# aleflabo/COSKAD

Measured on AMD Instinct MI355X. Metric: pose_clips_per_sec_fwd_bwd, higher is better.
Workload: dtype f32; 1 GPU; euclidean_encoder_dynamicCenter train step (fwd+mse-to-centre+L2 reg+bwd+Adam), synthetic clips B=4096/GPU T=12 V=17 C=2, channels 2-32-16-32-64, latent 16; clips_per_gpu=4096, global_batch=4096, head=euclidean, parallelism=dp1, hip_graph=False

## Files before the change

coskad_amd/csrc/api.hip:

```cpp
#include "common.h"
#include <utility>
#include <vector>

namespace coskad {

char* err_buf() {
  static thread_local char buf[512] = {0};
  return buf;
}

int fail(int code, const char* fmt, ...) {
  va_list ap;
  va_start(ap, fmt);
  vsnprintf(err_buf(), 512, fmt, ap);
  va_end(ap);
  return code;
}

int check_launch(const char* what) {
  hipError_t e = hipGetLastError();
  if (e != hipSuccess) return fail(COSKAD_ERR_LAUNCH, "%s: %s", what, hipGetErrorString(e));
  return COSKAD_OK;
}

}

namespace coskad {
namespace {
struct Probe {
  int kernel = 0, ci = 0, co = 0;
  int stride = 1, seen = 0;
  std::vector<std::pair<hipEvent_t, hipEvent_t>> evs;
} g_probe;
}

ProbeScope::ProbeScope(int kernel, int ci, int co, hipStream_t st) : st_(st) {
  if (g_probe.kernel == kernel && g_probe.ci == ci && g_probe.co == co && g_probe.evs.size() < 4096 &&
      (g_probe.seen++ % g_probe.stride) == 0) {
    hipEvent_t a, b;
    if (hipEventCreate(&a) == hipSuccess && hipEventCreate(&b) == hipSuccess) {
      (void)hipEventRecord(a, st);
      g_probe.evs.emplace_back(a, b);
      armed_ = true;
    }
  }
}
ProbeScope::~ProbeScope() {
  if (armed_) (void)hipEventRecord(g_probe.evs.back().second, st_);
}
}

extern "C" {
int coskad_probe_begin(int kernel, int Ci, int Co) {
  for (auto& e : coskad::g_probe.evs) { (void)hipEventDestroy(e.first); (void)hipEventDestroy(e.second); }
  coskad::g_probe.evs.clear();
  coskad::g_probe.kernel = kernel;
  coskad::g_probe.ci = Ci;
  coskad::g_probe.co = Co;
  coskad::g_probe.seen = 0;
  return COSKAD_OK;
}

int coskad_probe_stride(int n) {
  if (n < 1) return coskad::fail(COSKAD_ERR_ARG, "probe_stride: n=%d", n);
  coskad::g_probe.stride = n;
  return COSKAD_OK;
}

int coskad_probe_end(float* avg_ms, int* launches) {
  double tot = 0.0;
  int n = 0;
  for (auto& e : coskad::g_probe.evs) {
    float ms = 0.f;
    if (hipEventSynchronize(e.second) == hipSuccess && hipEventElapsedTime(&ms, e.first, e.second) == hipSuccess) {
      tot += ms;
      ++n;
    }
    (void)hipEventDestroy(e.first);
    (void)hipEventDestroy(e.second);
  }
  coskad::g_probe.evs.clear();
  coskad::g_probe.kernel = 0;
  if (avg_ms) *avg_ms = n ? (float)(tot / n) : 0.f;
  if (launches) *launches = n;
  return COSKAD_OK;
}

int coskad_abi_version(void) { return COSKAD_ABI_VERSION; }
const char* coskad_last_error(void) { return coskad::err_buf(); }
}
```

coskad_amd/csrc/bottleneck.hip:

```cpp
#include "tile_ops.h"
#include "layer_launch.h"

namespace coskad {

constexpr int kBtlBlock = 256;
constexpr int kBtlWaves = kBtlBlock / 64;
constexpr int kBtlFwdWaves = 8;

__global__ __launch_bounds__(64 * kBtlFwdWaves) void k_btlnk_fwd(const float* __restrict__ U,
                                                     const float* __restrict__ W,
                                                     const float* __restrict__ bias,
                                                     const float* __restrict__ slope,
                                                     float* __restrict__ z, int B, int K, int L) {
  __shared__ float red[kBtlFwdWaves][256];
  const int lane = threadIdx.x & 63, wave = threadIdx.x >> 6;
  const int i = lane & 15, kk = lane >> 4;
  const int n = blockIdx.x * 16 + i;
  const bool pre = slope != nullptr;
  const float a = pre ? slope[0] : 0.f;
  const bool rowok = n < B, colok = i < L;
  const float* up = U + (size_t)(rowok ? n : 0) * K;
  const float* wp = W + (size_t)(colok ? i : 0) * K;
  const int nsteps = ceil_div(K, 16);
  const int per = ceil_div(nsteps, kBtlFwdWaves);
  const int s0 = wave * per, s1 = min(nsteps, s0 + per);
  f32x4 acc = {0.f, 0.f, 0.f, 0.f};
  constexpr int UB = 4;
  for (int sb = s0; sb < s1; sb += UB) {
    float4 x[UB], w[UB];
#pragma unroll
    for (int u = 0; u < UB; ++u) {
      const int k = (sb + u) * 16 + 4 * kk;
      const bool ok = sb + u < s1 && k < K;
      x[u] = (ok && rowok) ? *reinterpret_cast<const float4*>(up + k) : float4{0.f, 0.f, 0.f, 0.f};
      w[u] = (ok && colok) ? *reinterpret_cast<const float4*>(wp + k) : float4{0.f, 0.f, 0.f, 0.f};
    }
#pragma unroll
    for (int u = 0; u < UB; ++u) {
      float4 xv = x[u];
      if (pre) { xv.x = prelu_f(xv.x, a); xv.y = prelu_f(xv.y, a); xv.z = prelu_f(xv.z, a); xv.w = prelu_f(xv.w, a); }
      acc = __builtin_amdgcn_mfma_f32_16x16x4f32(xv.x, w[u].x, acc, 0, 0, 0);
      acc = __builtin_amdgcn_mfma_f32_16x16x4f32(xv.y, w[u].y, acc, 0, 0, 0);
      acc = __builtin_amdgcn_mfma_f32_16x16x4f32(xv.z, w[u].z, acc, 0, 0, 0);
      acc = __builtin_amdgcn_mfma_f32_16x16x4f32(xv.w, w[u].w, acc, 0, 0, 0);
    }
  }
#pragma unroll
  for (int r = 0; r < 4; ++r) red[wave][(4 * (lane >> 4) + r) * 16 + (lane & 15)] = acc[r];
  __syncthreads();
  const int e = threadIdx.x, row = (e >> 4) & 15, col = e & 15;
  const int nn = blockIdx.x * 16 + row;
  if (e < 256 && nn < B && col < L) {
    float s = 0.f;
#pragma unroll
// ... 124 lines not shown
#pragma unroll
    for (int g = 0; g < 4; ++g) {
      const int nn = n0 + c, j = 4 * g + q;
      const float av = (nn < nend && j < L) ? dz[(size_t)nn * L + j] : 0.f;
      dx[0] = __builtin_amdgcn_mfma_f32_16x16x4f32(av, wf[g].x, dx[0], 0, 0, 0);
      dx[1] = __builtin_amdgcn_mfma_f32_16x16x4f32(av, wf[g].y, dx[1], 0, 0, 0);
      dx[2] = __builtin_amdgcn_mfma_f32_16x16x4f32(av, wf[g].z, dx[2], 0, 0, 0);
      dx[3] = __builtin_amdgcn_mfma_f32_16x16x4f32(av, wf[g].w, dx[3], 0, 0, 0);
    }
#pragma unroll
    for (int s = 0; s < 4; ++s) {
      const int nn = n0 + 4 * q + s;
      const bool ok = kok && nn < nend;
      const float4 u = ucur[s];
      float4 x = u;
      if (pre) { x.x = prelu_f(u.x, a); x.y = prelu_f(u.y, a); x.z = prelu_f(u.z, a); x.w = prelu_f(u.w, a); }
      const float dzv = (nn < nend && c < L) ? dz[(size_t)nn * L + c] : 0.f;
      dw[0] = __builtin_amdgcn_mfma_f32_16x16x4f32(dzv, x.x, dw[0], 0, 0, 0);
      dw[1] = __builtin_amdgcn_mfma_f32_16x16x4f32(dzv, x.y, dw[1], 0, 0, 0);
      dw[2] = __builtin_amdgcn_mfma_f32_16x16x4f32(dzv, x.z, dw[2], 0, 0, 0);
      dw[3] = __builtin_amdgcn_mfma_f32_16x16x4f32(dzv, x.w, dw[3], 0, 0, 0);
      float4 g = {dx[0][s], dx[1][s], dx[2][s], dx[3][s]};
      if (pre) {
        da += (u.x < 0.f ? g.x * u.x : 0.f) + (u.y < 0.f ? g.y * u.y : 0.f) +
              (u.z < 0.f ? g.z * u.z : 0.f) + (u.w < 0.f ? g.w * u.w : 0.f);
        g.x = u.x > 0.f ? g.x : a * g.x; g.y = u.y > 0.f ? g.y : a * g.y;
        g.z = u.z > 0.f ? g.z : a * g.z; g.w = u.w > 0.f ? g.w : a * g.w;
      }
      if (ok) *reinterpret_cast<float4*>(dU + (size_t)nn * K + kc) = g;
    }
#pragma unroll
    for (int s = 0; s < 4; ++s) ucur[s] = unext[s];
  }
  if (kok) {
    float* dst = dWp + (size_t)blockIdx.y * L * K;
#pragma unroll
    for (int r = 0; r < 4; ++r) {
      const int j = 4 * q + r;
      if (j < L) *reinterpret_cast<float4*>(dst + (size_t)j * K + kc) = float4{dw[0][r], dw[1][r], dw[2][r], dw[3][r]};
    }
  }
  da = wave_sum(da);
  if (lane == 0) sred[wave] = da;
  __syncthreads();
  if (threadIdx.x == 0) dap[blockIdx.y * gridDim.x + blockIdx.x] = (sred[0] + sred[1]) + (sred[2] + sred[3]);
}

__global__ __launch_bounds__(256) void k_btlnk_reduce(const float* __restrict__ partials, int P, size_t E,
                                                       float* __restrict__ out, const float* __restrict__ dz,
                                                       int B, int L, float* __restrict__ db,
                                                       const float* __restrict__ dap, int nda,
                                                       float* __restrict__ dslope, int accumulate,
                                                       const float* __restrict__ rows, int RP, int RE,
                                                       double* __restrict__ rsum) {
  __shared__ double sh[256];
  const unsigned nE = (unsigned)((E + 255) / 256);
  if (blockIdx.x > nE + L) {
    const int col = threadIdx.x & 15, slice = threadIdx.x >> 4;
    const int e = (int)(blockIdx.x - (nE + L + 1)) * 16 + col;
    double s = 0.0;
    if (e < RE) {
      const float* base = rows + e;
      int p = slice;
      for (; p + 7 * 16 < RP; p += 8 * 16) {
        float v[8];
#pragma unroll
        for (int u = 0; u < 8; ++u) v[u] = base[(size_t)(p + 16 * u) * RE];
#pragma unroll
        for (int u = 0; u < 8; ++u) s += (double)v[u];
      }
      for (; p < RP; p += 16) s += (double)base[(size_t)p * RE];
    }
    sh[threadIdx.x] = s;
    __syncthreads();
    if (slice == 0 && e < RE) {
      double t = 0.0;
#pragma unroll
      for (int k = 0; k < 16; ++k) t += sh[col + 16 * k];
      rsum[e] = t;
    }
    return;
  }
  if (blockIdx.x < nE) {
    const size_t e = (size_t)blockIdx.x * 256 + threadIdx.x;
    if (e >= E) return;
    double s = 0.0;
    int p = 0;
    for (; p + 8 <= P; p += 8) {
      float v[8];
#pragma unroll
      for (int u = 0; u < 8; ++u) v[u] = partials[(size_t)(p + u) * E + e];
#pragma unroll
      for (int u = 0; u < 8; ++u) s += (double)v[u];
    }
    for (; p < P; ++p) s += (double)partials[(size_t)p * E + e];
    out[e] = accumulate ? out[e] + (float)s : (float)s;
    return;
  }
  const int r = (int)(blockIdx.x - nE);
  double s = 0.0;
  if (r < L) {
    if (!db) return;
    for (int n = threadIdx.x; n < B; n += 256) s += (double)dz[(size_t)n * L + r];
  } else {
    if (!dslope) return;
    for (int i = threadIdx.x; i < nda; i += 256) s += (double)dap[i];
  }
  sh[threadIdx.x] = s;
  __syncthreads();
  for (int w = 128; w > 0; w >>= 1) {
    if ((int)threadIdx.x < w) sh[threadIdx.x] += sh[threadIdx.x + w];
    __syncthreads();
  }
  if (threadIdx.x == 0) {
    float* o = r < L ? db + r : dslope;
    o[0] = accumulate ? o[0] + (float)sh[0] : (float)sh[0];
  }
}

static int btl_chunks(int B, int K) {
  const int gx = ceil_div(K, 256);
  int s = (1024 + gx / 2) / gx;
  const int smax = ceil_div(B, 16);
  if (s > smax) s = smax;
  if (s > 64) s = 64;
  return s < 1 ? 1 : s;
}

int launch_btlnk_reduce(const float* partials, int P, size_t E, float* out, const float* dz, int B, int L, float* db,
                        const float* dap, int nda, float* dslope, int accumulate, hipStream_t stream, const float* rows,
                        int RP, int RE, double* rsum) {
  const unsigned extra = rows ? (unsigned)ceil_div(RE, 16) : 0u;
  hipLaunchKernelGGL(k_btlnk_reduce, dim3((unsigned)((E + 255) / 256) + L + 1 + extra), dim3(256), 0, stream, partials, P, E, out, dz,
                     B, L, db, dap, nda, dslope, accumulate, rows, RP, RE, rsum);
  return check_launch("btlnk_bwd_reduce");
}

constexpr int kBtlWideMax = 512;

}

using namespace coskad;

extern "C" {

int coskad_btlnk_fwd_f32(const float* U, const float* W, const float* bias, const float* slope, float* z,
                         int B, int K, int L, hipStream_t stream) {
  if (!U || !W || !z) return fail(COSKAD_ERR_ARG, "btlnk_fwd: null pointer");
  if (B <= 0 || K <= 0 || L <= 0) return fail(COSKAD_ERR_ARG, "btlnk_fwd: B=%d K=%d L=%d", B, K, L);
  if (L > 16) return fail(COSKAD_ERR_SHAPE, "btlnk_fwd: latent_dim=%d > 16 needs the workspace entry point coskad_btlnk_fwd_ws_f32", L);
  if (K % 4) return fail(COSKAD_ERR_SHAPE, "btlnk_fwd: K=%d must be a multiple of 4", K);
  hipLaunchKernelGGL(k_btlnk_fwd, dim3(ceil_div(B, 16)), dim3(64 * kBtlFwdWaves), 0, stream, U, W, bias, slope, z, B, K, L);
  return check_launch("btlnk_fwd");
}

size_t coskad_btlnk_fwd_ws_bytes(int B) { return (size_t)kBtlKS * (size_t)(B > 0 ? B : 0) * 16 * sizeof(float); }

size_t coskad_btlnk_fwd_ws_bytes_l(int B, int K, int L) {
  if (L > 16 && L <= kBtlWideMax) return wide_btlnk_fwd_ws_bytes(B, K, L);
  return coskad_btlnk_fwd_ws_bytes(B);
}

int coskad_btlnk_fwd_ws_f32(const float* U, const float* W, const float* bias, const float* slope, float* z, void* ws,
                            size_t ws_bytes, int B, int K, int L, hipStream_t stream) {
  if (!U || !W || !z || !ws) return fail(COSKAD_ERR_ARG, "btlnk_fwd_ws: null pointer");
  if (B <= 0 || K <= 0 || L <= 0) return fail(COSKAD_ERR_ARG, "btlnk_fwd_ws: B=%d K=%d L=%d", B, K, L);
  if (L > kBtlWideMax) return fail(COSKAD_ERR_SHAPE, "btlnk_fwd_ws: latent_dim=%d > %d not supported", L, kBtlWideMax);
  if (L > 16) {
    if (ws_bytes < wide_btlnk_fwd_ws_bytes(B, K, L)) return fail(COSKAD_ERR_WORKSPACE, "btlnk_fwd_ws: workspace too small");
    return wide_btlnk_fwd(U, W, bias, slope, z, ws, B, K, L, stream);
  }
  if (K % 16) return fail(COSKAD_ERR_SHAPE, "btlnk_fwd_ws: K=%d must be a multiple of 16", K);
  if (ws_bytes < coskad_btlnk_fwd_ws_bytes(B)) return fail(COSKAD_ERR_WORKSPACE, "btlnk_fwd_ws: workspace too small");
  float* part = reinterpret_cast<float*>(ws);
  hipLaunchKernelGGL(k_btlnk_fwd_t, dim3(ceil_div(B, 64), kBtlKS), dim3(256), 0, stream, U, W, slope, part, B, K, L);
  int rc;
  if ((rc = check_launch("btlnk_fwd_t"))) return rc;
  hipLaunchKernelGGL(k_btlnk_fwd_sum, dim3(ceil_div(B * 16, 256)), dim3(256), 0, stream, part, bias, z, B, L, kBtlKS);
  return check_launch("btlnk_fwd_sum");
}

size_t coskad_btlnk_bwd_ws_bytes(int B, int K, int L) {
  if (L > 16 && L <= kBtlWideMax) return wide_btlnk_bwd_ws_bytes(B, K, L);
  const int S = btl_chunks(B, K);
  return ((size_t)S * L * K + (size_t)S * ceil_div(K, 256) + 64) * sizeof(float);
}

int coskad_btlnk_bwd_f32(const float* U, const float* W, const float* dz, const float* slope, float* dU,
                         float* dW, float* db, float* dslope, void* ws, size_t ws_bytes, int accumulate,
                         int B, int K, int L, hipStream_t stream) {
  if (!U || !W || !dz || !dU || !dW || !ws) return fail(COSKAD_ERR_ARG, "btlnk_bwd: null pointer");
  if (B <= 0 || K <= 0 || L <= 0) return fail(COSKAD_ERR_ARG, "btlnk_bwd: B=%d K=%d L=%d", B, K, L);
  if (L > kBtlWideMax) return fail(COSKAD_ERR_SHAPE, "btlnk_bwd: latent_dim=%d > %d not supported", L, kBtlWideMax);
  if (ws_bytes < coskad_btlnk_bwd_ws_bytes(B, K, L)) return fail(COSKAD_ERR_WORKSPACE, "btlnk_bwd: workspace too small");
  if (L > 16) return wide_btlnk_bwd(U, W, dz, slope, dU, dW, db, dslope, ws, accumulate, B, K, L, stream);
  if (K % 4) return fail(COSKAD_ERR_SHAPE, "btlnk_bwd: K=%d must be a multiple of 4", K);
  const int S = btl_chunks(B, K);
  const int chunk = round_up(ceil_div(B, S), 16);
  const int gx = ceil_div(K, 256);
  float* dWp = reinterpret_cast<float*>(ws);
  float* dap = dWp + (size_t)S * L * K;
  {
    ProbeScope probe(KID_BTLNK_BWD, 0, L, stream);
    hipLaunchKernelGGL(k_btlnk_bwd, dim3(gx, S), dim3(kBtlBlock), 0, stream, U, W, dz, slope, dU, dWp, dap, B, K, L, chunk);
  }
  int rc = check_launch("btlnk_bwd");
  if (rc) return rc;
  return launch_btlnk_reduce(dWp, S, (size_t)L * K, dW, dz, B, L, db, dap, gx * S, (dslope && slope) ? dslope : nullptr, accumulate, stream,
                             nullptr, 0, 0, nullptr);
}

}
```

coskad_amd/csrc/btlnk_chain.hip:

```cpp
#include "fused_ops.h"
#include "layer_launch.h"

namespace coskad {
namespace bc {

using ff::f32x4; using ff::mfma; using ff::BufRes; using ff::make_res; using ff::buf_load4; using ff::buf_load1;
__device__ __forceinline__ void buf_store1(BufRes r, int voff, int soff, float v) {
  __builtin_amdgcn_raw_buffer_store_b32(__float_as_uint(v), r, voff, soff, 0);
}

constexpr int HID = 64;
constexpr int PT = 16;
constexpr int NCL = 16;
constexpr int RSTR = 17;
constexpr int kThreads = 512;
#ifndef BC_XCD
#define BC_XCD 1
#endif
#ifndef BC_PF
#define BC_PF 1
#endif
#ifndef BC_SKIP
#define BC_SKIP 0
#endif
// ... 174 lines not shown
      }
  }
  float* row = lds;
  float* red = lds + E;
  const float s4 = ssum + __shfl_xor(ssum, 16, 64);
  const float sch = s4 + __shfl_xor(s4, 32, 64);
  da = wave_sum(da);
  for (int hh = 0; hh < 2; ++hh) {
    if (h == hh) {
#pragma unroll
      for (int t = 0; t < CT; ++t)
#pragma unroll
        for (int r = 0; r < 4; ++r) {
          const int o = 16 * wc + 4 * q + r, cc = 16 * t + c;
          float* p = row + o * Ci + cc;
          p[0] = (hh ? p[0] : 0.f) + pacc[t][r];
          p[HID * Ci] = (hh ? p[HID * Ci] : 0.f) + qacc[t][r];
        }
      if (q == 0) {
        float* p = row + 2 * HID * Ci + 16 * wc + c;
        p[0] = (hh ? p[0] : 0.f) + sch;
      }
      if (lane == 0) red[wave] = da;
    }
    __syncthreads();
  }
  float* dstrow = prow + (size_t)wg * E;
  for (int e = tid; e < E; e += kThreads) dstrow[e] = row[e];
  if (tid == 0) dap[wg] = ((red[0] + red[1]) + (red[2] + red[3])) + ((red[4] + red[5]) + (red[6] + red[7]));
}

struct Plan {
  int npt, S, chunk;
};
static Plan plan(int B, int TV) {
  Plan p;
  p.npt = ceil_div(TV, PT);
  int s = 256 / p.npt;
  const int smax = ceil_div(B, NCL);
  if (s > smax) s = smax;
  if (s < 1) s = 1;
  p.chunk = round_up(ceil_div(B, s), NCL);
  p.S = ceil_div(B, p.chunk);
  return p;
}
static inline size_t sums_offset(int rows, int E) { return ((size_t)rows * E + 1) / 2 * 2; }

}

}

using namespace coskad;

extern "C" {

int coskad_btlnk_bwd_chain_ok(int K, int TV, int below_Ci) {
  return TV > 0 && TV % 4 == 0 && K == bc::HID * TV && (below_Ci == 16 || below_Ci == 32);
}

int coskad_btlnk_bwd_chain_rows(int B, int TV) {
  if (B <= 0 || TV <= 0) return 0;
  const bc::Plan p = bc::plan(B, TV);
  return p.npt * p.S;
}

size_t coskad_btlnk_bwd_chain_floats(int B, int TV, int below_Ci) {
  const size_t E = 2 * (size_t)bc::HID * below_Ci + bc::HID;
  return bc::sums_offset(coskad_btlnk_bwd_chain_rows(B, TV), (int)E) + 2 * E;
}

size_t coskad_btlnk_bwd_chain_ws_bytes(int B, int K, int L, int TV) {
  if (B <= 0 || TV <= 0) return 0;
  const bc::Plan p = bc::plan(B, TV);
  return ((size_t)p.S * L * K + (size_t)p.S * p.npt + 64) * sizeof(float);
}

int coskad_btlnk_bwd_chain_f32(const float* U, const float* W, const float* dz, const float* slope, float* dU, float* dW,
                               float* db, float* dslope, void* ws, size_t ws_bytes, int accumulate, int B, int K, int L,
                               const float* below_in, const float* below_Z, const float* below_in_slope, int below_Ci, int TV,
                               float* stats_out, size_t stats_out_bytes, int* stats_rows, hipStream_t stream) {
  if (!U || !W || !dz || !dU || !dW || !ws || !below_in || !below_Z || !stats_out || !stats_rows)
    return fail(COSKAD_ERR_ARG, "btlnk_bwd_chain: null pointer");
  if (B <= 0 || K <= 0 || L <= 0) return fail(COSKAD_ERR_ARG, "btlnk_bwd_chain: B=%d K=%d L=%d", B, K, L);
  if (L > 16) return fail(COSKAD_ERR_SHAPE, "btlnk_bwd_chain: latent_dim=%d > 16 not supported", L);
  if (!coskad_btlnk_bwd_chain_ok(K, TV, below_Ci))
    return fail(COSKAD_ERR_SHAPE, "btlnk_bwd_chain: K=%d TV=%d below_Ci=%d (needs K = 64 TV, TV %% 4 == 0, 16 / 32 channels below)", K, TV, below_Ci);
  if ((size_t)stats_out & 7) return fail(COSKAD_ERR_ARG, "btlnk_bwd_chain: stats_out must be 8-byte aligned");
  if (ws_bytes < coskad_btlnk_bwd_chain_ws_bytes(B, K, L, TV)) return fail(COSKAD_ERR_WORKSPACE, "btlnk_bwd_chain: workspace too small");
  if (stats_out_bytes < coskad_btlnk_bwd_chain_floats(B, TV, below_Ci) * sizeof(float))
    return fail(COSKAD_ERR_WORKSPACE, "btlnk_bwd_chain: stats_out %zu bytes too small", stats_out_bytes);
  const bc::Plan p = bc::plan(B, TV);
  const int rows = p.npt * p.S;
  const int E = 2 * bc::HID * below_Ci + bc::HID;
  float* dWp = reinterpret_cast<float*>(ws);
  float* dap = dWp + (size_t)p.S * L * K;
  const size_t lds = (size_t)bc::NCL * ((bc::HID * bc::RSTR + 4) + (2 * below_Ci * bc::RSTR + 4)) * sizeof(float);
  int rc;
  {
  ProbeScope probe(KID_BTLNK_BWD, below_Ci, L, stream);
  if (below_Ci == 32) {
    auto k = bc::k_btlnk_bwd_stats<2>;
    (void)hipFuncSetAttribute((const void*)k, hipFuncAttributeMaxDynamicSharedMemorySize, (int)lds);
    hipLaunchKernelGGL(k, dim3(p.npt * p.S), dim3(bc::kThreads), lds, stream, U, W, dz, slope, dU, dWp, dap, below_in, below_Z,
                       below_in_slope, stats_out, B, TV, L, p.chunk);
  } else {
    auto k = bc::k_btlnk_bwd_stats<1>;
    (void)hipFuncSetAttribute((const void*)k, hipFuncAttributeMaxDynamicSharedMemorySize, (int)lds);
    hipLaunchKernelGGL(k, dim3(p.npt * p.S), dim3(bc::kThreads), lds, stream, U, W, dz, slope, dU, dWp, dap, below_in, below_Z,
                       below_in_slope, stats_out, B, TV, L, p.chunk);
  }
  }
  if ((rc = check_launch("btlnk_bwd_stats"))) return rc;
  *stats_rows = rows;
  return launch_btlnk_reduce(dWp, p.S, (size_t)L * K, dW, dz, B, L, db, dap, rows, (dslope && slope) ? dslope : nullptr, accumulate, stream,
                             stats_out, rows, E, reinterpret_cast<double*>(stats_out + bc::sums_offset(rows, E)));
}

}
```

coskad_amd/csrc/common.h:

```cpp
#pragma once
#include <hip/hip_runtime.h>
#include <cstdarg>
#include <cstdio>
#include <cstring>

#define COSKAD_ABI_VERSION 1

#define COSKAD_OK 0
#define COSKAD_ERR_ARG (-1)
#define COSKAD_ERR_SHAPE (-2)
#define COSKAD_ERR_LAUNCH (-3)
#define COSKAD_ERR_WORKSPACE (-4)

namespace coskad {

char* err_buf();
int fail(int code, const char* fmt, ...);
int check_launch(const char* what);

#ifndef COSKAD_BLOCK
#define COSKAD_BLOCK 512
#endif
constexpr int kFlatBlock = COSKAD_BLOCK;
#ifndef COSKAD_MINWAVES
#define COSKAD_MINWAVES 4
#endif
constexpr int kMinWaves = COSKAD_MINWAVES;
constexpr int kMaxLdsBytes = 160 * 1024;
constexpr float kBnEps = 1e-5f;

template <int T, int V>
struct Geo {
  static constexpr int TV = T * V;
  static constexpr int LD = (TV % 2 == 0) ? TV + 1 : TV;
  static constexpr int Block = TV > 256 ? 2 * COSKAD_BLOCK : COSKAD_BLOCK;
  static constexpr int Scratch = (Block / 64) * 256;
};

enum { KID_LAYER_APPLY = 1, KID_BWD_DATA = 2, KID_BWD_REDUCE = 3, KID_FWD_MOMENTS = 4, KID_GCN_PARAMS = 5,
       KID_LAYER_BWD = 6 , KID_FUSED_FWD = 7,
       KID_BTLNK_BWD = 8  };
struct ProbeScope {
  ProbeScope(int kernel, int ci, int co, hipStream_t st);
  ~ProbeScope();
  hipStream_t st_;
  bool armed_ = false;
};

__host__ __device__ inline int ceil_div(int a, int b) { return (a + b - 1) / b; }
__host__ __device__ inline int round_up(int a, int b) { return ceil_div(a, b) * b; }

__device__ __forceinline__ float prelu_f(float x, float a) { return x > 0.f ? x : a * x; }

__device__ __forceinline__ int tid_here() {
  int t = threadIdx.x;
  asm volatile("" : "+v"(t));
  return t;
}

// ... 52 lines not shown
```

coskad_amd/csrc/first_layer.hip:

```cpp
#include "mfma_ops.h"
#include "layer_launch.h"

namespace coskad {
namespace fl {

__device__ __forceinline__ float act(float x, bool pre, float a) { return (pre && x < 0.f) ? a * x : x; }
__device__ __forceinline__ float4 act4(float4 v, bool pre, float a) {
  return float4{act(v.x, pre, a), act(v.y, pre, a), act(v.z, pre, a), act(v.w, pre, a)};
}
__device__ __forceinline__ float dot4(const float4& a, const float4& b) { return (a.x * b.x + a.y * b.y) + (a.z * b.z + a.w * b.w); }

constexpr int NW = 4;
template <int CI, int RW>
__global__ __launch_bounds__(64 * NW, 4) void k_first_stats(const float* __restrict__ in, const float* __restrict__ Zg,
                                                           const float* __restrict__ dU, const float* __restrict__ in_slope,
                                                           float* __restrict__ partials, int B, int Co, int TVr, int need_q) {
  const int lane = threadIdx.x & 63;
  const int wave = uniform(threadIdx.x >> 6);
  const bool pre = in_slope != nullptr;
  const float a_in = pre ? in_slope[0] : 0.f;
  const int n4 = TVr >> 2;
  float pP[RW][CI], pQ[RW][CI], pS[RW];
#pragma unroll
  for (int k = 0; k < RW; ++k) {
    pS[k] = 0.f;
#pragma unroll
    for (int c = 0; c < CI; ++c) { pP[k][c] = 0.f; pQ[k][c] = 0.f; }
  }
  for (int clip = blockIdx.x; clip < B; clip += gridDim.x) {
    const float* gz = Zg + (size_t)clip * CI * TVr;
    const float* gx = in + (size_t)clip * CI * TVr;
    const float* gd = dU + ((size_t)clip * Co + (size_t)wave * RW) * TVr;
    for (int l = lane; l < n4; l += 64) {
      float4 z[CI], x[CI];
#pragma unroll
      for (int c = 0; c < CI; ++c) {
        z[c] = *reinterpret_cast<const float4*>(gz + c * TVr + 4 * l);
        x[c] = need_q ? act4(*reinterpret_cast<const float4*>(gx + c * TVr + 4 * l), pre, a_in) : float4{0.f, 0.f, 0.f, 0.f};
      }
      float4 d[RW];
#pragma unroll
      for (int k = 0; k < RW; ++k)
        d[k] = (wave * RW + k < Co) ? *reinterpret_cast<const float4*>(gd + (size_t)k * TVr + 4 * l) : float4{0.f, 0.f, 0.f, 0.f};
#pragma unroll
      for (int k = 0; k < RW; ++k) {
        pS[k] += (d[k].x + d[k].y) + (d[k].z + d[k].w);
#pragma unroll
        for (int c = 0; c < CI; ++c) {
          pP[k][c] += dot4(d[k], z[c]);
          pQ[k][c] += dot4(d[k], x[c]);
        }
      }
    }
// ... 91 lines not shown
      }
#pragma unroll
      for (int c = 0; c < CI; ++c) *reinterpret_cast<float4*>(part + (wave * CI + c) * TV + 4 * l) = dz[c];
    }
    __syncthreads();
    for (int e = tid; e < CI * TV; e += NTH) {
      const int c = e / TV, p = e - c * TV;
      float v = kt[c];
#pragma unroll
      for (int c2 = 0; c2 < CI; ++c2) v = fmaf(Kt[c2 * CiP + c], Zg[((size_t)clip * CI + c2) * TV + p], v);
#pragma unroll
      for (int w = 0; w < NW; ++w) v += part[(w * CI + c) * TV + p];
      dZl[e] = v;
      Xl[e] = act(in[(size_t)clip * CI * TV + e], pre, a_in);
    }
    __syncthreads();
    for (int e = tid; e < CI * TV; e += NTH) {
      const int c = e / TV, p = e - c * TV, q = p / V, v = p - q * V;
      float y = 0.f, dy = 0.f;
#pragma unroll
      for (int t = 0; t < T; ++t) y = fmaf(Xl[c * TV + t * V + v], TwL[(t * T + q) * V + v], y);
#pragma unroll
      for (int w = 0; w < V; ++w) dy = fmaf(AwL[q * V * V + v * V + w], dZl[c * TV + q * V + w], dy);
      Yl[e] = y;
      dYl[e] = dy;
    }
    __syncthreads();
#pragma unroll
    for (int k = 0; k < KA; ++k) {
      float s = 0.f;
#pragma unroll
      for (int c = 0; c < CI; ++c) s = fmaf(Yl[c * TV + ya[k]], dZl[c * TV + za[k]], s);
      accA[k] += s;
    }
#pragma unroll
    for (int k = 0; k < KT; ++k) {
      float s = 0.f;
#pragma unroll
      for (int c = 0; c < CI; ++c) s = fmaf(Xl[c * TV + xt[k]], dYl[c * TV + yt[k]], s);
      accT[k] += s;
    }
  }
  float* dst = partials + (size_t)blockIdx.x * (NA + NT);
#pragma unroll
  for (int k = 0; k < KA; ++k)
    if (tid + NTH * k < NA) dst[tid + NTH * k] = accA[k];
#pragma unroll
  for (int k = 0; k < KT; ++k)
    if (tid + NTH * k < NT) dst[NA + tid + NTH * k] = accT[k];
}


constexpr int NWM = 8;
template <int T, int V, int CI>
__global__ __launch_bounds__(64 * NWM, 4) void k_first_moments(const float* __restrict__ in, const float* __restrict__ Aw,
                                                          const float* __restrict__ Tw, const float* __restrict__ in_slope,
                                                          float* __restrict__ partials, int B, float* __restrict__ Zout) {
  constexpr int TV = T * V, NA = T * V * V, NT = V * T * T, KP = (TV + 63) / 64;
  extern __shared__ __attribute__((aligned(16))) float lds[];
  float* AwL = lds;
  float* TwL = AwL + NA;
  const int tid = threadIdx.x, lane = tid & 63;
  const int wave = uniform(tid >> 6);
  float* Xl = TwL + NT + wave * 2 * CI * TV;
  float* Yl = Xl + CI * TV;
  const bool pre = in_slope != nullptr;
  const float a_in = pre ? in_slope[0] : 0.f;
  for (int e = tid; e < NA; e += 64 * NWM) AwL[e] = Aw[e];
  for (int e = tid; e < NT; e += 64 * NWM) {
    const int v = e / (T * T), tq = e - v * T * T;
    TwL[tq * V + v] = Tw[e];
  }
  float mx[CI][CI], mz[CI][CI], sx[CI], sz[CI];
#pragma unroll
  for (int a = 0; a < CI; ++a) {
    sx[a] = 0.f; sz[a] = 0.f;
#pragma unroll
    for (int b = 0; b < CI; ++b) { mx[a][b] = 0.f; mz[a][b] = 0.f; }
  }
  __syncthreads();
  const int rounds = (B + gridDim.x * NWM - 1) / (gridDim.x * NWM);
  for (int r = 0; r < rounds; ++r) {
    const int clip = (r * gridDim.x + blockIdx.x) * NWM + wave;
    const bool live = clip < B;
    const float* gx = in + (size_t)(live ? clip : 0) * CI * TV;
#pragma unroll
    for (int k = 0; k < KP; ++k) {
      const int p = lane + 64 * k;
      if (p < TV) {
        float x[CI];
#pragma unroll
        for (int c = 0; c < CI; ++c) {
          x[c] = live ? act(gx[c * TV + p], pre, a_in) : 0.f;
          Xl[c * TV + p] = x[c];
          sx[c] += x[c];
        }
#pragma unroll
        for (int a = 0; a < CI; ++a)
#pragma unroll
          for (int b = 0; b < CI; ++b) mx[a][b] = fmaf(x[a], x[b], mx[a][b]);
      }
    }
    __syncthreads();
#pragma unroll
    for (int k = 0; k < KP; ++k) {
      const int p = lane + 64 * k;
      if (p < TV) {
        const int q = p / V, v = p - q * V;
#pragma unroll
        for (int c = 0; c < CI; ++c) {
          float y = 0.f;
#pragma unroll
          for (int t = 0; t < T; ++t) y = fmaf(Xl[c * TV + t * V + v], TwL[(t * T + q) * V + v], y);
          Yl[c * TV + p] = y;
        }
      }
    }
    __syncthreads();
    float* gz = Zout + (size_t)(live ? clip : 0) * CI * TV;
#pragma unroll
    for (int k = 0; k < KP; ++k) {
      const int p = lane + 64 * k;
      if (p < TV) {
        const int t = p / V, w = p - t * V;
        float z[CI];
#pragma unroll
        for (int c = 0; c < CI; ++c) {
          float acc = 0.f;
#pragma unroll
          for (int v = 0; v < V; ++v) acc = fmaf(Yl[c * TV + t * V + v], AwL[t * V * V + v * V + w], acc);
          z[c] = acc;
          if (live) gz[c * TV + p] = acc;
          sz[c] += acc;
        }
#pragma unroll
        for (int a = 0; a < CI; ++a)
#pragma unroll
          for (int b = 0; b < CI; ++b) mz[a][b] = fmaf(z[a], z[b], mz[a][b]);
      }
    }
    __syncthreads();
  }
  constexpr int E = 2 * (CI * CI + CI);
  float* row = TwL + NT;
  __syncthreads();
#pragma unroll
// ... 71 lines not shown
    else if (Ci == 2) LAUNCH_FS_C(2);
    else if (Ci == 3) LAUNCH_FS_C(3);
    else LAUNCH_FS_C(4);
  }
#undef LAUNCH_FS_C
#undef LAUNCH_FS
  return check_launch("first_stats");
}

template <int T, int V>
static int launch_first_bwd_tv(const float* in, const float* Zg, const float* dU, const float* Aw, const float* Tw, const float* coef,
                               const float* in_slope, float* partials, int B, int Ci, int Co, int max_rows, hipStream_t st,
                               int* rows_out) {
  constexpr int NWB = fl::first_bwd_waves<T, V>();
  int grid = B < 512 ? B : 512;
  if (grid > max_rows) grid = max_rows;
  *rows_out = grid;
  const int rw = ceil_div(Co, NWB);
  const size_t lds = ((size_t)T * V * V + (size_t)V * T * T + (4 + NWB) * (size_t)Ci * T * V) * sizeof(float);
#define LAUNCH_FB1(CI, RW)                                                                                              \
  do {                                                                                                                  \
    auto k = fl::k_first_bwd<T, V, CI, RW>;                                                                             \
    if (lds > 64 * 1024) (void)hipFuncSetAttribute((const void*)k, hipFuncAttributeMaxDynamicSharedMemorySize, (int)lds); \
    hipLaunchKernelGGL(k, dim3(grid), dim3(64 * NWB), lds, st, in, Zg, dU, Aw, Tw, coef, in_slope, partials, B, Co);             \
  } while (0)
#define LAUNCH_FB1_C(CI)                        \
  do {                                          \
    if (rw <= 4) LAUNCH_FB1(CI, 4);             \
    else if (rw <= 8) LAUNCH_FB1(CI, 8);        \
    else LAUNCH_FB1(CI, 16);                    \
  } while (0)
  {
    ProbeScope probe(KID_BWD_DATA, Ci, Co, st);
    if (Ci == 1) LAUNCH_FB1_C(1);
    else if (Ci == 2) LAUNCH_FB1_C(2);
    else if (Ci == 3) LAUNCH_FB1_C(3);
    else LAUNCH_FB1_C(4);
  }
#undef LAUNCH_FB1_C
#undef LAUNCH_FB1
  return check_launch("first_bwd");
}

int launch_first_bwd(const float* in, const float* Zg, const float* dU, const float* Aw, const float* Tw, const float* coef,
                     const float* in_slope, float* partials, int B, int Ci, int Co, int T, int V, int max_rows, hipStream_t st,
                     int* rows_out) {
#define CALL(T_, V_) return launch_first_bwd_tv<T_, V_>(in, Zg, dU, Aw, Tw, coef, in_slope, partials, B, Ci, Co, max_rows, st, rows_out)
  COSKAD_DISPATCH_TV(T, V, CALL);
#undef CALL
}

template <int T, int V>
static int launch_first_moments_tv(const float* in, const float* Aw, const float* Tw, const float* in_slope, float* partials, int B,
                                   int Ci, float* Zout, int max_rows, hipStream_t st, int* rows_out) {
  int grid = (B + fl::NWM - 1) / fl::NWM;
  if (grid > 512) grid = 512;
  if (grid > max_rows) grid = max_rows;
  *rows_out = grid;
  const size_t lds = ((size_t)T * V * V + (size_t)V * T * T + 2 * fl::NWM * (size_t)Ci * T * V) * sizeof(float);
#define LAUNCH_FM(CI)                                                                                                   \
  do {                                                                                                                  \
    auto k = fl::k_first_moments<T, V, CI>;                                                                             \
    if (lds > 64 * 1024) (void)hipFuncSetAttribute((const void*)k, hipFuncAttributeMaxDynamicSharedMemorySize, (int)lds); \
    hipLaunchKernelGGL(k, dim3(grid), dim3(64 * fl::NWM), lds, st, in, Aw, Tw, in_slope, partials, B, Zout);                    \
  } while (0)
  {
    ProbeScope probe(KID_FWD_MOMENTS, Ci, 0, st);
    if (Ci == 1) LAUNCH_FM(1);
    else if (Ci == 2) LAUNCH_FM(2);
    else if (Ci == 3) LAUNCH_FM(3);
    else LAUNCH_FM(4);
  }
#undef LAUNCH_FM
  return check_launch("first_moments");
}

int launch_first_moments(const float* in, const float* Aw, const float* Tw, const float* in_slope, float* partials, int B, int Ci,
                         int T, int V, float* Zout, int max_rows, hipStream_t st, int* rows_out) {
#define CALL(T_, V_) return launch_first_moments_tv<T_, V_>(in, Aw, Tw, in_slope, partials, B, Ci, Zout, max_rows, st, rows_out)
  COSKAD_DISPATCH_TV(T, V, CALL);
#undef CALL
}

int launch_first_apply(const float* Z, const float* in, float* out, const float* wfold, const float* bias, const float* in_slope,
                       int B, int Ci, int Co, int TVr, hipStream_t st) {
  const int grid = B < 2048 ? B : 2048;
  const size_t lds = 2 * (size_t)Ci * TVr * sizeof(float);
  const int CoP = round_up(Co, 16);
#define LAUNCH_FAP(CI) hipLaunchKernelGGL((fl::k_first_apply<CI>), dim3(grid), dim3(256), lds, st, Z, in, out, wfold, bias, in_slope, B, Co, CoP, TVr)
  {
    ProbeScope probe(KID_LAYER_APPLY, Ci, Co, st);
    if (Ci == 1) LAUNCH_FAP(1);
    else if (Ci == 2) LAUNCH_FAP(2);
    else if (Ci == 3) LAUNCH_FAP(3);
    else LAUNCH_FAP(4);
  }
#undef LAUNCH_FAP
  return check_launch("first_apply");
}

}
```

coskad_amd/csrc/fused_apply_next.hip:

```cpp
#include "fused_ops.h"
#include "layer_launch.h"

#ifndef FN_ABLATE
#define FN_ABLATE 0
#endif

namespace coskad {
namespace fn {

using namespace ff;

struct FtabArgs {
  const float* A[4];
  const float* Tm[4];
  float* tab[4];
};
__global__ void k_build_ftab(FtabArgs args) {
  const int layer = blockIdx.y;
  const float* __restrict__ Aw = args.A[layer];
  const float* __restrict__ Tw = args.Tm[layer];
  const int e = blockIdx.x * blockDim.x + threadIdx.x;
  if (e >= LAYER_F4 * 4) return;
  float val = 0.f;
  if (e < TEMP_F4 * 4) {
    const int v = e / 256, l = (e >> 2) & 63, s = e & 3, j = l & 15, q = l >> 4;
    if (s < 3 && j < T) val = Tw[v * T * T + (4 * s + q) * T + j];
  } else {
    const int r = e - TEMP_F4 * 4;
    const int t = r / (3 * 256), c = (r / 256) % 3, l = (r >> 2) & 63, k = 4 * c + (r & 3), j = l & 15, q = l >> 4;
    if (k < 10) {
      const int s = k < 5 ? k : k - 5, w = 4 * s + q;
      if (w < V) val = Aw[t * V * V + w * V + (k < 5 ? j : 16)];
    }
  }
  args.tab[layer][e] = val;
}

template <int CT, int OTP>
__global__ __launch_bounds__(256, 1) void k_layer_apply_next(const float* __restrict__ in, const float* __restrict__ Zg,
                                                            const float* __restrict__ wfold, const float* __restrict__ bias,
                                                            const float* __restrict__ in_slope, const float* __restrict__ out_slope,
                                                            const float* __restrict__ ftab, float* __restrict__ out,
                                                            float* __restrict__ Znext, float* __restrict__ partials, int B) {
  constexpr int Ci = CT ? 16 * CT : 2, Co = 16 * OTP, CoP = Co, NG = 2 * CT;
  constexpr int NACC = OTP == 1 ? 2 : 3;
  constexpr int E = 2 * (Co * Co + Co);
  static_assert(OTP == 1 || OTP == 2, "the 32-row image holds the whole output");
  extern __shared__ __attribute__((aligned(16))) float lds_all[];
  const int lane = threadIdx.x & 63;
  const int wave = __builtin_amdgcn_readfirstlane(threadIdx.x >> 6);
  float* lds = lds_all + wave * WAVE_LDS_W;
  float* r1 = lds + R1;
  float* r2 = lds + R2;
  auto geo = [&]() {
    int l = lane;
    asm volatile("" : "+v"(l));
    return Lane{l & 15, l >> 4};
  };
  auto olane = [&]() {
    int l = lane;
    asm volatile("" : "+v"(l));
    return l;
  };
  const bool pre = in_slope != nullptr;
  const float a_in = pre ? in_slope[0] : 0.f;
  const float a_out = out_slope[0];
  const int l16 = lane * 16;
  const BufRes wres = make_res(wfold, 2 * Ci * CoP * 4u);
  const BufRes bres = make_res(bias, CoP * 4u);
  const BufRes tabres = make_res(ftab, LAYER_F4 * 16u);
  const int nwaves = gridDim.x * 4;
  auto clip_res = [&](const float* base, int c, int rows) {
    const bool in_range = c < B;
#ifdef COSKAD_HOT
    return make_res(base + (size_t)(in_range ? (c & 63) : 0) * rows * TV, in_range ? rows * TV * 4u : 0u);
#else
    return make_res(base + (size_t)(in_range ? c : 0) * rows * TV, in_range ? rows * TV * 4u : 0u);
#endif
  };
  constexpr int QTAIL = 4 * (TV / 4) - 192;
  const int l16t = lane < QTAIL ? l16 : 0x7ffffff0;
  float4 gb[16];
  auto qload = [&](const BufRes& res, int row0, int q) {
#pragma unroll
    for (int c = 0; c < 4; ++c) gb[4 * q + c] = buf_load4(res, c < 3 ? l16 : l16t, ((row0 + 4 * q) * (TV / 4) + 64 * c) * 16);
  };
  auto qstore = [&](int q, bool act) {
    const int ln = olane();
// ... 202 lines not shown
  }

  float* row = lds_all;
  __syncthreads();
  const Lane L = geo();
  auto put = [&](int w, float* base, const f32x4 (&g)[NACC], const float (&s)[OTP]) {
#pragma unroll
    for (int r = 0; r < 4; ++r) {
      const int i = 4 * L.q + r, j = L.j;
      if constexpr (OTP == 1) {
        float* p = base + i * Co + j;
        p[0] = (w ? p[0] : 0.f) + (g[0][r] + g[1][r]);
      } else {
        float* p00 = base + i * Co + j;
        float* p01 = base + i * Co + 16 + j;
        float* p10 = base + (16 + j) * Co + i;
        float* p11 = base + (16 + i) * Co + 16 + j;
        p00[0] = (w ? p00[0] : 0.f) + g[0][r];
        p01[0] = (w ? p01[0] : 0.f) + g[1][r];
        p10[0] = (w ? p10[0] : 0.f) + g[1][r];
        p11[0] = (w ? p11[0] : 0.f) + g[2][r];
      }
    }
#pragma unroll
    for (int rt = 0; rt < OTP; ++rt) {
      const float t = quad_sum(s[rt]);
      if (L.q == 0) {
        float* p = base + Co * Co + 16 * rt + L.j;
        p[0] = (w ? p[0] : 0.f) + t;
      }
    }
  };
  for (int w = 0; w < 4; ++w) {
    if (wave == w) {
      put(w, row, gx, sx);
      put(w, row + Co * Co + Co, gz, sz);
    }
    __syncthreads();
  }
  float* dst = partials + (size_t)blockIdx.x * E;
  for (int e = threadIdx.x; e < E; e += 256) dst[e] = row[e];
}

}

bool layer_apply_next_ok(int T_, int V_, int Ci, int Co) {
  return T_ == ff::T && V_ == ff::V && (Ci == 2 || Ci == 16 || Ci == 32) && (Co == 16 || Co == 32);
}

int ftab_floats() { return ff::LAYER_F4 * 4; }

int launch_build_ftab(const float* const* A, const float* const* Tm, float* const* tab, int n, hipStream_t st) {
  if (n < 1 || n > 4) return fail(COSKAD_ERR_ARG, "build_ftab: 1..4 layers per launch, got %d", n);
  fn::FtabArgs args{};
  for (int i = 0; i < n; ++i) {
    if (!A[i] || !Tm[i] || !tab[i]) return fail(COSKAD_ERR_ARG, "build_ftab: null pointer (layer %d)", i);
    args.A[i] = A[i]; args.Tm[i] = Tm[i]; args.tab[i] = tab[i];
  }
  hipLaunchKernelGGL(fn::k_build_ftab, dim3(ceil_div(ff::LAYER_F4 * 4, 256), n), dim3(256), 0, st, args);
  return check_launch("build_ftab");
}

static bool apply_next_bpc_on(int Ci, int Co) { return (Ci == 2 && Co == 32) || (Ci == 32 && Co == 16) || (Ci == 16 && Co == 32); }
int layer_apply_next_rows(int B, int Ci, int Co) {
  if (apply_next_bpc_on(Ci, Co)) return apply_next_bpc_rows(B);
  const int nblk = (B + 3) / 4;
  return nblk < 256 ? nblk : 256;
}

int launch_layer_apply_next(const float* Z, const float* in, float* out, const float* wfold, const float* bias,
                            const float* in_slope, const float* out_slope, const float* ftab, float* Znext, float* partials,
                            int B, int Ci, int Co, hipStream_t st, int* rows_out) {
  const size_t lds = (size_t)4 * ff::WAVE_LDS_W * sizeof(float);
  const int grid = layer_apply_next_rows(B, Ci, Co);
  *rows_out = grid;
  if (apply_next_bpc_on(Ci, Co))
    return launch_layer_apply_next_bpc(Z, in, out, wfold, bias, in_slope, out_slope, ftab, Znext, partials, B, Ci, Co, st);
#define LAUNCH_FN(CT, OTP)                                                                                            \
  do {                                                                                                                \
    auto k = fn::k_layer_apply_next<CT, OTP>;                                                                         \
    (void)hipFuncSetAttribute((const void*)k, hipFuncAttributeMaxDynamicSharedMemorySize, (int)lds);                  \
    hipLaunchKernelGGL(k, dim3(grid), dim3(256), lds, st, in, Z, wfold, bias, in_slope, out_slope, ftab, out, Znext,  \
                       partials, B);                                                                                  \
  } while (0)
  {
    ProbeScope probe(KID_LAYER_APPLY, Ci, Co, st);
    if (Ci == 2 && Co == 16) LAUNCH_FN(0, 1);
    else if (Ci == 2 && Co == 32) LAUNCH_FN(0, 2);
    else if (Ci == 16 && Co == 16) LAUNCH_FN(1, 1);
    else if (Ci == 16 && Co == 32) LAUNCH_FN(1, 2);
    else if (Ci == 32 && Co == 16) LAUNCH_FN(2, 1);
    else if (Ci == 32 && Co == 32) LAUNCH_FN(2, 2);
    else return fail(COSKAD_ERR_SHAPE, "apply_next: unsupported channels (%d, %d)", Ci, Co);
  }
#undef LAUNCH_FN
  return check_launch("layer_apply_next");
}

}

using namespace coskad;
extern "C" {

int coskad_layer_apply_next_ok(int Ci, int Co, int T, int V) { return layer_apply_next_ok(T, V, Ci, Co) ? 1 : 0; }
int coskad_ftab_floats(void) { return ftab_floats(); }
int coskad_layer_apply_next_rows(int B, int Ci, int Co) { return layer_apply_next_rows(B, Ci, Co); }

// ... 24 lines not shown
```

coskad_amd/csrc/fused_ops.h:

```cpp
#pragma once
#include "common.h"

namespace coskad {
namespace ff {

using f32x4 = __attribute__((ext_vector_type(4))) float;

constexpr int T = 12, V = 17, TV = T * V;
#ifndef FF_LD
#define FF_LD 206
#endif
constexpr int LD = FF_LD;
constexpr int R1 = 0, R2 = 32 * LD;
constexpr int PADCOL = TV;
constexpr int WAVE_LDS = 48 * LD;
constexpr int LDW = 208;
constexpr int WAVE_LDS_W = 32 * LD + 16 * LDW;
constexpr int NTILE = T + 1;
#ifndef FF_AB_UNROLL
#define FF_AB_UNROLL _Pragma("unroll")
#endif
#ifndef FF_ABLATE
#define FF_ABLATE 0
#endif
#ifndef FF_CABL
#define FF_CABL 0
#endif
#ifndef FF_TILE_FENCE
#define FF_TILE_FENCE
#endif
constexpr int KP = NTILE * 4 * 64 * 4;
constexpr int TEMP_F4 = V * 64;
constexpr int LAYER_F4 = TEMP_F4 + T * 3 * 64;
enum { W1A = 0, W1B = 2, WP = 4, WR = 12, WX3 = 20, WZ3 = 28, WZ4 = 36, WX4 = 68, B1 = 100, B2 = 108, B3 = 112, B4 = 120, NWREG = 136 };

__device__ __forceinline__ f32x4 mfma(float a, float b, f32x4 c) {
  return __builtin_amdgcn_mfma_f32_16x16x4f32(a, b, c, 0, 0, 0);
}
__device__ __forceinline__ float prelu(float x, float a) { return x > 0.f ? x : a * x; }
__device__ __forceinline__ f32x4 prelu4(f32x4 v, float a) {
  return f32x4{prelu(v[0], a), prelu(v[1], a), prelu(v[2], a), prelu(v[3], a)};
}

struct Lane {
  int j, q;
};

using u32x4 = __attribute__((ext_vector_type(4))) unsigned int;
using BufRes = __amdgpu_buffer_rsrc_t;
__device__ __forceinline__ BufRes make_res(const void* p, unsigned bytes) {
  return __builtin_amdgcn_make_buffer_rsrc(const_cast<void*>(p), 0, bytes, 0x00020000);
}
__device__ __forceinline__ float4 buf_load4(BufRes r, int voff, int soff) {
  const u32x4 v = __builtin_amdgcn_raw_buffer_load_b128(r, voff, soff, 0);
  return float4{__uint_as_float(v[0]), __uint_as_float(v[1]), __uint_as_float(v[2]), __uint_as_float(v[3])};
}
__device__ __forceinline__ float buf_load1(BufRes r, int voff, int soff) {
  return __uint_as_float(__builtin_amdgcn_raw_buffer_load_b32(r, voff, soff, 0));
}
__device__ __forceinline__ void buf_store4(BufRes r, int voff, int soff, const float4& v) {
  const u32x4 u = {__float_as_uint(v.x), __float_as_uint(v.y), __float_as_uint(v.z), __float_as_uint(v.w)};
  __builtin_amdgcn_raw_buffer_store_b128(u, r, voff, soff, 0);
}

struct TOp {
  float a0, a1, a2;
};
template <int ROWS, bool ACT = false>
__device__ __forceinline__ TOp temporal_read(const float* img, int rt, int v, const Lane& L, float slope = 0.f) {
  const float* p = img + (16 * rt + L.j) * LD + L.q * V + v;
  TOp o{p[0], p[4 * V], p[8 * V]};
  if (ACT) { o.a0 = prelu(o.a0, slope); o.a1 = prelu(o.a1, slope); o.a2 = prelu(o.a2, slope); }
  if (ROWS < 16) {
    const bool ok = L.j < ROWS;
    o.a0 = ok ? o.a0 : 0.f; o.a1 = ok ? o.a1 : 0.f; o.a2 = ok ? o.a2 : 0.f;
  }
  return o;
}
__device__ __forceinline__ f32x4 temporal_mm(const TOp& o, const float4& rec) {
  f32x4 acc = {0.f, 0.f, 0.f, 0.f};
  acc = mfma(o.a0, rec.x, acc);
  acc = mfma(o.a1, rec.y, acc);
  acc = mfma(o.a2, rec.z, acc);
  return acc;
}
template <int ROWS>
// ... 230 lines not shown
```

coskad_amd/csrc/heads.hip:

```cpp
#include "tile_ops.h"
#include "heads_common.h"

namespace coskad {

struct Vec {
  float v[LMAX];
};

__device__ __forceinline__ Vec load_vec(const float* p, int L) {
  Vec r;
#pragma unroll
  for (int j = 0; j < LMAX; ++j) r.v[j] = j < L ? p[j] : 0.f;
  return r;
}
__device__ __forceinline__ void store_vec(float* p, const Vec& a, int L) {
#pragma unroll
  for (int j = 0; j < LMAX; ++j)
    if (j < L) p[j] = a.v[j];
}
__device__ __forceinline__ float dot(const Vec& a, const Vec& b) {
  float s = 0.f;
#pragma unroll
  for (int j = 0; j < LMAX; ++j) s = fmaf(a.v[j], b.v[j], s);
  return s;
}

struct Embed {
  Vec p;
  float un_raw, un, tn, en_raw;
  bool clamped;
};
__device__ __forceinline__ Embed hyp_embed(const Vec& u) {
  Embed r;
  r.un_raw = sqrtf(dot(u, u));
  r.un = fmaxf(r.un_raw, kMinNorm);
  r.tn = tanhf(fminf(fmaxf(r.un, -kTanhClamp), kTanhClamp));
  const float f = r.tn / r.un;
  Vec e;
#pragma unroll
  for (int j = 0; j < LMAX; ++j) e.v[j] = f * u.v[j];
  r.en_raw = sqrtf(dot(e, e));
  const float en = fmaxf(r.en_raw, kMinNorm);
  const float maxnorm = 1.f - kBallEps;
  r.clamped = en > maxnorm;
  const float s = r.clamped ? maxnorm / en : 1.f;
#pragma unroll
  for (int j = 0; j < LMAX; ++j) r.p.v[j] = r.clamped ? e.v[j] / en * maxnorm : e.v[j];
  (void)s;
  return r;
}

__device__ __forceinline__ float poincare_dist(const Vec& c, const Vec& p, Vec* gp) {
  const float x2 = dot(c, c), y2 = dot(p, p), xy = -dot(c, p);
  const float alpha = 1.f + 2.f * xy + y2, beta = 1.f - x2;
  const float den = 1.f + 2.f * xy + x2 * y2;
  const float D = den + kMobiusEps;
  Vec m;
#pragma unroll
  for (int j = 0; j < LMAX; ++j) m.v[j] = (alpha * (-c.v[j]) + beta * p.v[j]) / D;
  const float mn = sqrtf(dot(m, m));
  const float mc = fminf(fmaxf(mn, -1.f + kArtanhEps), 1.f - kArtanhEps);
  const float d = (log1pf(mc) - log1pf(-mc));
  if (gp) {
    const float gmn = 2.f / (1.f - mc * mc);
    const float inv = mn > 0.f ? gmn / mn : 0.f;
    Vec gm;
#pragma unroll
    for (int j = 0; j < LMAX; ++j) gm.v[j] = inv * m.v[j];
    const float gD = -dot(gm, m) / D;
    float galpha = 0.f;
#pragma unroll
// ... 16 lines not shown
    float egp = 0.f;
#pragma unroll
    for (int j = 0; j < LMAX; ++j) egp = fmaf(f * u.v[j], gp.v[j], egp);
#pragma unroll
    for (int j = 0; j < LMAX; ++j) ge.v[j] = maxnorm * (gp.v[j] / en - f * u.v[j] * egp / (en * en * en));
  } else {
    ge = gp;
  }
  Vec gu;
  float gf = dot(ge, u);
  float coef = 0.f;
  if (em.un_raw > kMinNorm) {
    const float sech2 = em.un < kTanhClamp ? 1.f - em.tn * em.tn : 0.f;
    const float df = (sech2 * em.un - em.tn) / (em.un * em.un);
    coef = gf * df / em.un_raw;
  }
#pragma unroll
  for (int j = 0; j < LMAX; ++j) gu.v[j] = f * ge.v[j] + coef * u.v[j];
  return gu;
}

constexpr int kHeadSlots = LMAX + 3;

constexpr int kHeadSingleRows = kFlatBlock;
__host__ __device__ inline int head_blocks(int B) { return B <= kHeadSingleRows ? 1 : ceil_div(B, kFlatBlock); }

__device__ __forceinline__ void block_partials(const float (&vals)[kHeadSlots], float* partials, float scale0, float* stats,
                                               float* acc) {
  __shared__ float sh[kFlatBlock / 64][kHeadSlots];
  const int lane = threadIdx.x & 63, wave = threadIdx.x >> 6;
#pragma unroll
  for (int k = 0; k < kHeadSlots; ++k) {
    const float s = wave_sum(vals[k]);
    if (lane == 0) sh[wave][k] = s;
  }
  __syncthreads();
  if (threadIdx.x < kHeadSlots) {
    float s = 0.f;
    for (int w = 0; w < kFlatBlock / 64; ++w) s += sh[w][threadIdx.x];
    if (gridDim.x == 1) {
      if (stats) stats[threadIdx.x] = threadIdx.x == 0 ? s * scale0 : s;
      if (acc) acc[threadIdx.x] += s;
    } else {
      partials[blockIdx.x * kHeadSlots + threadIdx.x] = s;
    }
  }
}

__global__ __launch_bounds__(kFlatBlock) void k_mse_head(const float* __restrict__ z,
                                                    const float* __restrict__ cvec,
                                                    float* __restrict__ dz, float* __restrict__ score,
                                                    float* __restrict__ partials, int B, int L,
                                                    float gscale, float scale0, float* __restrict__ stats,
                                                    float* __restrict__ acc) {
  float vals[kHeadSlots];
#pragma unroll
  for (int k = 0; k < kHeadSlots; ++k) vals[k] = 0.f;
  const Vec c = load_vec(cvec, L);
#pragma unroll 4
  for (int n = blockIdx.x * kFlatBlock + threadIdx.x; n < B; n += gridDim.x * kFlatBlock) {
    const Vec u = load_vec(z + (size_t)n * L, L);
    Vec g;
    float sq = 0.f;
#pragma unroll
    for (int j = 0; j < LMAX; ++j) {
      const float d = j < L ? u.v[j] - c.v[j] : 0.f;
      sq = fmaf(d, d, sq);
      g.v[j] = 2.f * d * gscale;
      vals[1 + j] += u.v[j];
    }
    vals[0] += sq;
    vals[LMAX + 1] += 1.f;
    vals[LMAX + 2] += sqrtf(dot(u, u));
    if (dz) store_vec(dz + (size_t)n * L, g, L);
    if (score) score[n] = sq / (float)L;
  }
  block_partials(vals, partials, scale0, stats, acc);
}

__global__ __launch_bounds__(kFlatBlock) void k_mahalanobis_head(const float* __restrict__ z,
                                                            const float* __restrict__ cvec,
                                                            const float* __restrict__ VI,
                                                            float* __restrict__ dz, float* __restrict__ score,
                                                            float* __restrict__ partials, int B, int L,
                                                            float gscale, float scale0, float* __restrict__ stats,
                                                            float* __restrict__ acc) {
  __shared__ float vi[LMAX * LMAX];
  for (int e = threadIdx.x; e < LMAX * LMAX; e += kFlatBlock) {
    const int r = e / LMAX, q = e - r * LMAX;
    vi[e] = (r < L && q < L) ? VI[r * L + q] : 0.f;
  }
  __syncthreads();
  float vals[kHeadSlots];
#pragma unroll
  for (int k = 0; k < kHeadSlots; ++k) vals[k] = 0.f;
  const Vec c = load_vec(cvec, L);
  for (int n = blockIdx.x * kFlatBlock + threadIdx.x; n < B; n += gridDim.x * kFlatBlock) {
    const Vec u = load_vec(z + (size_t)n * L, L);
    Vec d, w, wt;
#pragma unroll
    for (int j = 0; j < LMAX; ++j) { d.v[j] = j < L ? u.v[j] - c.v[j] : 0.f; w.v[j] = 0.f; wt.v[j] = 0.f; }
#pragma unroll
    for (int r = 0; r < LMAX; ++r)
#pragma unroll
      for (int q = 0; q < LMAX; ++q) {
        const float a = vi[r * LMAX + q];
        w.v[r] = fmaf(a, d.v[q], w.v[r]);
        wt.v[q] = fmaf(a, d.v[r], wt.v[q]);
      }
    const float dist = sqrtf(dot(d, w));
    vals[0] += dist;
#pragma unroll
    for (int j = 0; j < LMAX; ++j) vals[1 + j] += u.v[j];
    vals[LMAX + 1] += 1.f;
    vals[LMAX + 2] += sqrtf(dot(u, u));
    if (score) score[n] = dist;
    if (dz) {
      Vec g;
      const float inv = gscale / (2.f * dist);
#pragma unroll
      for (int j = 0; j < LMAX; ++j) g.v[j] = (w.v[j] + wt.v[j]) * inv;
      store_vec(dz + (size_t)n * L, g, L);
    }
  }
  block_partials(vals, partials, scale0, stats, acc);
}

// ... 6 lines not shown
  for (int n0 = 0; n0 < B; n0 += CH) {
    const int nc = min(CH, B - n0);
    __syncthreads();
    for (int e = threadIdx.x; e < nc * L; e += LMAX * LMAX) {
      const int r = e / L, q = e - r * L;
      zs[r * LMAX + q] = z[(size_t)(n0 + r) * L + q];
    }
    __syncthreads();
    if (i < L && j < L)
      for (int r = 0; r < nc; ++r) s = fmaf(zs[r * LMAX + i], zs[r * LMAX + j], s);
  }
  if (i < L && j < L) gram[i * L + j] = accumulate ? gram[i * L + j] + s : s;
}

__global__ __launch_bounds__(kFlatBlock) void k_poincare_head(const float* __restrict__ z,
                                                         const float* __restrict__ cvec,
                                                         float* __restrict__ dz, float* __restrict__ zh,
                                                         float* __restrict__ score,
                                                         float* __restrict__ partials, int B, int L,
                                                         float gscale, float scale0, float* __restrict__ stats,
                                                         float* __restrict__ acc) {
  float vals[kHeadSlots];
#pragma unroll
  for (int k = 0; k < kHeadSlots; ++k) vals[k] = 0.f;
  for (int n = blockIdx.x * kFlatBlock + threadIdx.x; n < B; n += gridDim.x * kFlatBlock) {
    const Vec u = load_vec(z + (size_t)n * L, L);
    const Embed em = hyp_embed(u);
    if (zh) store_vec(zh + (size_t)n * L, em.p, L);
    const float y2 = dot(em.p, em.p);
    const float gamma = 2.f / (1.f - y2);
#pragma unroll
    for (int j = 0; j < LMAX; ++j) vals[1 + j] += gamma * em.p.v[j];
    vals[LMAX + 1] += gamma - 1.f;
    vals[LMAX + 2] += sqrtf(y2);
    if (cvec) {
      const Vec c = load_vec(cvec, L);
      Vec gp;
      const float d = poincare_dist(c, em.p, dz ? &gp : nullptr);
      vals[0] += d;
      if (score) score[n] = d;
      if (dz) {
#pragma unroll
        for (int j = 0; j < LMAX; ++j) gp.v[j] *= gscale;
        store_vec(dz + (size_t)n * L, hyp_embed_bwd(u, em, gp), L);
      }
    }
  }
  block_partials(vals, partials, scale0, stats, acc);
}

__global__ __launch_bounds__(64) void k_head_finalize(const float* __restrict__ partials, int P,
                                                       float scale0, float* __restrict__ stats,
                                                       float* __restrict__ acc) {
  const int k = threadIdx.x;
  if (k >= kHeadSlots) return;
  double s = 0.0;
  for (int p = 0; p < P; ++p) s += (double)partials[p * kHeadSlots + k];
  if (stats) stats[k] = (float)(k == 0 ? s * (double)scale0 : s);
  if (acc) acc[k] += (float)s;
}

__global__ __launch_bounds__(kFlatBlock) void k_poincare_dist(const float* __restrict__ zh,
                                                         const float* __restrict__ cvec,
                                                         float* __restrict__ score, int B, int L) {
  const int n = blockIdx.x * kFlatBlock + threadIdx.x;
  if (n >= B) return;
  const Vec p = load_vec(zh + (size_t)n * L, L), c = load_vec(cvec, L);
  score[n] = poincare_dist(c, p, nullptr);
}

__global__ __launch_bounds__(kFlatBlock) void k_poincare_logmap0(const float* __restrict__ y, float* __restrict__ out, int B, int L) {
  const int n = blockIdx.x * kFlatBlock + threadIdx.x;
  if (n >= B) return;
  const Vec p = load_vec(y + (size_t)n * L, L);
  const float yn = fmaxf(sqrtf(dot(p, p)), kMinNorm);
  const float yc = fminf(fmaxf(yn, -1.f + kArtanhEps), 1.f - kArtanhEps);
  const float at = 0.5f * (log1pf(yc) - log1pf(-yc));
  Vec o;
#pragma unroll
  for (int j = 0; j < LMAX; ++j) o.v[j] = p.v[j] / yn * at;
  store_vec(out + (size_t)n * L, o, L);
}

__global__ void k_midpoint_finalize(const float* __restrict__ acc, float* __restrict__ cvec, int L) {
  if (threadIdx.x != 0 || blockIdx.x != 0) return;
  const double s = fmax((double)acc[LMAX + 1], 1e-10);
  double m[LMAX], mn2 = 0.0;
  for (int j = 0; j < L; ++j) { m[j] = (double)acc[1 + j] / s; mn2 += m[j] * m[j]; }
  const double mn = fmax(sqrt(mn2), 1e-15);
  const double mc = fmin(mn, 1.0 - 1e-7);
  const double at = 0.5 * log((1.0 + mc) / (1.0 - mc));
  const double sc = tanh(0.5 * at) / mn;
  for (int j = 0; j < L; ++j) cvec[j] = (float)(sc * m[j]);
}

__global__ void k_center_finalize(const float* __restrict__ acc, float eps, float* __restrict__ cvec,
                                  int L) {
  const int j = threadIdx.x;
  if (j >= L || blockIdx.x != 0) return;
  float c = acc[1 + j] / acc[LMAX + 1];
  if (fabsf(c) < eps && c < 0.f) c = -eps;
  if (fabsf(c) < eps && c > 0.f) c = eps;
  cvec[j] = c;
}

__global__ __launch_bounds__(256) void k_sqnorm_masked(const float* __restrict__ p,
                                                        const float* __restrict__ mask, size_t n,
                                                        float* __restrict__ partials) {
  __shared__ float sh[4];
  float s = 0.f;
  for (size_t i = (size_t)blockIdx.x * 256 + threadIdx.x; i < n; i += (size_t)gridDim.x * 256) {
    const float v = p[i];
// ... 33 lines not shown
__global__ __launch_bounds__(256) void k_adam_dev(float* __restrict__ p, const float* __restrict__ g,
                                                   float* __restrict__ m, float* __restrict__ v,
                                                   const float* __restrict__ mask, size_t n,
                                                   const float* __restrict__ hyper, float beta1, float beta2,
                                                   float eps, float gscale, float reg_coef) {
  const size_t i = (size_t)blockIdx.x * 256 + threadIdx.x;
  if (i >= n) return;
  const float lr = hyper[0], bc1 = 1.f - hyper[1], bc2s = sqrtf(1.f - hyper[2]);
  const float pi = p[i];
  float gi = g[i] * gscale;
  if (reg_coef != 0.f) gi = fmaf(reg_coef * (mask ? mask[i] : 1.f), pi, gi);
  const float mi = beta1 * m[i] + (1.f - beta1) * gi;
  const float vi = beta2 * v[i] + (1.f - beta2) * gi * gi;
  m[i] = mi;
  v[i] = vi;
  p[i] = pi - (lr / bc1) * (mi / (sqrtf(vi) / bc2s + eps));
}

__global__ __launch_bounds__(256) void k_scale_sum(const float* __restrict__ v, int n, float scale,
                                                    float* __restrict__ out) {
  __shared__ double sh[256];
  double s = 0.0;
  for (int i = threadIdx.x; i < n; i += 256) s += (double)v[i];
  sh[threadIdx.x] = s;
  __syncthreads();
  for (int w = 128; w > 0; w >>= 1) {
    if (threadIdx.x < w) sh[threadIdx.x] += sh[threadIdx.x + w];
    __syncthreads();
  }
  if (threadIdx.x == 0) out[0] = (float)(sh[0] * (double)scale);
}

}

using namespace coskad;

extern "C" {

int coskad_head_slots(void) { return kHeadSlots; }
size_t coskad_head_ws_floats(int B) { return (size_t)ceil_div(B, kFlatBlock) * kHeadSlots; }
int coskad_head_slots_l(int L) { return L > 0 && L <= kWideLMax ? head_slots_for(L) : 0; }
size_t coskad_head_ws_floats_l(int B, int L) {
  if (L > LMAX && L <= kWideLMax) return wide_head_ws_floats(B, L);
  return coskad_head_ws_floats(B);
}

int coskad_mse_head_f32(const float* z, const float* c, float* dz, float* score, float* stats, float* acc,
                        float upstream, float* ws, int B, int L, hipStream_t stream) {
  if (!z || !c || !ws) return fail(COSKAD_ERR_ARG, "mse_head: null pointer");
  if (B <= 0 || L <= 0 || L > kWideLMax) return fail(COSKAD_ERR_SHAPE, "mse_head: B=%d latent=%d (max %d)", B, L, kWideLMax);
  if (L > LMAX) return wide_mse_head(z, c, dz, score, stats, acc, upstream, ws, B, L, stream);
  const int P = head_blocks(B);
  hipLaunchKernelGGL(k_mse_head, dim3(P), dim3(kFlatBlock), 0, stream, z, c, dz, score, ws, B, L,
                     upstream / ((float)B * (float)L), 1.f / ((float)B * (float)L), stats, acc);
  if ((stats || acc) && P > 1)
    hipLaunchKernelGGL(k_head_finalize, dim3(1), dim3(64), 0, stream, ws, P, 1.f / ((float)B * (float)L), stats, acc);
  return check_launch("mse_head");
}

int coskad_mahalanobis_head_f32(const float* z, const float* c, const float* VI, float* dz, float* score,
                                float* stats, float* acc, float* gram, int gram_accumulate, float upstream,
                                float* ws, int B, int L, hipStream_t stream) {
  if (!z || !c || !VI || !ws) return fail(COSKAD_ERR_ARG, "mahalanobis_head: null pointer");
  if (B <= 0 || L <= 0 || L > kWideLMax) return fail(COSKAD_ERR_SHAPE, "mahalanobis_head: B=%d latent=%d (max %d)", B, L, kWideLMax);
  if (L > LMAX) return wide_mahalanobis_head(z, c, VI, dz, score, stats, acc, gram, gram_accumulate, upstream, ws, B, L, stream);
  const int P = head_blocks(B);
  hipLaunchKernelGGL(k_mahalanobis_head, dim3(P), dim3(kFlatBlock), 0, stream, z, c, VI, dz, score, ws, B, L,
                     upstream / (float)B, 1.f / (float)B, stats, acc);
  if ((stats || acc) && P > 1)
    hipLaunchKernelGGL(k_head_finalize, dim3(1), dim3(64), 0, stream, ws, P, 1.f / (float)B, stats, acc);
  if (gram) hipLaunchKernelGGL(k_gram, dim3(1), dim3(LMAX * LMAX), 0, stream, z, gram, B, L, gram_accumulate);
  return check_launch("mahalanobis_head");
}

int coskad_poincare_head_f32(const float* z, const float* c, float* dz, float* zh, float* score,
                             float* stats, float* acc, float upstream, float* ws, int B, int L,
                             hipStream_t stream) {
  if (!z || !ws) return fail(COSKAD_ERR_ARG, "poincare_head: null pointer");
  if (B <= 0 || L <= 0 || L > kWideLMax) return fail(COSKAD_ERR_SHAPE, "poincare_head: B=%d latent=%d (max %d)", B, L, kWideLMax);
  if (L > LMAX) return wide_poincare_head(z, c, dz, zh, score, stats, acc, upstream, ws, B, L, stream);
  const int P = head_blocks(B);
  hipLaunchKernelGGL(k_poincare_head, dim3(P), dim3(kFlatBlock), 0, stream, z, c, dz, zh, score, ws, B, L,
                     upstream / (float)B, 1.f / (float)B, stats, acc);
  if ((stats || acc) && P > 1)
    hipLaunchKernelGGL(k_head_finalize, dim3(1), dim3(64), 0, stream, ws, P, 1.f / (float)B, stats, acc);
  return check_launch("poincare_head");
}

int coskad_poincare_dist_f32(const float* zh, const float* c, float* score, int B, int L, hipStream_t stream) {
  if (!zh || !c || !score) return fail(COSKAD_ERR_ARG, "poincare_dist: null pointer");
  if (B <= 0 || L <= 0 || L > kWideLMax) return fail(COSKAD_ERR_SHAPE, "poincare_dist: B=%d latent=%d (max %d)", B, L, kWideLMax);
  if (L > LMAX) return wide_poincare_dist(zh, c, score, B, L, stream);
  hipLaunchKernelGGL(k_poincare_dist, dim3(ceil_div(B, kFlatBlock)), dim3(kFlatBlock), 0, stream, zh, c, score, B, L);
  return check_launch("poincare_dist");
}

int coskad_poincare_logmap0_f32(const float* y, float* out, int B, int L, hipStream_t stream) {
  if (!y || !out) return fail(COSKAD_ERR_ARG, "poincare_logmap0: null pointer");
  if (B <= 0 || L <= 0 || L > kWideLMax) return fail(COSKAD_ERR_SHAPE, "poincare_logmap0: B=%d latent=%d (max %d)", B, L, kWideLMax);
  if (L > LMAX) return wide_poincare_logmap0(y, out, B, L, stream);
  hipLaunchKernelGGL(k_poincare_logmap0, dim3(ceil_div(B, kFlatBlock)), dim3(kFlatBlock), 0, stream, y, out, B, L);
  return check_launch("poincare_logmap0");
}

int coskad_center_finalize_f32(const float* acc, float* c, float eps, int L, hipStream_t stream) {
  if (!acc || !c || L <= 0 || L > kWideLMax) return fail(COSKAD_ERR_ARG, "center_finalize: bad argument (latent=%d, max %d)", L, kWideLMax);
  if (L > LMAX) return wide_center_finalize(acc, c, eps, L, stream);
  hipLaunchKernelGGL(k_center_finalize, dim3(1), dim3(64), 0, stream, acc, eps, c, L);
  return check_launch("center_finalize");
}

// ... 47 lines not shown
```

coskad_amd/csrc/heads_common.h:

```cpp
#pragma once
#include "common.h"

namespace coskad {

constexpr int LMAX = 16;
constexpr int kWideLMax = 512;
constexpr float kMinNorm = 1e-5f;
constexpr float kBallEps = 1e-3f;
constexpr float kArtanhEps = 1e-5f;
constexpr float kMobiusEps = 1e-5f;
constexpr float kTanhClamp = 15.f;

__host__ __device__ inline int head_lp(int L) { return L > LMAX ? L : LMAX; }
__host__ __device__ inline int head_slots_for(int L) { return head_lp(L) + 3; }

size_t wide_head_ws_floats(int B, int L);
int wide_mse_head(const float* z, const float* c, float* dz, float* score, float* stats, float* acc, float upstream, float* ws,
                  int B, int L, hipStream_t stream);
int wide_mahalanobis_head(const float* z, const float* c, const float* VI, float* dz, float* score, float* stats, float* acc,
                          float* gram, int gram_accumulate, float upstream, float* ws, int B, int L, hipStream_t stream);
int wide_poincare_head(const float* z, const float* c, float* dz, float* zh, float* score, float* stats, float* acc,
                       float upstream, float* ws, int B, int L, hipStream_t stream);
int wide_poincare_dist(const float* zh, const float* c, float* score, int B, int L, hipStream_t stream);
int wide_poincare_logmap0(const float* y, float* out, int B, int L, hipStream_t stream);
int wide_center_finalize(const float* acc, float* c, float eps, int L, hipStream_t stream);
int wide_midpoint_finalize(const float* acc, float* c, int L, hipStream_t stream);

}
```

coskad_amd/csrc/layer_launch.h:

```cpp
#pragma once
#include "common.h"
#include <cstdlib>
#include <type_traits>

extern "C" int coskad_window_ok(int T, int V);
extern "C" int coskad_layer_train_window_ok(int T, int V, int Ci, int Co);
extern "C" int coskad_layer_train_window_narrow_ok(int T, int V, int Ci, int Co);

namespace coskad {

#ifdef COSKAD_ABLATE
inline int ablate_env(const char* name, int dflt) {
  const char* e = getenv(name);
  return e ? atoi(e) : dflt;
}
#else
constexpr int ablate_env(const char*, int dflt) { return dflt; }
#endif

template <class F>
inline void with_tiles(int n, F&& f) {
  if (n == 1) f(std::integral_constant<int, 1>{});
  else if (n == 2) f(std::integral_constant<int, 2>{});
  else if (n == 3) f(std::integral_constant<int, 3>{});
// ... 26 lines not shown
  float* stats = nullptr;
};
struct StatsOnly {
  float* out = nullptr;
  int* rows_out = nullptr;
};
struct LayerBwdArgs {
  const float* in = nullptr;
  const float* dU = nullptr;
  const float* A = nullptr;
  const float* Tm = nullptr;
  const float* in_slope = nullptr;
  const float* stat = nullptr;
  const float* Wt = nullptr;
  const float* gt = nullptr;
  const float* Wr = nullptr;
  const float* gr = nullptr;
  const float* Z = nullptr;
  LayerGrads g;
  void* ws = nullptr;
  size_t ws_bytes = 0;
  int accumulate = 0;
  int B = 0, Ci = 0, Co = 0;
  hipStream_t stream = nullptr;
  ChainIn chain;
  double stats_count = 0.0;
  Below below;
  StatsOnly stats_only;
  float* dz_ext = nullptr;
};

struct BnConvParams {
  const float* Wt = nullptr;
  const float* bt = nullptr;
  const float* gt = nullptr;
  const float* bet = nullptr;
  float* rm_t = nullptr;
  float* rv_t = nullptr;
  long long* nbt_t = nullptr;
  const float* Wr = nullptr;
  const float* br = nullptr;
  const float* gr = nullptr;
  const float* ber = nullptr;
  float* rm_r = nullptr;
  float* rv_r = nullptr;
  long long* nbt_r = nullptr;
  float momentum = 0.f;
};
struct FoldOut {
  float* wfold = nullptr;
  float* bias = nullptr;
  float* stat = nullptr;
};
struct LayerStatsArgs {
  const float* in = nullptr;
  const float* A = nullptr;
  const float* Tm = nullptr;
  const float* in_slope = nullptr;
  const float* partials = nullptr;
  int rows = 0;
  BnConvParams p;
  FoldOut out;
  float* Zout = nullptr;
  double* sums = nullptr;
  void* ws = nullptr;
  size_t ws_bytes = 0;
  int B = 0, Ci = 0, Co = 0;
  hipStream_t stream = nullptr;
};

void launch_reduce_partials(const float* partials, int rows, int E, double* out, hipStream_t st);

int launch_window_gcn(const float* in, float* out, const float* Aw, const float* Tw, int rows, int T, int V, int adjoint,
                      hipStream_t st);
int launch_window_params(const float* x, const float* dZ, const float* Aw, const float* Tw, float* dA, float* dT, void* ws,
                         int accumulate, int rows, int T, int V, hipStream_t st, float* dX, const float* add,
                         const float* in_slope = nullptr, float* dap = nullptr, int* rows_out = nullptr);
size_t window_params_ws_bytes(int T, int V);

bool window_moments_ok(int T, int V, int Ci);
int launch_window_moments(const float* in, const float* Aw, const float* Tw, const float* in_slope, float* partials, int B, int Ci,
                          int T, int V, int need_x, float* Zout, hipStream_t st, int* rows_out);
bool window_flat_ok(int TV, int Ci, int Co);
int launch_window_apply(const float* Z, const float* in, float* out, const float* wfold, const float* bias, const float* in_slope,
                        int B, int Ci, int Co, int TV, hipStream_t st);
int launch_window_stats(const float* in, const float* Zg, const float* dU, const float* in_slope, float* partials, int B, int Ci, int Co,
                        int TV, int need_q, hipStream_t st, int* rows_out);
int launch_window_data(const float* in, const float* Z, const float* dU, const float* coef, const float* in_slope, float* dZ, float* dXr,
                       int B, int Ci, int Co, int TV, hipStream_t st);

int layer_bwd_below_rows(int T_, int V_, int B, int Ci, int Co, int below_Ci);
int launch_layer_bwd_bpc(const float* in, const float* Zg, const float* dU, const float* coef, const float* in_slope, float* dIn,
                         float* btab, float* partials, float* dap, int B, int Ci, int Co, hipStream_t st, int* rows_out,
                         const float* below_z, const float* below_x, const float* below_slope, int below_Ci, float* below_stats);
bool layer_bwd_fused_ok(int T_, int V_, int Ci, int Co);
int launch_reduce_fused(const float* partials, int rows, float* dA, float* dT, const float* dap, float* dslope, int accumulate,
                        hipStream_t st, const float* brows, int bE, double* bout);
bool bwd_stats_ring_ok(int T_, int V_, int Ci, int Co);
int launch_bwd_stats_ring(const float* in, const float* Zg, const float* dU, const float* in_slope, float* partials, int B,
                          int Ci, int Co, hipStream_t st, int* rows_out);
bool bwd_stats_bpc_ok(int T_, int V_, int Ci, int Co);
bool bwd_stats_flat_ok(int TV_, int Ci, int Co);
int launch_bwd_stats_flat(const float* in, const float* Zg, const float* dU, const float* in_slope, float* partials, int B,
                          int Ci, int Co, int TV_, hipStream_t st, int* rows_out);
int launch_bwd_stats_bpc(const float* in, const float* Zg, const float* dU, const float* in_slope, float* partials, int B,
                         int Ci, int Co, hipStream_t st, int* rows_out);
bool bwd_data_bpc_ok(int T_, int V_, int Ci, int Co);
int launch_bwd_data_bpc(const float* in, const float* Zg, const float* dU, const float* Aw, const float* Tw, const float* coef,
                        const float* in_slope, float* dIn, float* dZout, float* dap, int B, int Ci, int Co, int T_, int V_,
                        hipStream_t st, int* rows_out, float* gpart);
bool gcn_params_bpc_ok(int T_, int V_);
int launch_gcn_params_bpc(const float* in, const float* in_slope, const float* dz, const float* Aw, const float* Tw, float* partials,
                          int rows_total, int T_, int V_, hipStream_t st, int* rows_out);
bool first_layer_ok(int T_, int V_, int Ci, int Co);
int launch_first_stats(const float* in, const float* Zg, const float* dU, const float* in_slope, float* partials, int B, int Ci,
                       int Co, int TVr, int need_q, int max_rows, hipStream_t st, int* rows_out);
int launch_first_bwd(const float* in, const float* Zg, const float* dU, const float* Aw, const float* Tw, const float* coef,
                     const float* in_slope, float* partials, int B, int Ci, int Co, int T, int V, int max_rows, hipStream_t st,
                     int* rows_out);
int launch_first_moments(const float* in, const float* Aw, const float* Tw, const float* in_slope, float* partials, int B, int Ci,
                         int T, int V, float* Zout, int max_rows, hipStream_t st, int* rows_out);
int launch_first_apply(const float* Z, const float* in, float* out, const float* wfold, const float* bias, const float* in_slope,
                       int B, int Ci, int Co, int TVr, hipStream_t st);
bool fwd_moments_bpc_ok(int T_, int V_, int Ci);
int launch_fwd_moments_bpc(const float* in, const float* Aw, const float* Tw, const float* in_slope, float* partials, int B, int Ci,
                           int T_, int V_, int need_x, float* Zout, hipStream_t st, int* rows_out);
int launch_combine_moments_bpc(const float* Zy, const float* YR, const float* stat, float* U, const float* Aw, const float* Tw,
                               const float* slope, float* partials, int B, int T_, int V_, float* Zout, hipStream_t st, int* rows_out);
template <int T, int V>
int launch_layer_apply_m(const float* in, float* out, const float* Aw, const float* Tw, const float* wfold,
                         const float* bias, const float* in_slope, const float* out_slope, int B, int Ci,
                         int Co, hipStream_t st, const float* Zg);
bool eval_layer_bpc_ok(int T_, int V_, int Ci, int Co);
int launch_eval_layer_bpc(const float* in, float* out, const float* Aw, const float* Tw, const float* wfold, const float* bias,
                          const float* in_slope, const float* out_slope, int B, int Ci, int Co, int T_, int V_, hipStream_t st);
bool eval_layer_window_ok(int T_, int V_, int Ci, int Co);
int launch_eval_layer_window(const float* in, float* out, const float* Aw, const float* Tw, const float* wfold, const float* bias,
                             const float* in_slope, const float* out_slope, int B, int Ci, int Co, int T_, int V_, hipStream_t st);
bool eval_first_pair_window_ok(int T_, int V_, int Ci, int Cm, int Co);
int launch_eval_first_pair_window(const float* x, float* out, const float* A1, const float* T1, const float* wfold1,
                                  const float* bias1, const float* A2, const float* T2, const float* wfold2, const float* bias2,
                                  const float* mid_slope, const float* out_slope, int B, int Co, int T_, int V_, hipStream_t st);
bool layer_apply_ring_ok(int T_, int V_, int Ci, int Co);
int launch_layer_apply_ring(const float* Z, const float* in, float* out, const float* wfold, const float* bias,
                            const float* in_slope, int B, int Ci, int Co, hipStream_t st);
int launch_layer_apply_bpc(const float* Z, const float* in, float* out, const float* wfold, const float* bias,
                           const float* in_slope, int B, int Ci, int Co, hipStream_t st);
bool layer_apply_flat_ok(int TV_, int Ci, int Co);
int launch_layer_apply_flat(const float* Z, const float* in, float* out, const float* wfold, const float* bias,
                            const float* in_slope, int B, int Ci, int Co, int TV_, hipStream_t st);
int launch_commute_apply_mix(const float* in, float* out, const float* wt, const float* wr, const float* in_slope, const float* Aw,
                             const float* Tw, float* zy, float* mixpart, int B, int Ci, int Jo, int TV_, hipStream_t st, int* rows_out);
int apply_next_bpc_rows(int B);
int launch_layer_apply_next_bpc(const float* Z, const float* in, float* out, const float* wfold, const float* bias,
                                const float* in_slope, const float* out_slope, const float* ftab, float* Znext, float* partials,
                                int B, int Ci, int Co, hipStream_t st);
int launch_btlnk_reduce(const float* partials, int P, size_t E, float* out, const float* dz, int B, int L, float* db,
                        const float* dap, int nda, float* dslope, int accumulate, hipStream_t stream, const float* rows,
                        int RP, int RE, double* rsum);
size_t wide_btlnk_fwd_ws_bytes(int B, int K, int L);
size_t wide_btlnk_bwd_ws_bytes(int B, int K, int L);
int wide_btlnk_fwd(const float* U, const float* W, const float* bias, const float* slope, float* z, void* ws, int B, int K, int L,
                   hipStream_t stream);
int wide_btlnk_bwd(const float* U, const float* W, const float* dz, const float* slope, float* dU, float* dW, float* db,
                   float* dslope, void* ws, int accumulate, int B, int K, int L, hipStream_t stream);

}
```

coskad_amd/csrc/stsgcn_train.hip:

```cpp
#include "mfma_ops.h"
#include "layer_launch.h"

namespace coskad {

constexpr int kMaxGrid = 768;

template <int T, int V, int NTC>
__global__ __launch_bounds__((Geo<T, V>::Block), (Geo<T, V>::Block <= 512 && NTC <= 2 ? 6 : 4)) void k_fwd_moments(const float* __restrict__ in,
                                                       const float* __restrict__ Aw,
                                                       const float* __restrict__ Tw,
                                                       const float* __restrict__ in_slope,
                                                       float* __restrict__ partials, int B, int Ci,
                                                       int NB, int need_x, float* __restrict__ Zout) {
  constexpr int kScratchFloats = Geo<T, V>::Scratch;
  constexpr int TV = Geo<T, V>::TV, LD = TV + 2;
  extern __shared__ __attribute__((aligned(16))) float lds[];
  float* scratch = lds;
  float* AwL = lds + max(NB * Ci * LD, kScratchFloats);
  float* TwL = AwL + T * V * V;
  copy_to_lds(AwL, Aw, T * V * V);
  copy_to_lds(TwL, Tw, V * T * T);
  const bool pre = in_slope != nullptr;
  const float a_in = pre ? in_slope[0] : 0.f;
  f32x4 mx[NTC][NTC], mz[NTC][NTC];
// ... 219 lines not shown
size_t train_stats_ws_bytes(int Ci) {
  const size_t E = 2 * ((size_t)Ci * Ci + Ci);
  return kMaxGrid * E * sizeof(float) + round_up((int)(E * sizeof(double)), 256) + 256;
}

void launch_reduce_partials(const float* partials, int rows, int E, double* out, hipStream_t st) {
  hipLaunchKernelGGL(k_reduce_partials, dim3(ceil_div(E, kRedCols)), dim3(1024), 0, st, partials, rows, E, out);
}

static int launch_reduce_fold(const float* partials, int rows, double* red, double npos, const BnConvParams& p, const FoldOut& o,
                              int Ci, int Co, hipStream_t st) {
  const int E = 2 * (Ci * Ci + Ci);
  int rc = 0;
  const bool self_sum = partials && p.Wt && E <= kFoldSelfSum;
  if (partials && !self_sum) {
    launch_reduce_partials(partials, rows, E, red, st);
    if ((rc = check_launch("reduce_partials"))) return rc;
  }
  if (!p.Wt) return 0;
  const size_t fold_lds = (2 * (size_t)Ci * Ci + 2 * Ci) * sizeof(double) + (4 * (size_t)Co * Ci + 4 * Co) * sizeof(float);
  if (fold_lds > 64 * 1024) (void)hipFuncSetAttribute((const void*)k_train_fold, hipFuncAttributeMaxDynamicSharedMemorySize, (int)fold_lds);
  const int fold_blocks = Co >= 32 ? 8 : (Co >= 16 ? 4 : 1);
  hipLaunchKernelGGL(k_train_fold, dim3(fold_blocks), dim3(1024), fold_lds, st, red, npos, p.Wt, p.bt, p.gt, p.bet, p.rm_t,
                     p.rv_t, p.nbt_t, p.Wr, p.br, p.gr, p.ber, p.rm_r, p.rv_r, p.nbt_r, p.momentum, o.wfold, o.bias, o.stat, Ci,
                     Co, round_up(Co, 16), self_sum ? partials : (const float*)nullptr, rows);
  return check_launch("train_fold");
}

template <int T, int V>
static int launch_train_stats(const LayerStatsArgs& a) {
  constexpr int kBlock = Geo<T, V>::Block;
  constexpr int kScratchFloats = Geo<T, V>::Scratch;
  constexpr int TV = Geo<T, V>::TV, LD = TV + 2;
  static_assert(TV % 4 == 0, "the moments kernel stages with float4 and needs TV + 2 == 2 (mod 4)");
  const int B = a.B, Ci = a.Ci, Co = a.Co;
  hipStream_t st = a.stream;
  if (Ci > 64) return fail(COSKAD_ERR_SHAPE, "train_stats: C_in=%d > 64 not supported", Ci);
  if (a.ws_bytes < train_stats_ws_bytes(Ci))
    return fail(COSKAD_ERR_WORKSPACE, "train_stats: workspace %zu < %zu bytes", a.ws_bytes, train_stats_ws_bytes(Ci));
  const int E = 2 * (Ci * Ci + Ci);
  int NB = Ci >= 32 ? 1 : 32 / Ci;
  if (NB > B) NB = B;
  const size_t img = (size_t)NB * Ci * LD > (size_t)kScratchFloats ? (size_t)NB * Ci * LD : (size_t)kScratchFloats;
  const size_t lds = (img + (size_t)T * V * V + (size_t)V * T * T) * sizeof(float);
  if (lds > (size_t)kMaxLdsBytes) return fail(COSKAD_ERR_SHAPE, "train_stats: LDS %zu too large", lds);
  const int ntiles = ceil_div(B, NB);
  const int per_cu = lds <= (size_t)52 * 1024 && Ci <= 32 && kBlock <= 512 ? 3 : (lds <= (size_t)80 * 1024 ? 2 : 1);
  const int grid = ntiles < 256 * per_cu ? ntiles : 256 * per_cu;
  float* partials = reinterpret_cast<float*>(a.ws);
  double* red = reinterpret_cast<double*>(reinterpret_cast<char*>(a.ws) + round_up((int)(kMaxGrid * (size_t)E * sizeof(float)), 256));
  const int need_x = a.sums ? 1 : (a.p.Wr != nullptr);
  int rows = grid;
  if (a.Zout && Ci <= 4 && TV % 4 == 0) {
    int rc1 = launch_first_moments(a.in, a.A, a.Tm, a.in_slope, partials, B, Ci, T, V, a.Zout, kMaxGrid, st, &rows);
    if (rc1) return rc1;
  } else if (a.Zout && fwd_moments_bpc_ok(T, V, Ci)) {
    ProbeScope probe(KID_FWD_MOMENTS, Ci, Co, st);
    int rc1 = launch_fwd_moments_bpc(a.in, a.A, a.Tm, a.in_slope, partials, B, Ci, T, V, need_x, a.Zout, st, &rows);
    if (rc1) return rc1;
  } else {
    ProbeScope probe(KID_FWD_MOMENTS, Ci, Co, st);
    with_tiles(ceil_div(Ci, 16), [&](auto NTC) {
      auto k = k_fwd_moments<T, V, decltype(NTC)::value>;
      if (lds > 64 * 1024) (void)hipFuncSetAttribute((const void*)k, hipFuncAttributeMaxDynamicSharedMemorySize, (int)lds);
      hipLaunchKernelGGL(k, dim3(grid), dim3(kBlock), lds, st, a.in, a.A, a.Tm, a.in_slope, partials, B, Ci, NB, need_x, a.Zout);
    });
  }
  int rc = check_launch("fwd_moments");
  if (rc) return rc;
  if (a.sums) return launch_reduce_fold(partials, rows, a.sums, 0.0, BnConvParams{}, FoldOut{}, Ci, Co, st);
  return launch_reduce_fold(partials, rows, red, (double)B * TV, a.p, a.out, Ci, Co, st);
}

enum : unsigned {
  kNeedInput = 1,
  kNeedPartials = 2,
  kNeedSums = 4,
  kNeedFold = 8,
  kNeedWs = 16,
};
static int check_layer_stats(const char* who, const LayerStatsArgs& a, unsigned need) {
  bool null = false;
  if (need & kNeedInput) null = null || !a.in || !a.A || !a.Tm;
  if (need & kNeedPartials) null = null || !a.partials;
  if (need & kNeedSums) null = null || !a.sums;
  if (need & kNeedFold) null = null || !a.p.Wt || !a.p.gt || !a.p.bet || !a.out.wfold || !a.out.bias || !a.out.stat;
  if (need & kNeedWs) null = null || !a.ws;
  if (null) return fail(COSKAD_ERR_ARG, "%s: null pointer", who);
  if (need & kNeedFold) {
    if (a.p.Wr && (!a.p.gr || !a.p.ber)) return fail(COSKAD_ERR_ARG, "%s: residual BN missing", who);
    if (!a.p.Wr && a.Ci != a.Co) return fail(COSKAD_ERR_ARG, "%s: identity residual needs Ci == Co", who);
  }
  return COSKAD_OK;
}

static int launch_train_stats_window(const LayerStatsArgs& a, int T, int V) {
  const int B = a.B, Ci = a.Ci, Co = a.Co;
  if (a.ws_bytes < train_stats_ws_bytes(Ci))
    return fail(COSKAD_ERR_WORKSPACE, "train_stats: workspace %zu < %zu bytes", a.ws_bytes, train_stats_ws_bytes(Ci));
  const int E = 2 * (Ci * Ci + Ci);
  float* partials = reinterpret_cast<float*>(a.ws);
  double* red = reinterpret_cast<double*>(reinterpret_cast<char*>(a.ws) + round_up((int)(kMaxGrid * (size_t)E * sizeof(float)), 256));
  const int need_x = a.sums ? 1 : (a.p.Wr != nullptr);
  int rows = 0;
  if (int rc = launch_window_moments(a.in, a.A, a.Tm, a.in_slope, partials, B, Ci, T, V, need_x, a.Zout, a.stream, &rows)) return rc;
  if (a.sums) return launch_reduce_fold(partials, rows, a.sums, 0.0, BnConvParams{}, FoldOut{}, Ci, Co, a.stream);
  return launch_reduce_fold(partials, rows, red, (double)B * T * V, a.p, a.out, Ci, Co, a.stream);
}

static int dispatch_train_stats(const char* who, const LayerStatsArgs& a, int T, int V, bool full) {
  if (coskad_window_ok(T, V)) {
    if ((size_t)a.in & 15) return fail(COSKAD_ERR_ARG, "%s: `in` must be 16-byte aligned at window lengths 8, 16 and 24", who);
    if ((size_t)a.Zout & 15) return fail(COSKAD_ERR_ARG, "%s: `Z` must be 16-byte aligned at window lengths 8, 16 and 24", who);
    if (full ? (coskad_layer_train_window_ok(T, V, a.Ci, a.Co) || coskad_layer_train_window_narrow_ok(T, V, a.Ci, a.Co))
             : window_moments_ok(T, V, a.Ci))
      return launch_train_stats_window(a, T, V);
  }
#define CALL(T_, V_) return launch_train_stats<T_, V_>(a)
  COSKAD_DISPATCH_TV(T, V, CALL);
#undef CALL
}

}

using namespace coskad;

extern "C" {

size_t coskad_train_stats_ws_bytes(int Ci) { return train_stats_ws_bytes(Ci); }
int coskad_stat_floats(int Ci, int Co) { return stat_floats(Ci, Co); }

int coskad_layer_train_stats_z_f32(const float* in, const float* A, const float* Tm, const float* in_slope,
                                 const float* Wt, const float* bt, const float* gamma_t,
                                 const float* beta_t, float* rmean_t, float* rvar_t, long long* nbt_t,
                                 const float* Wr, const float* br, const float* gamma_r,
                                 const float* beta_r, float* rmean_r, float* rvar_r, long long* nbt_r,
                                 float momentum, float* wfold, float* bias, float* stat, void* ws,
                                 size_t ws_bytes, int B, int Ci, int Co, int T, int V,
                                 hipStream_t stream, float* Z) {
  const LayerStatsArgs a{
      .in = in, .A = A, .Tm = Tm, .in_slope = in_slope,
      .p = {.Wt = Wt, .bt = bt, .gt = gamma_t, .bet = beta_t, .rm_t = rmean_t, .rv_t = rvar_t, .nbt_t = nbt_t, .Wr = Wr, .br = br,
            .gr = gamma_r, .ber = beta_r, .rm_r = rmean_r, .rv_r = rvar_r, .nbt_r = nbt_r, .momentum = momentum},
      .out = {.wfold = wfold, .bias = bias, .stat = stat},
      .Zout = Z, .ws = ws, .ws_bytes = ws_bytes, .B = B, .Ci = Ci, .Co = Co, .stream = stream};
  if (int rc = check_layer_stats("layer_train_stats", a, kNeedInput | kNeedFold | kNeedWs)) return rc;
  if (B <= 0 || Ci <= 0 || Co <= 0) return fail(COSKAD_ERR_ARG, "layer_train_stats: B=%d Ci=%d Co=%d", B, Ci, Co);
  return dispatch_train_stats("layer_train_stats", a, T, V, true);
}

int coskad_layer_train_stats_f32(const float* in, const float* A, const float* Tm, const float* in_slope,
                                 const float* Wt, const float* bt, const float* gamma_t,
                                 const float* beta_t, float* rmean_t, float* rvar_t, long long* nbt_t,
                                 const float* Wr, const float* br, const float* gamma_r,
                                 const float* beta_r, float* rmean_r, float* rvar_r, long long* nbt_r,
                                 float momentum, float* wfold, float* bias, float* stat, void* ws,
                                 size_t ws_bytes, int B, int Ci, int Co, int T, int V,
                                 hipStream_t stream) {
  return coskad_layer_train_stats_z_f32(in, A, Tm, in_slope, Wt, bt, gamma_t, beta_t, rmean_t, rvar_t, nbt_t, Wr, br, gamma_r, beta_r,
                                        rmean_r, rvar_r, nbt_r, momentum, wfold, bias, stat, ws, ws_bytes, B, Ci, Co, T, V, stream,
                                        nullptr);
}

int coskad_layer_train_fold_f32(const float* partials, int rows, const float* Wt, const float* bt, const float* gamma_t,
                                const float* beta_t, float* rmean_t, float* rvar_t, long long* nbt_t,
                                const float* Wr, const float* br, const float* gamma_r,
                                const float* beta_r, float* rmean_r, float* rvar_r, long long* nbt_r,
                                float momentum, float* wfold, float* bias, float* stat, void* ws,
                                size_t ws_bytes, int B, int Ci, int Co, int T, int V, hipStream_t stream) {
  const LayerStatsArgs a{
      .partials = partials, .rows = rows,
      .p = {.Wt = Wt, .bt = bt, .gt = gamma_t, .bet = beta_t, .rm_t = rmean_t, .rv_t = rvar_t, .nbt_t = nbt_t, .Wr = Wr, .br = br,
            .gr = gamma_r, .ber = beta_r, .rm_r = rmean_r, .rv_r = rvar_r, .nbt_r = nbt_r, .momentum = momentum},
      .out = {.wfold = wfold, .bias = bias, .stat = stat},
      .ws = ws, .ws_bytes = ws_bytes, .B = B, .Ci = Ci, .Co = Co, .stream = stream};
  if (int rc = check_layer_stats("layer_train_fold", a, kNeedPartials | kNeedFold | kNeedWs)) return rc;
  if (B <= 0 || Ci <= 0 || Co <= 0 || Ci > 64 || rows <= 0) return fail(COSKAD_ERR_ARG, "layer_train_fold: B=%d Ci=%d Co=%d rows=%d", B, Ci, Co, rows);
  const size_t E = 2 * ((size_t)Ci * Ci + Ci);
  if (ws_bytes < round_up((int)(E * sizeof(double)), 256)) return fail(COSKAD_ERR_WORKSPACE, "layer_train_fold: workspace %zu too small", ws_bytes);
  return launch_reduce_fold(partials, rows, reinterpret_cast<double*>(ws), (double)B * T * V, a.p, a.out, Ci, Co, stream);
}


int coskad_layer_train_moments_f32(const float* in, const float* A, const float* Tm, const float* in_slope, float* Z, double* sums,
                                   void* ws, size_t ws_bytes, int B, int Ci, int T, int V, hipStream_t stream) {
  const LayerStatsArgs a{.in = in, .A = A, .Tm = Tm, .in_slope = in_slope, .Zout = Z, .sums = sums, .ws = ws, .ws_bytes = ws_bytes,
                         .B = B, .Ci = Ci, .Co = Ci, .stream = stream};
  if (int rc = check_layer_stats("layer_train_moments", a, kNeedInput | kNeedSums | kNeedWs)) return rc;
  if (B <= 0 || Ci <= 0) return fail(COSKAD_ERR_ARG, "layer_train_moments: B=%d Ci=%d", B, Ci);
  if ((size_t)sums & 7) return fail(COSKAD_ERR_ARG, "layer_train_moments: sums must be 8-byte aligned");
  return dispatch_train_stats("layer_train_moments", a, T, V, false);
}

int coskad_layer_moment_sums_f32(const float* partials, int rows, int Ci, double* sums, hipStream_t stream) {
  if (!partials || !sums || rows <= 0 || Ci <= 0 || Ci > 64) return fail(COSKAD_ERR_ARG, "layer_moment_sums: bad argument");
  if ((size_t)sums & 7) return fail(COSKAD_ERR_ARG, "layer_moment_sums: sums must be 8-byte aligned");
  return launch_reduce_fold(partials, rows, sums, 0.0, BnConvParams{}, FoldOut{}, Ci, Ci, stream);
}

int coskad_layer_train_fold_sums_f32(const double* sums, double count, const float* Wt, const float* bt, const float* gamma_t,
                                     const float* beta_t, float* rmean_t, float* rvar_t, long long* nbt_t,
                                     const float* Wr, const float* br, const float* gamma_r,
                                     const float* beta_r, float* rmean_r, float* rvar_r, long long* nbt_r,
// ... 18 lines not shown
```

coskad_amd/engine.py:

```python
from __future__ import annotations

import os
from dataclasses import dataclass, field
from typing import Dict, List, Optional

import torch

from . import ops

Tensor = torch.Tensor


@dataclass
class LayerTensors:
    A: Tensor
    T: Tensor
    Wt: Tensor
    bt: Optional[Tensor]
    gt: Tensor
    bet: Tensor
    rm_t: Tensor
    rv_t: Tensor
    nbt_t: Tensor
    Wr: Optional[Tensor]
# ... 57 lines not shown

    def __init__(self) -> None:
        self.buf: Optional[Tensor] = None

    def get(self, nbytes: int, device) -> Tensor:
        if self.buf is None or self.buf.numel() < nbytes or self.buf.device != device:
            self.buf = torch.empty(int(nbytes), dtype=torch.uint8, device=device)
        return self.buf


@dataclass
class ChainCtx:
    inputs: List[Tensor] = field(default_factory=list)
    stats: List[Tensor] = field(default_factory=list)
    zs: List[Optional[Tensor]] = field(default_factory=list)
    in_slope: Optional[Tensor] = None
    sync: object = None
    sync_count: float = 0.0


EVAL_FIRST_PAIR = True
EVAL_WINDOW = True
EVAL_TAIL = True


def eval_fold(L: LayerTensors):
    key = L.fold_key() if L.cache is not None else None
    if key is not None and L.cache.get("key") == key:
        return L.cache["fold"]
    wb = ops.bn_fold(L.w2(L.Wt), L.bt, L.gt, L.bet, L.rm_t, L.rv_t, L.w2(L.Wr), L.br, L.gr, L.ber, L.rm_r, L.rv_r)
    if key is not None:
        L.cache["key"], L.cache["fold"] = key, wb
    return wb


def chain_forward(x: Tensor, layers: List[LayerTensors], training: bool, ws: Workspace,
                  in_slope: Optional[Tensor] = None, want_ctx: bool = False, sync=None, pending0=None):
    B, C, T, V = x.shape
    ctx = ChainCtx(in_slope=in_slope) if want_ctx else None
    sync_count = None
    batch_stats = [training or L.rm_t is None for L in layers]
    if sync is not None and training:
        import torch.distributed as dist
        if not STORE_Z:
            raise ValueError("SyncBN runs on the stored-Z training path")
        cnt = torch.tensor([float(B * T * V)], device=x.device, dtype=torch.float64)
        dist.all_reduce(cnt, group=sync)
        sync_count = float(cnt.item())
        if ctx is not None:
            ctx.sync, ctx.sync_count = sync, sync_count
    h, slope = x, in_slope
    n = len(layers)
    fuse = [False] * n
    ftab = None
    if all(batch_stats) and STORE_Z and FUSE_NEXT:
        for i in range(n - 1):
            fuse[i] = layers[i + 1].Ci == layers[i].Co and ops.layer_apply_next_ok(layers[i].Ci, layers[i].Co, T, V)
        nxt = [i + 1 for i in range(n - 1) if fuse[i]]
        if nxt:
            ftab = torch.empty(n, ops.ftab_floats(), device=x.device, dtype=torch.float32)
            for k in range(0, len(nxt), 4):
                grp = nxt[k:k + 4]
                ops.build_ftabs([layers[i].A for i in grp], [layers[i].T for i in grp], [ftab[i] for i in grp])
    fuse_flat = [False] * n
    if all(batch_stats) and STORE_Z and FUSE_NEXT and sync is None:
        for i in range(n - 1):
            fuse_flat[i] = (not fuse[i] and layers[i + 1].Ci == layers[i].Co and layers[i].Wr is not None
                            and ops.layer_apply_next_flat_ok(layers[i].Ci, layers[i].Co, T, V))
    skip = -1
    pending = pending0
    if pending0 is not None and not (batch_stats[0] and STORE_Z and sync is None):
        raise ValueError("chain_forward: pending0 is for the stored-Z training path without SyncBN")
    for i, L in enumerate(layers):
        if i == skip:
            continue
        if h.shape[1] != L.Ci:
            raise ValueError(f"layer expects {L.Ci} input channels, got {h.shape[1]}")
        Z = None
        if batch_stats[i]:
            if L.cache:
                L.cache.clear()
            buf = ws.get(ops.train_stats_ws_bytes(L.Ci), x.device)
            if sync_count is not None:
                if pending is not None:
                    Z, partials, rows = pending
                    sums = ops.layer_moment_sums(partials, rows, L.Ci)
                else:
                    Z = torch.empty_like(h)
                    sums = ops.layer_train_moments(h, L.A, L.T, slope, buf, Z=Z)
                dist.all_reduce(sums, group=sync)
                wfold, bias, stat = ops.layer_train_fold_sums(
                    sums, sync_count, L.w2(L.Wt), L.bt, L.gt, L.bet, L.rm_t, L.rv_t, L.nbt_t,
                    L.w2(L.Wr), L.br, L.gr, L.ber, L.rm_r, L.rv_r, L.nbt_r, momentum=L.step_momentum())
            elif pending is not None:
                Z, partials, rows = pending
                wfold, bias, stat = ops.layer_train_fold(
                    partials, rows, B, T, V, L.w2(L.Wt), L.bt, L.gt, L.bet, L.rm_t, L.rv_t, L.nbt_t,
                    L.w2(L.Wr), L.br, L.gr, L.ber, L.rm_r, L.rv_r, L.nbt_r, buf, momentum=L.step_momentum())
            else:
                if STORE_Z:
                    Z = torch.empty_like(h)
                wfold, bias, stat = ops.layer_train_stats(
                    h, L.A, L.T, slope, L.w2(L.Wt), L.bt, L.gt, L.bet, L.rm_t, L.rv_t, L.nbt_t,
                    L.w2(L.Wr), L.br, L.gr, L.ber, L.rm_r, L.rv_r, L.nbt_r, buf, momentum=L.step_momentum(), Z=Z)
        else:
            wfold, bias = eval_fold(L)
            stat = None
            if (EVAL_FIRST_PAIR and i == 0 and ctx is None and slope is None and n > 1 and not batch_stats[1] and layers[1].Ci == L.Co
                    and L.Wr is not None and wfold.shape[1] == L.Co
                    and ops.layer_first_pair_ok(L.Ci, L.Co, layers[1].Co, T, V)):
                N = layers[1]
                wf2, b2 = eval_fold(N)
                if wf2.shape[1] == N.Co:
                    h = ops.layer_first_pair_apply(h, L.A, L.T, wfold, bias, N.A, N.T, wf2, b2, L.Co, N.Co, L.slope)
                    slope, skip = N.slope, 1
                    continue
        pending = None
        if fuse[i]:
            rows_max = ops.layer_apply_next_rows(B, h.shape[1], L.Co)
            partials = torch.empty(rows_max * 2 * (L.Co * L.Co + L.Co), device=x.device, dtype=torch.float32)
            u, Zn, rows = ops.layer_apply_next(Z, h, wfold, bias, L.Co, slope, L.slope, ftab[i + 1], partials, T, V)
            pending = (Zn, partials, rows)
        elif fuse_flat[i] and Z is not None:
            u, Zn, partials, rows = ops.layer_apply_next_flat(Z, h, wfold, bias, L.Co, slope, L.slope, layers[i + 1].A, layers[i + 1].T)
            pending = (Zn, partials, rows)
        elif Z is not None:
            u = ops.layer_apply_z(Z, h, L.A, L.T, wfold, bias, L.Co, in_slope=slope)
        else:
            u = ops.layer_apply(h, L.A, L.T, wfold, bias, L.Co, in_slope=slope)
        if ctx is not None:
            ctx.inputs.append(h)
            ctx.stats.append(stat)
            ctx.zs.append(Z)
        h, slope = u, L.slope
    return h, ctx


STORE_Z = True
FUSE_BELOW = True
CHAIN_SKIP = frozenset()
FUSE_TOP = True
FUSE_NEXT = True


class SideStream:

    def __init__(self) -> None:
        self.stream: Optional[torch.cuda.Stream] = None
        self.dz = [None, None]
        self.ws = None
        self.done = [None, None]

    def ensure(self, nfloats: int, ws_bytes: int, device) -> None:
        if self.stream is None:
            self.stream = torch.cuda.Stream(device=device)
        for k in range(2):
            if self.dz[k] is None or self.dz[k].numel() < nfloats:
                self.dz[k] = torch.empty(nfloats, device=device, dtype=torch.float32)
        if self.ws is None or self.ws.numel() < ws_bytes:
            self.ws = torch.empty(ws_bytes, device=device, dtype=torch.uint8)


def btlnk_backward(ctx: Optional[ChainCtx], layers: List[LayerTensors], U: Tensor, W: Tensor, dz: Tensor, slope: Optional[Tensor],
                   dW: Tensor, db: Optional[Tensor], dslope: Optional[Tensor], ws: Workspace):
    B = U.shape[0]
    K, L = U.numel() // B, W.shape[0]
    i = len(layers) - 1 if layers else -1
    Z = ctx.zs[i] if (ctx is not None and ctx.zs and i >= 0) else None
    if (FUSE_TOP and Z is not None and U.dim() == 4 and layers[i].Wr is not None and L <= 16
            and ops.btlnk_bwd_chain_ok(K, U.shape[2] * U.shape[3], layers[i].Ci)):
        in_slope = layers[i - 1].slope if i > 0 else ctx.in_slope
        return ops.btlnk_bwd_chain(U, W, dz, slope, dW, db, dslope, ws, ctx.inputs[i], Z, in_slope)
    buf = ws.get(ops.btlnk_bwd_ws_bytes(B, K, L), U.device)
    return ops.btlnk_bwd(U, W, dz, slope, dW, db, dslope, buf), None


def chain_backward(ctx: ChainCtx, layers: List[LayerTensors], dU: Tensor, ws: Workspace,
                   grads: List[Dict[str, Tensor]], need_dx: bool, accumulate: bool = False,
                   side: Optional[SideStream] = None, stats_in=None, in_slope_grad: Optional[Tensor] = None) -> Optional[Tensor]:
    n = len(layers)
    if side is not None and stats_in is not None:
        raise ValueError("chain_backward: the side-stream path runs its own batch reductions (stats_in must be None)")
    if ctx.sync is not None and side is not None:
        raise ValueError("SyncBN runs on the main stream (side=None)")
    main = torch.cuda.current_stream() if side is not None else None
    if side is not None:
        side.done = [None, None]
    for i in range(n - 1, -1, -1):
        L = layers[i]
        x_in = ctx.inputs[i]
        B, Ci, T, V = x_in.shape
        in_slope = layers[i - 1].slope if i > 0 else ctx.in_slope
        g = dict(grads[i])
        g.pop("slope", None)
        if i > 0:
            g["slope_in"] = grads[i - 1]["slope"]
        elif in_slope_grad is not None and in_slope is not None:
            g["slope_in"] = in_slope_grad
        want_dx = need_dx or i > 0
        buf = ws.get(ops.layer_bwd_ws_bytes(B, Ci, L.Co, T, V), x_in.device)
        args = (x_in, dU, L.A, L.T, in_slope, ctx.stats[i], L.w2(L.Wt), L.gt, L.w2(L.Wr), L.gr, _as2d(g), buf)
        if side is None:
            sync = ctx.sync
            if sync is not None:
                import torch.distributed as dist
                if stats_in is None:
                    stats_in = ops.layer_bwd_stats(x_in, dU, L.A, L.T, in_slope, L.Wr is not None, buf, Z=ctx.zs[i])
                dist.all_reduce(ops.chain_sums(stats_in[0], stats_in[1], Ci, L.Co), group=sync)
            below = None
            Zi = ctx.zs[i] if ctx.zs else None
            if (FUSE_BELOW and i not in CHAIN_SKIP and Zi is not None and i > 0 and ctx.zs[i - 1] is not None
                    and in_slope is not None and layers[i - 1].Wr is not None):
                cb = ctx.inputs[i - 1].shape[1]
                rows = ops.layer_bwd_below_rows(B, Ci, L.Co, cb, T, V)
                if rows:
                    below = (ctx.inputs[i - 1], ctx.zs[i - 1], layers[i - 2].slope if i > 1 else ctx.in_slope,
                             torch.empty(ops.layer_bwd_below_floats(B, Ci, L.Co, cb, T, V), device=x_in.device, dtype=torch.float32))
            dIn = ops.layer_bwd(*args, need_dx=want_dx, accumulate=accumulate, Z=Zi,
                                stats_in=stats_in, below=below, stats_count=ctx.sync_count if sync is not None else 0.0)
            stats_in = (below[3], rows) if below is not None else None
        else:
            k = i & 1
            side.ensure(max(x.numel() for x in ctx.inputs), ops.layer_gcn_params_ws_bytes(T, V), x_in.device)
            if side.done[k] is not None:
                main.wait_event(side.done[k])
# ... 70 lines not shown
```

coskad_amd/ops.py:

```python
from __future__ import annotations

import ctypes
from typing import Optional

import torch

from . import _lib
from ._lib import call

Tensor = torch.Tensor


def _stream() -> ctypes.c_void_p:
    return ctypes.c_void_p(torch.cuda.current_stream().cuda_stream)


def _chk(t: Optional[Tensor], name: str, shape=None, dtype=torch.float32, optional=False) -> None:
    if t is None:
        if optional:
            return
        raise ValueError(f"{name}: tensor required")
    if not t.is_cuda:
        raise _lib.CoskadHipError(f"{name}: expected a CUDA (ROCm) tensor, got device {t.device}; "
                                  "the COSKAD hot path runs only on the HIP extension (no CPU fallback)")
# ... 92 lines not shown
               out: Optional[Tensor] = None, score: Optional[Tensor] = None):
    B, Ci, T, V = x_in.shape
    _chk(x_in, "x_in"); _chk(A, "A", (T, V, V)); _chk(Tm, "T", (V, T, T))
    _chk(wfold, "wfold", (2 * Ci, cop(Co))); _chk(bias, "bias", (cop(Co),))
    _chk(in_slope, "in_slope", (1,), optional=True); _chk(out_slope, "out_slope", (1,), optional=True)
    if not (want_out or want_score):
        raise ValueError("layer_tail: neither the reconstruction nor the score asked for")
    if want_score:
        _chk(x, "x", (B, Co, T, V))
        if score is None:
            score = torch.empty(B, device=x_in.device, dtype=torch.float32)
        else:
            _chk(score, "score", (B,))
    if want_out:
        if out is None:
            out = torch.empty(B, Co, T, V, device=x_in.device, dtype=torch.float32)
        else:
            _chk(out, "out", (B, Co, T, V))
    out, score = (out if want_out else None), (score if want_score else None)
    call("coskad_layer_tail_f32", x_in, x if want_score else None, out, score, A, Tm, wfold, bias, in_slope, out_slope, B, Ci, Co, T, V,
         _stream(), tag=(Ci, Co))
    return out, score


def layer_first_pair_ok(Ci: int, Cm: int, Co: int, T: int, V: int) -> bool:
    return bool(_lib.lib().coskad_layer_first_pair_ok(T, V, Ci, Cm, Co))


def layer_first_pair_apply(x: Tensor, A1: Tensor, T1: Tensor, wfold1: Tensor, bias1: Tensor, A2: Tensor, T2: Tensor, wfold2: Tensor,
                           bias2: Tensor, Cm: int, Co: int, mid_slope: Tensor, out_slope: Optional[Tensor] = None) -> Tensor:
    B, Ci, T, V = x.shape
    _chk(x, "x", (B, 2, T, V)); _chk(A1, "A1", (T, V, V)); _chk(T1, "T1", (V, T, T)); _chk(A2, "A2", (T, V, V)); _chk(T2, "T2", (V, T, T))
    _chk(wfold1, "wfold1", (4, Cm)); _chk(bias1, "bias1", (Cm,)); _chk(wfold2, "wfold2", (2 * Cm, Co)); _chk(bias2, "bias2", (Co,))
    _chk(mid_slope, "mid_slope", (1,)); _chk(out_slope, "out_slope", (1,), optional=True)
    out = torch.empty(B, Co, T, V, device=x.device, dtype=torch.float32)
    call("coskad_layer_first_pair_apply_f32", x, out, A1, T1, wfold1, bias1, A2, T2, wfold2, bias2, mid_slope, out_slope, B, Cm, Co, T, V,
         _stream())
    return out


def layer_fits(Ci: int, Co: int, T: int, V: int) -> bool:
    return bool(_lib.lib().coskad_layer_fits(Ci, Co, T, V))


def stat_floats(Ci: int, Co: int) -> int:
    return _lib.lib().coskad_stat_floats(Ci, Co)


def train_stats_ws_bytes(Ci: int) -> int:
    return _lib.lib().coskad_train_stats_ws_bytes(Ci)


def layer_train_stats(x, A, Tm, in_slope, Wt, bt, gt, bet, rm_t, rv_t, nbt_t,
                      Wr, br, gr, ber, rm_r, rv_r, nbt_r, ws, momentum: float = 0.1, Z: Optional[Tensor] = None):
    B, Ci, T, V = x.shape
    Co = Wt.shape[0]
    _chk(x, "x"); _chk(A, "A", (T, V, V)); _chk(Tm, "T", (V, T, T))
    _chk(Wt, "Wt", (Co, Ci)); _chk(gt, "gamma_t", (Co,)); _chk(bet, "beta_t", (Co,))
    for n, t in (("bt", bt), ("rm_t", rm_t), ("rv_t", rv_t), ("br", br), ("gamma_r", gr), ("beta_r", ber),
                 ("rm_r", rm_r), ("rv_r", rv_r)):
        _chk(t, n, (Co,), optional=True)
    _chk(Wr, "Wr", (Co, Ci), optional=True)
    _chk(in_slope, "in_slope", (1,), optional=True)
    _chk(nbt_t, "nbt_t", (), dtype=torch.int64, optional=True)
    _chk(nbt_r, "nbt_r", (), dtype=torch.int64, optional=True)
    need = train_stats_ws_bytes(Ci)
    if ws is None or ws.numel() * ws.element_size() < need:
        raise ValueError(f"workspace too small: need {need} bytes")
    wfold = torch.empty(2 * Ci, cop(Co), device=x.device, dtype=torch.float32)
    bias = torch.empty(cop(Co), device=x.device, dtype=torch.float32)
    stat = torch.empty(stat_floats(Ci, Co), device=x.device, dtype=torch.float32)
    _chk(Z, "Z", tuple(x.shape), optional=True)
    args = (x, A, Tm, in_slope, Wt, bt, gt, bet, rm_t, rv_t, nbt_t, Wr, br, gr, ber, rm_r, rv_r, nbt_r, momentum, wfold, bias, stat, ws,
            ws.numel() * ws.element_size(), B, Ci, Co, T, V, _stream())
    if Z is None:
        call("coskad_layer_train_stats_f32", *args)
    else:
        call("coskad_layer_train_stats_z_f32", *args, Z)
    return wfold, bias, stat


def layer_train_moments(x, A, Tm, in_slope, ws, Z: Optional[Tensor] = None) -> Tensor:
    B, Ci, T, V = x.shape
    _chk(x, "x"); _chk(A, "A", (T, V, V)); _chk(Tm, "T", (V, T, T)); _chk(in_slope, "in_slope", (1,), optional=True)
    _chk(Z, "Z", tuple(x.shape), optional=True)
    need = train_stats_ws_bytes(Ci)
    if ws is None or _bytes(ws) < need:
        raise ValueError(f"workspace too small: need {need} bytes")
    sums = torch.empty(2 * (Ci * Ci + Ci), device=x.device, dtype=torch.float64)
    call("coskad_layer_train_moments_f32", x, A, Tm, in_slope, Z, sums, ws, _bytes(ws), B, Ci, T, V, _stream())
    return sums


def layer_moment_sums(partials: Tensor, rows: int, Ci: int) -> Tensor:
    _chk(partials, "partials")
    if partials.numel() < rows * 2 * (Ci * Ci + Ci):
        raise ValueError("layer_moment_sums: partials smaller than rows x 2 (Ci^2 + Ci)")
    sums = torch.empty(2 * (Ci * Ci + Ci), device=partials.device, dtype=torch.float64)
    call("coskad_layer_moment_sums_f32", partials, rows, Ci, sums, _stream())
    return sums


def layer_train_fold_sums(sums, count, Wt, bt, gt, bet, rm_t, rv_t, nbt_t, Wr, br, gr, ber, rm_r, rv_r, nbt_r, momentum: float = 0.1):
    Co, Ci = Wt.shape
    _chk(sums, "sums", (2 * (Ci * Ci + Ci),), dtype=torch.float64); _chk(Wt, "Wt", (Co, Ci)); _chk(gt, "gamma_t", (Co,)); _chk(bet, "beta_t", (Co,))
    for n, t in (("bt", bt), ("rm_t", rm_t), ("rv_t", rv_t), ("br", br), ("gamma_r", gr), ("beta_r", ber), ("rm_r", rm_r), ("rv_r", rv_r)):
        _chk(t, n, (Co,), optional=True)
    _chk(Wr, "Wr", (Co, Ci), optional=True)
    _chk(nbt_t, "nbt_t", (), dtype=torch.int64, optional=True); _chk(nbt_r, "nbt_r", (), dtype=torch.int64, optional=True)
    wfold = torch.empty(2 * Ci, cop(Co), device=Wt.device, dtype=torch.float32)
    bias = torch.empty(cop(Co), device=Wt.device, dtype=torch.float32)
    stat = torch.empty(stat_floats(Ci, Co), device=Wt.device, dtype=torch.float32)
    call("coskad_layer_train_fold_sums_f32", sums, float(count), Wt, bt, gt, bet, rm_t, rv_t, nbt_t, Wr, br, gr, ber, rm_r, rv_r, nbt_r,
         momentum, wfold, bias, stat, Ci, Co, _stream())
    return wfold, bias, stat


def layer_bwd_stats(x_in, dU, A, Tm, in_slope, has_residual: bool, ws, Z=None):
    B, Ci, T, V = x_in.shape
    Co = dU.shape[1]
    _chk(x_in, "x_in"); _chk(dU, "dU", (B, Co, T, V)); _chk(A, "A", (T, V, V)); _chk(Tm, "T", (V, T, T))
    _chk(in_slope, "in_slope", (1,), optional=True); _chk(Z, "Z", (B, Ci, T, V), optional=True)
    need = layer_bwd_ws_bytes(B, Ci, Co, T, V)
    if ws is None or _bytes(ws) < need:
        raise ValueError(f"workspace too small: need {need} bytes")
    buf = torch.empty(_lib.lib().coskad_layer_bwd_stats_floats(B, Ci, Co, T, V), device=x_in.device, dtype=torch.float32)
    rows = ctypes.c_int(0)
    call("coskad_layer_bwd_stats_f32", x_in, dU, A, Tm, in_slope, 1 if has_residual else 0, buf, _bytes(buf), ctypes.byref(rows), ws,
         _bytes(ws), B, Ci, Co, T, V, _stream(), Z)
    return buf, rows.value


# ... 180 lines not shown
    Co = Wt.shape[0]
    _chk(x_in, "x_in"); _chk(dU, "dU", (B, Co, T, V)); _chk(A, "A", (T, V, V)); _chk(Tm, "T", (V, T, T))
    _chk(Wt, "Wt", (Co, Ci)); _chk(gt, "gamma_t", (Co,)); _chk(stat, "stat", (stat_floats(Ci, Co),))
    _chk(Wr, "Wr", (Co, Ci), optional=True); _chk(gr, "gamma_r", (Co,), optional=True)
    _chk(in_slope, "in_slope", (1,), optional=True); _chk(dZ, "dZ", (B, Ci, T, V)); _chk(Z, "Z", (B, Ci, T, V), optional=True)
    for k, shp in (("Wt", (Co, Ci)), ("gt", (Co,)), ("bet", (Co,))):
        _chk(grads[k], "grad " + k, shp)
    for k, shp in (("bt", (Co,)), ("Wr", (Co, Ci)), ("br", (Co,)), ("gr", (Co,)), ("ber", (Co,)), ("slope_in", (1,))):
        _chk(grads.get(k), "grad " + k, shp, optional=True)
    need = layer_bwd_ws_bytes(B, Ci, Co, T, V)
    if ws is None or _bytes(ws) < need:
        raise ValueError(f"workspace too small: need {need} bytes")
    if need_dx and dIn is None:
        dIn = torch.empty_like(x_in)
    call("coskad_layer_bwd_data_f32", x_in, dU, A, Tm, in_slope, stat, Wt, gt, Wr, gr, dIn if need_dx else None, dZ, grads["Wt"],
         grads.get("bt"), grads["gt"], grads["bet"], grads.get("Wr"), grads.get("br"), grads.get("gr"), grads.get("ber"),
         grads.get("slope_in"), ws, _bytes(ws), 1 if accumulate else 0, B, Ci, Co, T, V, _stream(), Z)
    return dIn if need_dx else None


def layer_gcn_params_ws_bytes(T, V) -> int:
    return _lib.lib().coskad_layer_gcn_params_ws_bytes(T, V)


def layer_gcn_params(x_in, in_slope, dZ, A, Tm, dA, dT, ws, accumulate=False):
    B, Ci, T, V = x_in.shape
    _chk(x_in, "x_in"); _chk(dZ, "dZ", (B, Ci, T, V)); _chk(A, "A", (T, V, V)); _chk(Tm, "T", (V, T, T))
    _chk(dA, "dA", (T, V, V)); _chk(dT, "dT", (V, T, T)); _chk(in_slope, "in_slope", (1,), optional=True)
    if ws is None or _bytes(ws) < layer_gcn_params_ws_bytes(T, V):
        raise ValueError("workspace too small")
    call("coskad_layer_gcn_params_f32", x_in, in_slope, dZ, A, Tm, dA, dT, ws, _bytes(ws), 1 if accumulate else 0, B, Ci, T, V, _stream())


def btlnk_fwd(U: Tensor, W: Tensor, bias: Optional[Tensor], slope: Optional[Tensor], ws=None) -> Tensor:
    B = U.shape[0]
    K = U.numel() // B
    L = W.shape[0]
    _chk(U, "U"); _chk(W, "W", (L, K)); _chk(bias, "bias", (L,), optional=True); _chk(slope, "slope", (1,), optional=True)
    z = torch.empty(B, L, device=U.device, dtype=torch.float32)
    if L > 16:
        nbytes = _lib.lib().coskad_btlnk_fwd_ws_bytes_l(B, K, L)
        buf = ws.get(nbytes, U.device) if ws is not None else torch.empty(nbytes, dtype=torch.uint8, device=U.device)
        call("coskad_btlnk_fwd_ws_f32", U, W, bias, slope, z, buf, nbytes, B, K, L, _stream())
        return z
    if B >= BTLNK_SPLITK_MIN_B and K % 16 == 0:
        nbytes = _lib.lib().coskad_btlnk_fwd_ws_bytes(B)
        buf = ws.get(nbytes, U.device) if ws is not None else torch.empty(nbytes, dtype=torch.uint8, device=U.device)
        call("coskad_btlnk_fwd_ws_f32", U, W, bias, slope, z, buf, nbytes, B, K, L, _stream())
        return z
    call("coskad_btlnk_fwd_f32", U, W, bias, slope, z, B, K, L, _stream())
    return z


BTLNK_SPLITK_MIN_B = 1
BTLNK_LMAX = 512


def btlnk_bwd_ws_bytes(B, K, L) -> int:
    return _lib.lib().coskad_btlnk_bwd_ws_bytes(B, K, L)


def btlnk_bwd(U, W, dz, slope, dW, db, dslope, ws, dU=None, accumulate=False):
    B = U.shape[0]
    K = U.numel() // B
    L = W.shape[0]
    _chk(U, "U"); _chk(W, "W", (L, K)); _chk(dz, "dz", (B, L)); _chk(dW, "dW", (L, K))
    _chk(db, "db", (L,), optional=True); _chk(dslope, "dslope", (1,), optional=True); _chk(slope, "slope", (1,), optional=True)
    need = btlnk_bwd_ws_bytes(B, K, L)
    if ws is None or _bytes(ws) < need:
        raise ValueError(f"workspace too small: need {need} bytes")
    if dU is None:
        dU = torch.empty_like(U)
    call("coskad_btlnk_bwd_f32", U, W, dz, slope, dU, dW, db, dslope, ws, _bytes(ws), 1 if accumulate else 0, B, K, L, _stream())
    return dU


def btlnk_bwd_chain_ok(K: int, TV: int, below_Ci: int) -> bool:
    return bool(_lib.lib().coskad_btlnk_bwd_chain_ok(K, TV, below_Ci))


def btlnk_bwd_chain(U, W, dz, slope, dW, db, dslope, ws, below_in, below_Z, below_in_slope, dU=None, accumulate=False):
    B, Ch, T, V = U.shape
    TV = T * V
    K = Ch * TV
    L = W.shape[0]
    Ci = below_in.shape[1]
    _chk(U, "U"); _chk(W, "W", (L, K)); _chk(dz, "dz", (B, L)); _chk(dW, "dW", (L, K))
    _chk(db, "db", (L,), optional=True); _chk(dslope, "dslope", (1,), optional=True); _chk(slope, "slope", (1,), optional=True)
    _chk(below_in, "below_in", (B, Ci, T, V)); _chk(below_Z, "below_Z", (B, Ci, T, V)); _chk(below_in_slope, "below_in_slope", (1,), optional=True)
    if not btlnk_bwd_chain_ok(K, TV, Ci):
        raise ValueError(f"btlnk_bwd_chain: shape K={K} TV={TV} Ci={Ci} not supported")
    lib = _lib.lib()
    need = lib.coskad_btlnk_bwd_chain_ws_bytes(B, K, L, TV)
    buf = ws.get(need, U.device)
    stats = torch.empty(lib.coskad_btlnk_bwd_chain_floats(B, TV, Ci), device=U.device, dtype=torch.float32)
    if dU is None:
        dU = torch.empty_like(U)
    rows = ctypes.c_int(0)
    call("coskad_btlnk_bwd_chain_f32", U, W, dz, slope, dU, dW, db, dslope, buf, _bytes(buf), 1 if accumulate else 0, B, K, L, below_in,
         below_Z, below_in_slope, Ci, TV, stats, _bytes(stats), ctypes.byref(rows), _stream())
    return dU, (stats, rows.value)


def _cuda_f32(t: Tensor, name: str) -> None:
    if not t.is_cuda:
        raise _lib.CoskadHipError(f"{name}: expected a CUDA (ROCm) tensor, got device {t.device}; no CPU fallback")
    if t.dtype != torch.float32:
        raise TypeError(f"{name}: expected float32, got {t.dtype}")


def _b3(t: Tensor):
    if t.dim() == 2:
        return 1, t.shape[0], t.shape[1], 0, t.stride(0), t.stride(1)
    if t.dim() == 3:
        return t.shape[0], t.shape[1], t.shape[2], t.stride(0), t.stride(1), t.stride(2)
    raise ValueError("gemm operands are 2-D or 3-D")


def gemm(A: Tensor, B: Tensor, out: Optional[Tensor] = None, bias: Optional[Tensor] = None, bias_mode: int = 0,
         bias_mod: int = 1, relu: bool = False, accumulate: bool = False) -> Tensor:
    _cuda_f32(A, "A"); _cuda_f32(B, "B")
    ba, M, K, sab, sam, sak = _b3(A)
    bb, K2, N, sbb, sbk, sbn = _b3(B)
    if K != K2:
        raise ValueError(f"gemm: inner sizes differ ({K} vs {K2})")
    batch = max(ba, bb)
    if ba not in (1, batch) or bb not in (1, batch):
        raise ValueError("gemm: batch sizes do not broadcast")
    if ba == 1:
        sab = 0
    if bb == 1:
        sbb = 0
    if out is None:
        out = torch.empty((batch, M, N) if (A.dim() == 3 or B.dim() == 3) else (M, N), device=A.device, dtype=torch.float32)
    _cuda_f32(out, "out")
    bc, Mc, Nc, scb, scm, scn = _b3(out)
    if (Mc, Nc) != (M, N) or bc != batch:
        raise ValueError(f"gemm: out has shape {tuple(out.shape)}, expected batch {batch} x {M} x {N}")
    _chk(bias, "bias", optional=True)
    call("coskad_gemm_f32", A, B, out, bias, sab, sam, sak, sbb, sbk, sbn, scb, scm, scn, M, N, K, batch, bias_mode, bias_mod,
         1 if relu else 0, 0, 0, 0, 1 if accumulate else 0, _stream())
    return out


def gemm_reduce(A: Tensor, B: Tensor, out: Tensor, target_chunks: int = 64, ktotal: int = 0, accumulate: bool = False) -> Tensor:
    _cuda_f32(A, "A"); _cuda_f32(B, "B"); _chk(out, "out")
    ba, M, K, sab, sam, sak = _b3(A)
    bb, K2, N, sbb, sbk, sbn = _b3(B)
    if K != K2 or ba != bb or tuple(out.shape) != (M, N):
        raise ValueError("gemm_reduce: shape mismatch")
    chunk = max(1, (ba + target_chunks - 1) // target_chunks)
# ... 215 lines not shown
    L = W2.shape[0]
    _chk(y1, "y1"); _chk(gamma, "gamma", (H,)); _chk(beta, "beta", (H,)); _chk(W2, "W2", (L, H)); _chk(b2, "b2", (L,), optional=True)
    _chk(running_mean, "running_mean", (H,), optional=True); _chk(running_var, "running_var", (H,), optional=True)
    _chk(nbt, "num_batches_tracked", (), dtype=torch.int64, optional=True)
    z = torch.empty(B, L, device=y1.device, dtype=torch.float32)
    stat = torch.empty(mlp_head_ws_floats(B, H, L), device=y1.device, dtype=torch.float32)
    call("coskad_mlp_head_fwd_f32", y1, gamma, beta, running_mean, running_var, nbt, momentum, eps, 1 if training else 0, W2, b2, z, stat,
         B, H, L, _stream())
    return z, stat


def mlp_head_bwd(y1, stat, gamma, beta, W2, dz, grads: dict, training: bool, accumulate: bool = False):
    B, H = y1.shape
    L = W2.shape[0]
    _chk(y1, "y1"); _chk(stat, "stat"); _chk(gamma, "gamma", (H,)); _chk(beta, "beta", (H,)); _chk(W2, "W2", (L, H))
    if stat.numel() < 2 * H:
        raise ValueError("mlp_head_bwd: stat holds fewer than 2 H values")
    _chk(dz, "dz", (B, L)); _chk(grads["gamma"], "dgamma", (H,)); _chk(grads["beta"], "dbeta", (H,)); _chk(grads["W2"], "dW2", (L, H))
    _chk(grads.get("b2"), "db2", (L,), optional=True)
    dy1 = torch.empty_like(y1)
    red = torch.empty(mlp_head_ws_floats(B, H, L), device=y1.device, dtype=torch.float32)
    call("coskad_mlp_head_bwd_f32", y1, stat, gamma, beta, W2, dz, dy1, grads["gamma"], grads["beta"], grads["W2"], grads.get("b2"), red,
         1 if training else 0, 1 if accumulate else 0, B, H, L, _stream())
    return dy1


HEAD_SLOTS = 19


def head_slots(L: int) -> int:
    if not 0 < L <= BTLNK_LMAX:
        raise ValueError(f"latent_dim={L}: the head kernels take 1 .. {BTLNK_LMAX}")
    return max(L, 16) + 3


def head_count_slot(L: int) -> int:
    return max(L, 16) + 1


def head_ws(B: int, device, L: int = 16) -> Tensor:
    return torch.empty(_lib.lib().coskad_head_ws_floats_l(B, L), device=device, dtype=torch.float32)


def mse_head(z, c, need_grad=True, need_score=False, acc=None, upstream=1.0, ws=None):
    B, L = z.shape
    S = head_slots(L)
    _chk(z, "z"); _chk(c, "c", (L,)); _chk(acc, "acc", (S,), optional=True)
    ws = head_ws(B, z.device, L) if ws is None else ws
    dz = torch.empty_like(z) if need_grad else None
    score = torch.empty(B, device=z.device, dtype=torch.float32) if need_score else None
    stats = torch.empty(S, device=z.device, dtype=torch.float32)
    call("coskad_mse_head_f32", z, c, dz, score, stats, acc, upstream, ws, B, L, _stream())
    return stats, dz, score


def mahalanobis_head(z, c, VI, need_grad=True, need_score=False, acc=None, gram=None, gram_accumulate=True,
                     upstream=1.0, ws=None):
    B, L = z.shape
    S = head_slots(L)
    _chk(z, "z"); _chk(c, "c", (L,)); _chk(VI, "VI", (L, L)); _chk(acc, "acc", (S,), optional=True)
    _chk(gram, "gram", (L, L), optional=True)
    ws = head_ws(B, z.device, L) if ws is None else ws
    dz = torch.empty_like(z) if need_grad else None
    score = torch.empty(B, device=z.device, dtype=torch.float32) if need_score else None
    stats = torch.empty(S, device=z.device, dtype=torch.float32)
    call("coskad_mahalanobis_head_f32", z, c, VI, dz, score, stats, acc, gram, int(gram_accumulate), upstream, ws, B, L, _stream())
    return stats, dz, score


def poincare_head(z, c, need_grad=True, need_zh=False, need_score=False, acc=None, upstream=1.0, ws=None):
    B, L = z.shape
    S = head_slots(L)
    _chk(z, "z"); _chk(c, "c", (L,), optional=True); _chk(acc, "acc", (S,), optional=True)
    ws = head_ws(B, z.device, L) if ws is None else ws
    dz = torch.empty_like(z) if (need_grad and c is not None) else None
    zh = torch.empty_like(z) if need_zh else None
    score = torch.empty(B, device=z.device, dtype=torch.float32) if (need_score and c is not None) else None
    stats = torch.empty(S, device=z.device, dtype=torch.float32)
    call("coskad_poincare_head_f32", z, c, dz, zh, score, stats, acc, upstream, ws, B, L, _stream())
    return stats, dz, zh, score


def poincare_dist(zh, c):
    B, L = zh.shape
    _chk(zh, "zh"); _chk(c, "c", (L,))
    score = torch.empty(B, device=zh.device, dtype=torch.float32)
    call("coskad_poincare_dist_f32", zh, c, score, B, L, _stream())
    return score


def poincare_logmap0(y):
    B, L = y.shape
    _chk(y, "y")
    out = torch.empty_like(y)
    call("coskad_poincare_logmap0_f32", y, out, B, L, _stream())
    return out


def lowrank_fold_ok(latent: int, TV: int) -> bool:
    return bool(_lib.lib().coskad_lowrank_fold_ok(latent, TV))


def lowrank_fold_fwd(X: Tensor, G: Tensor, bn_t, bn_r, bias_t, bias_r, n_pos: float):
    R, K, Co, TV = X.shape
    _chk(X, "X", (2, 9, Co, TV)); _chk(G, "G", (9, 9), dtype=torch.float64)
    dev = X.device
# ... 322 lines not shown
```

coskad_amd/trainer.py:

```python
from __future__ import annotations

from typing import Dict, List, Optional

import torch
import torch.distributed as dist

from . import engine, ops, parallel
from .models.graph_layers.stsgcn import layer_tensors

Tensor = torch.Tensor


class FlatParams:

    def __init__(self, module: torch.nn.Module) -> None:
        named = [(n, p) for n, p in module.named_parameters()]
        self.names = [n for n, _ in named]
        al = lambda k: (k + 3) // 4 * 4
        total = sum(al(p.numel()) for _, p in named)
        dev = named[0][1].device
        self.flat = torch.zeros(total, device=dev, dtype=torch.float32)
        self.grad = torch.zeros(total, device=dev, dtype=torch.float32)
        self.reg_mask = torch.zeros(total, device=dev, dtype=torch.float32)
        self.views: Dict[str, Tensor] = {}
# ... 472 lines not shown
        from .models.common.components import MLP
        self.mlp = isinstance(model.btlnk, MLP)
        if not isinstance(model, STSE) or not (isinstance(model.btlnk, torch.nn.Linear) or (self.mlp and model.btlnk.hip_ok)):
            raise TypeError("STSETrainStep drives an STSE with projector='linear' or an 'mlp' within the kernels' widths")
        super().__init__(model, lr, alpha, betas, eps, process_group)
        self.head = head
        dev = self.fp.flat.device
        self.hyper = torch.tensor([lr, 1.0, 1.0, 0.0], device=dev, dtype=torch.float32)
        L = model.latent_dim
        self.center_acc = torch.zeros(ops.head_slots(L), device=dev, dtype=torch.float32)
        self.gram_acc = torch.zeros(L, L, device=dev, dtype=torch.float32) if head == 'mahalanobis' else None
        plain_gcn = _is_plain_gcn(model.encoder)
        wide = plain_gcn or any(l.is_wide for l in model.encoder.model)
        if plain_gcn and (side_stream or use_graph):
            raise ValueError("a plain-GCN encoder runs on the main stream, outside hipGraph capture")
        if wide and (side_stream or use_graph):
            raise ValueError("an encoder with wide layers runs on the main stream, outside hipGraph capture")
        self.side = engine.SideStream() if side_stream else None
        self.sync_group = None
        if sync_bn and self.world > 1:
            if self.mlp or side_stream or use_graph or wide:
                raise ValueError("sync_bn: encoder BatchNorm only (STS-GCN encoder within the tile kernels, linear projector), on the "
                                 "main stream, outside hipGraph capture")
            self.sync_group = process_group if process_group is not None else dist.group.WORLD
        if plain_gcn:
            self.stack = _PlainGCNStack(model.encoder, self.fp)
        else:
            plain = not wide and (use_graph or side_stream or sync_bn or not any(_is_commute(l) for l in model.encoder.model))
            self.stack = _FlatStack(list(model.encoder.model), self.fp, "encoder.model.", plain=plain, side=self.side,
                                    sync=self.sync_group, window=fused_window)
        names = self.fp.names
        first_tail = next((i for i, n in enumerate(names) if n.startswith("btlnk.")), None)
        tail = first_tail is not None and all(n.startswith("btlnk.") for n in names[first_tail:])
        self.tail_off = self.fp.offsets[names[first_tail]] if tail else None
        if use_graph and any(isinstance(b, torch.nn.modules.batchnorm._BatchNorm) and b.momentum is None for b in model.modules()):
            raise ValueError("use_graph: BatchNorm with momentum=None changes its averaging factor every step (a launch argument here); "
                             "capture needs a fixed momentum")
        self.use_graph = use_graph
        self._graph = self._x_static = self._stats_static = None

    @property
    def layers(self) -> List[engine.LayerTensors]:
        segs = self.stack.segs
        return segs[0].layers if len(segs) == 1 and segs[0].kind == 'tile' else []

    def set_lr(self, lr: float) -> None:
        self.hyper[0] = lr
        self.lr = float(lr)

    def _body(self, x: Tensor) -> Tensor:
        m, gv = self.model, self.fp.gviews
        U, slope, saved_stack = self.stack.forward(x, self.ws)
        ctx, top_layers = self.stack.top(saved_stack)
        if self.mlp:
            wname, W = "btlnk.net.0.", m.btlnk.net[0].weight
            z, saved = self._mlp_forward(U, slope)
        else:
            wname, W = "btlnk.", m.btlnk.weight
            z = ops.btlnk_fwd(U, W, m.btlnk.bias, slope, ws=self.ws)
        stats, dz = self._head(z)
        if self.mlp:
            dz = self._mlp_backward(saved, dz)
        dU, top_stats = engine.btlnk_backward(ctx if self.side is None else None, top_layers or [], U, W, dz, slope, gv[wname + "weight"],
                                              gv.get(wname + "bias"), self.stack.last_slope_grad, self.ws)
        work = None
        if self.world > 1 and self.tail_off is not None:
            work = dist.all_reduce(self.fp.grad[self.tail_off:], group=self.pg, async_op=True)
        self.stack.backward(saved_stack, dU, self.ws, need_dx=False, top_stats=top_stats)
        if self.world > 1:
            head = self.fp.grad if work is None else self.fp.grad[:self.tail_off]
            dist.all_reduce(head, group=self.pg)
            if work is not None:
                work.wait()
        self._adam()
        return stats

    def step(self, x: Tensor) -> Tensor:
        self.steps += 1
        x = x.contiguous()
        if not self.use_graph:
            return self._body(x)
        if self._graph is None or self._x_static.shape != x.shape:
            self._x_static = x.clone()
            s = torch.cuda.Stream()
            s.wait_stream(torch.cuda.current_stream())
            with torch.cuda.stream(s):
                self._body(self._x_static)
            torch.cuda.current_stream().wait_stream(s)
            self.steps += 1
            self._graph = torch.cuda.CUDAGraph()
            with torch.cuda.graph(self._graph):
                self._stats_static = self._body(self._x_static)
        self._x_static.copy_(x)
        self._graph.replay()
        return self._stats_static


class STSAETrainStep(_FlatStep):

    def __init__(self, model, mode: str = 'ae', lr: float = 1e-4, alpha: float = 0.0, lambda_: float = 0.01, phi: float = 1.0,
                 beta: float = 1.0, gamma: float = 1.0, betas=(0.9, 0.999), eps: float = 1e-8, process_group=None,
                 fused_window: bool = False) -> None:
        from .models.sts.ae import STSAE
        from .models.sts.vae import STSVAE
        from .models.common.components import Encoder
        if not isinstance(model, STSAE) or not isinstance(model.encoder, Encoder):
            raise TypeError("STSAETrainStep drives an STSAE / STSVAE with the STS-GCN encoder")
        if mode not in ('ae', 'vae') or (mode == 'vae') != isinstance(model, STSVAE):
            raise ValueError(f"mode {mode!r} does not fit {type(model).__name__}")
        if not self.supports(model):
            raise TypeError("STSAETrainStep: projector / latent size outside the bottleneck kernels (latent rows <= 16, "
                            "'linear' projector)")
        super().__init__(model, lr, alpha, betas, eps, process_group)
        self.mode = mode
        self.lambda_, self.phi, self.beta, self.gamma = float(lambda_), float(phi), float(beta), float(gamma)
        self.enc = _FlatStack(list(model.encoder.model), self.fp, "encoder.model.", window=fused_window)
        from . import lowrank
# ... 221 lines not shown
```

include/coskad_hip.h:

```cpp
#ifndef COSKAD_HIP_H
#define COSKAD_HIP_H
#include <hip/hip_runtime_api.h>

#ifdef __cplusplus
extern "C" {
#endif

int coskad_abi_version(void);
const char* coskad_last_error(void);

int coskad_probe_begin(int kernel, int Ci, int Co);
int coskad_probe_stride(int n);
int coskad_probe_end(float* avg_ms, int* launches);


int coskad_window_ok(int T, int V);

int coskad_gcn_f32(const float* in, float* out, const float* A, const float* Tm, int rows, int T, int V,
                   int adjoint, hipStream_t stream);

int coskad_bn_fold_f32(const float* Wt, const float* bt, const float* gamma_t, const float* beta_t,
                       const float* mean_t, const float* var_t, const float* Wr, const float* br,
                       const float* gamma_r, const float* beta_r, const float* mean_r,
                       const float* var_r, float* wfold, float* bias, int Ci, int Co,
                       hipStream_t stream);

int coskad_layer_apply_window_ok(int T, int V, int Ci, int Co);
int coskad_layer_apply_f32(const float* in, float* out, const float* A, const float* Tm,
                           const float* wfold, const float* bias, const float* in_slope,
                           const float* out_slope, int B, int Ci, int Co, int T, int V,
                           hipStream_t stream);

int coskad_layer_tail_ok(int T, int V, int Ci, int Co);
int coskad_layer_tail_max_grid(int T, int V, int Ci);
int coskad_layer_tail_f32(const float* in, const float* x, float* out, float* score,
                          const float* A, const float* Tm, const float* wfold, const float* bias,
                          const float* in_slope, const float* out_slope,
                          int B, int Ci, int Co, int T, int V, hipStream_t stream);

int coskad_prelu_fwd_f32(const float* u, const float* slope, float* out, size_t n, hipStream_t stream);
int coskad_prelu_bwd_f32(const float* u, const float* dout, const float* slope, float* du, float* dslope,
                         float* ws, int accumulate, size_t n, hipStream_t stream);

int coskad_rec_head_f32(const float* U, const float* x, const float* slope, float* xrec, float* dU, float* loss, float* dslope,
                        float upstream, float* ws, int accumulate, size_t n, hipStream_t stream);

size_t coskad_rev_btlnk_ws_floats(int B, int N, int L);
int coskad_rev_btlnk_fwd_f32(const float* z, const float* W, const float* bias, float* H, int B, int N, int L, hipStream_t stream);
int coskad_rev_btlnk_bwd_f32(const float* dH, const float* z, const float* W, float* dz, int dz_accumulate, float* dW, float* db,
                             int accumulate, float* ws, int B, int N, int L, hipStream_t stream);


size_t coskad_train_stats_ws_bytes(int Ci);
int coskad_stat_floats(int Ci, int Co);

int coskad_layer_train_stats_f32(const float* in, const float* A, const float* Tm, const float* in_slope,
                                 const float* Wt, const float* bt, const float* gamma_t,
                                 const float* beta_t, float* rmean_t, float* rvar_t, long long* nbt_t,
                                 const float* Wr, const float* br, const float* gamma_r,
                                 const float* beta_r, float* rmean_r, float* rvar_r, long long* nbt_r,
                                 float momentum, float* wfold, float* bias, float* stat, void* ws,
                                 size_t ws_bytes, int B, int Ci, int Co, int T, int V,
                                 hipStream_t stream);

int coskad_layer_train_window_ok(int T, int V, int Ci, int Co);

int coskad_layer_train_window_narrow_ok(int T, int V, int Ci, int Co);

int coskad_layer_train_stats_z_f32(const float* in, const float* A, const float* Tm, const float* in_slope,
                                   const float* Wt, const float* bt, const float* gamma_t,
                                   const float* beta_t, float* rmean_t, float* rvar_t, long long* nbt_t,
                                   const float* Wr, const float* br, const float* gamma_r,
                                   const float* beta_r, float* rmean_r, float* rvar_r, long long* nbt_r,
                                   float momentum, float* wfold, float* bias, float* stat, void* ws,
                                   size_t ws_bytes, int B, int Ci, int Co, int T, int V,
                                   hipStream_t stream, float* Z);
int coskad_layer_apply_z_f32(const float* Z, const float* in, float* out, const float* A, const float* Tm,
                             const float* wfold, const float* bias, const float* in_slope, const float* out_slope,
                             int B, int Ci, int Co, int T, int V, hipStream_t stream);

int coskad_layer_apply_next_ok(int Ci, int Co, int T, int V);
int coskad_ftab_floats(void);
int coskad_layer_apply_next_rows(int B, int Ci, int Co);
int coskad_build_ftab_f32(const float* const* A, const float* const* Tm, float* const* tab, int n, int T, int V,
                          hipStream_t stream);
int coskad_layer_apply_next_f32(const float* Z, const float* in, float* out, const float* wfold, const float* bias,
                                const float* in_slope, const float* out_slope, const float* ftab_next, float* Z_next,
                                float* partials, size_t partials_bytes, int B, int Ci, int Co, int T, int V,
                                hipStream_t stream);
int coskad_layer_train_fold_f32(const float* partials, int rows, const float* Wt, const float* bt, const float* gamma_t,
                                const float* beta_t, float* rmean_t, float* rvar_t, long long* nbt_t,
                                const float* Wr, const float* br, const float* gamma_r,
                                const float* beta_r, float* rmean_r, float* rvar_r, long long* nbt_r,
                                float momentum, float* wfold, float* bias, float* stat, void* ws,
                                size_t ws_bytes, int B, int Ci, int Co, int T, int V, hipStream_t stream);

int coskad_gather_f32(const float* src, const int* idx, float* out, size_t n, hipStream_t stream);
int coskad_fused_encoder_out_floats(void);
int coskad_fused_encoder_f32(const float* x, float* out, const float* tab, const float* wreg, const float* slopes, int B,
                             int T, int V, hipStream_t stream);

int coskad_gemm_f32(const float* A, const float* B, float* C, const float* bias, long long sa_b, long long sa_m,
                    long long sa_k, long long sb_b, long long sb_k, long long sb_n, long long sc_b, long long sc_m,
                    long long sc_n, int M, int N, int K, int batch, int bias_mode, int bias_mod, int relu, int reduce,
                    int chunk, long long ktotal, int accum, hipStream_t stream);
int coskad_gemm_sum_f32(const float* partials, int chunks, size_t E, float* out, int accumulate, hipStream_t stream);
int coskad_relu_bwd_f32(const float* out, const float* dout, float* g, float* part, int Nb, int C, int P, int slices,
                        hipStream_t stream);
int coskad_softmax_rows_f32(const float* x, float* y, int n, hipStream_t stream);
int coskad_softmax_rows_bwd_f32(const float* y, const float* dy, float* dx, int n, hipStream_t stream);

int coskad_plain_gcn_ok(int Ci, int Co, int P);
size_t coskad_plain_gcn_ws_bytes(int B, int Ci, int Co, int P, int grid_cap);
int coskad_plain_gcn_fwd_f32(const float* X, const float* W, const float* Ap, const float* bias, float* O, float* save, int B,
                             int Ci, int Co, int P, int grid_cap, hipStream_t stream);
int coskad_plain_gcn_bwd_f32(const float* X, const float* S, const float* O, const float* dO, const float* W, const float* Ap,
                             float* dX, float* dW, float* db, float* D, void* ws, size_t ws_bytes, int B, int Ci, int Co, int P,
                             int need_dx, int need_da, int accumulate, int grid_cap, hipStream_t stream);

int coskad_conv1x1_ok(int M, int K, int P);
int coskad_conv1x1_stat_rows(int M, int K, int P, int batch);
int coskad_conv1x1_f32(const float* A, long long sa_m, long long sa_k, const float* In, float* Out, const float* bias, double* stats,
                       int M, int K, int P, int batch, int accumulate, hipStream_t stream);
int coskad_bn2_stats_parts_f32(const double* parts, int rows, float* stat, float* running_mean, float* running_var,
                               long long* num_batches_tracked, float momentum, float eps, double count, int C, hipStream_t stream);
int coskad_conv1x1_wgrad_ok(int M, int K, int P);
int coskad_conv1x1_wgrad_f32(const float* G, const float* X, float* partials, int M, int K, int P, int batch, int chunk,
                             hipStream_t stream);

// ... 44 lines not shown
int coskad_layer_train_fold_sums_f32(const double* sums, double count, const float* Wt, const float* bt, const float* gamma_t,
                                     const float* beta_t, float* rmean_t, float* rvar_t, long long* nbt_t,
                                     const float* Wr, const float* br, const float* gamma_r,
                                     const float* beta_r, float* rmean_r, float* rvar_r, long long* nbt_r,
                                     float momentum, float* wfold, float* bias, float* stat, int Ci, int Co, hipStream_t stream);
size_t coskad_layer_bwd_stats_floats(int B, int Ci, int Co, int T, int V);
size_t coskad_layer_bwd_sums_offset(int rows, int Ci, int Co);
int coskad_layer_bwd_stats_f32(const float* in, const float* dU, const float* A, const float* Tm, const float* in_slope,
                               int has_residual, float* stats_out, size_t stats_out_bytes, int* rows_out, void* ws, size_t ws_bytes,
                               int B, int Ci, int Co, int T, int V, hipStream_t stream, const float* Z);

int coskad_layer_bwd_f32(const float* in, const float* dU, const float* A, const float* Tm,
                         const float* in_slope, const float* stat, const float* Wt, const float* gamma_t,
                         const float* Wr, const float* gamma_r, float* dIn, float* dA, float* dT, float* dWt,
                         float* dbt, float* dgamma_t, float* dbeta_t, float* dWr, float* dbr,
                         float* dgamma_r, float* dbeta_r, float* dslope_in, void* ws, size_t ws_bytes,
                         int accumulate, int B, int Ci, int Co, int T, int V, hipStream_t stream);

int coskad_layer_bwd_z_f32(const float* in, const float* dU, const float* A, const float* Tm,
                           const float* in_slope, const float* stat, const float* Wt, const float* gamma_t,
                           const float* Wr, const float* gamma_r, float* dIn, float* dA, float* dT, float* dWt,
                           float* dbt, float* dgamma_t, float* dbeta_t, float* dWr, float* dbr,
                           float* dgamma_r, float* dbeta_r, float* dslope_in, void* ws, size_t ws_bytes,
                           int accumulate, int B, int Ci, int Co, int T, int V, hipStream_t stream, const float* Z);

int coskad_layer_bwd_data_f32(const float* in, const float* dU, const float* A, const float* Tm,
                              const float* in_slope, const float* stat, const float* Wt, const float* gamma_t,
                              const float* Wr, const float* gamma_r, float* dIn, float* dZ, float* dWt, float* dbt,
                              float* dgamma_t, float* dbeta_t, float* dWr, float* dbr, float* dgamma_r,
                              float* dbeta_r, float* dslope_in, void* ws, size_t ws_bytes, int accumulate, int B,
                              int Ci, int Co, int T, int V, hipStream_t stream, const float* Z );
size_t coskad_layer_gcn_params_ws_bytes(int T, int V);
int coskad_layer_gcn_params_f32(const float* in, const float* in_slope, const float* dZ, const float* A,
                                const float* Tm, float* dA, float* dT, void* ws, size_t ws_bytes, int accumulate,
                                int B, int Ci, int T, int V, hipStream_t stream);

size_t coskad_gcn_bwd_params_ws_bytes(int T, int V);
int coskad_gcn_bwd_params_f32(const float* x, const float* dZ, const float* A, const float* Tm, float* dA,
                              float* dT, void* ws, size_t ws_bytes, int accumulate, int rows, int T, int V,
                              hipStream_t stream);

int coskad_gcn_bwd_params_dx_f32(const float* x, const float* dZ, const float* A, const float* Tm, float* dA, float* dT,
                                 float* dX, const float* dX_add, void* ws, size_t ws_bytes, int accumulate, int rows, int T,
                                 int V, hipStream_t stream);


int coskad_btlnk_fwd_f32(const float* U, const float* W, const float* bias, const float* slope, float* z,
                         int B, int K, int L, hipStream_t stream);

size_t coskad_btlnk_fwd_ws_bytes(int B);
size_t coskad_btlnk_fwd_ws_bytes_l(int B, int K, int L);
int coskad_btlnk_fwd_ws_f32(const float* U, const float* W, const float* bias, const float* slope, float* z, void* ws,
                            size_t ws_bytes, int B, int K, int L, hipStream_t stream);
size_t coskad_btlnk_bwd_ws_bytes(int B, int K, int L);
int coskad_btlnk_bwd_f32(const float* U, const float* W, const float* dz, const float* slope, float* dU,
                         float* dW, float* db, float* dslope, void* ws, size_t ws_bytes, int accumulate,
                         int B, int K, int L, hipStream_t stream);

int coskad_btlnk_bwd_chain_ok(int K, int TV, int below_Ci);
int coskad_btlnk_bwd_chain_rows(int B, int TV);
size_t coskad_btlnk_bwd_chain_floats(int B, int TV, int below_Ci);
size_t coskad_btlnk_bwd_chain_ws_bytes(int B, int K, int L, int TV);
int coskad_btlnk_bwd_chain_f32(const float* U, const float* W, const float* dz, const float* slope, float* dU, float* dW,
                               float* db, float* dslope, void* ws, size_t ws_bytes, int accumulate, int B, int K, int L,
                               const float* below_in, const float* below_Z, const float* below_in_slope, int below_Ci, int TV,
                               float* stats_out, size_t stats_out_bytes, int* stats_rows, hipStream_t stream);


int coskad_gather_transform_f32(const float* xy, const long long* index, const float* mats, float* out, int B, int N,
                                int ntrans, int TV, hipStream_t stream);


int coskad_head_slots(void);
size_t coskad_head_ws_floats(int B);
int coskad_head_slots_l(int L);
size_t coskad_head_ws_floats_l(int B, int L);

int coskad_mse_head_f32(const float* z, const float* c, float* dz, float* score, float* stats, float* acc,
                        float upstream, float* ws, int B, int L, hipStream_t stream);

int coskad_mahalanobis_head_f32(const float* z, const float* c, const float* VI, float* dz, float* score,
                                float* stats, float* acc, float* gram, int gram_accumulate, float upstream,
                                float* ws, int B, int L, hipStream_t stream);

int coskad_poincare_head_f32(const float* z, const float* c, float* dz, float* zh, float* score,
                             float* stats, float* acc, float upstream, float* ws, int B, int L,
                             hipStream_t stream);
int coskad_poincare_dist_f32(const float* zh, const float* c, float* score, int B, int L, hipStream_t stream);
int coskad_poincare_logmap0_f32(const float* y, float* out, int B, int L, hipStream_t stream);

int coskad_lowrank_fold_ok(int latent, int TV);
int coskad_lowrank_fold_fwd_f32(const float* X, const double* G, const float* gamma0, const float* beta0, const float* cbias0,
                                float* rmean0, float* rvar0, long long* nbt0, float momentum0, float eps0, const float* gamma1,
                                const float* beta1, const float* cbias1, float* rmean1, float* rvar1, long long* nbt1, float momentum1,
                                float eps1, double n_pos, float* Mw, float* Mb, double* saved, double* xbar, double* xx, int Co, int TV,
                                hipStream_t stream);
int coskad_lowrank_fold_bwd_f32(const float* X, const double* G, const float* dMw, const float* dMb, const double* saved,
                                const double* xbar, const double* xx, const float* gamma0, const float* gamma1, double n_pos, float* dX,
                                float* dgamma, float* dbeta, double* dGc, int Co, int TV, hipStream_t stream);

int coskad_narrow_conv_rows(int B, int TV);
int coskad_narrow_conv_fwd_f32(const float* U, const float* in_slope, const float* W, float* out, int B, int Ci, int J, int TV,
                               hipStream_t stream);
int coskad_narrow_conv_bwd_f32(const float* U, const float* in_slope, const float* W, const float* dOut, float* dU, float* partials,
                               size_t partials_floats, int B, int Ci, int J, int TV, hipStream_t stream);

int coskad_layer_apply_next_flat_ok(int Ci, int Co, int T, int V);
int coskad_layer_apply_next_flat_rows(int B);
int coskad_layer_apply_next_flat_f32(const float* Z, const float* in, float* out, const float* wfold, const float* bias,
                                     const float* in_slope, const float* out_slope, const float* A_next, const float* T_next,
                                     float* Z_next, float* partials, size_t partials_bytes, int B, int Ci, int Co, int T, int V,
                                     hipStream_t stream);

int coskad_layer_first_pair_ok(int T, int V, int Ci, int Cm, int Co);
int coskad_layer_first_pair_apply_f32(const float* x, float* out, const float* A1, const float* T1, const float* wfold1, const float* bias1,
                                      const float* A2, const float* T2, const float* wfold2, const float* bias2, const float* mid_slope,
                                      const float* out_slope, int B, int Cm, int Co, int T, int V, hipStream_t stream);

int coskad_commute_ok(int T, int V, int Ci, int Co);
size_t coskad_commute_ws_floats(int B, int T, int V);
int coskad_commute_fwd_f32(const float* u_prev, const float* in_slope, const float* wt, const float* wr, const float* A, const float* Tm,
                           const float* gamma_t, const float* beta_t, const float* gamma_r, const float* beta_r, const float* bias_t,
                           const float* bias_r, float* rm_t, float* rv_t, float* rm_r, float* rv_r, long long* nbt_t, long long* nbt_r,
                           float momentum, float eps, float* YR, float* Zy, float* U, float* stat, float* ws, size_t ws_floats,
                           const float* A_next, const float* T_next, const float* slope_out, float* Z_next, float* partials_next,
                           int* rows_next, int B, int T, int V, hipStream_t stream);
int coskad_commute_bwd_f32(const float* u_prev, const float* in_slope, const float* wt, const float* wr, const float* A, const float* Tm,
                           const float* YR, const float* Zy, const float* stat, const float* dU, float* d_in, float* dA, float* dT,
                           float* dWt, float* dWr, float* dgamma_t, float* dbeta_t, float* dgamma_r, float* dbeta_r, float* dslope,
                           float* ws, size_t ws_floats, const float* below_x, const float* below_z, float* below_stats,
                           size_t below_stats_floats, int B, int T, int V, hipStream_t stream);
int coskad_commute_below_rows(int B);
// ... 31 lines not shown
```

Before: 2.984 million clips/s.

## Fuse bottleneck slab sum into MSE head and piggyback launches on existing kernels

The bottleneck forward now writes split-K slabs that a new fused kernel sums while computing the euclidean MSE head. The head's final column reduction is deferred and rides as an extra block on the bottleneck backward reduce kernel. The operand-table build rides as extra blocks on the first-layer moments kernel, which also prefetches clip inputs into registers. The aim is to remove several small kernel launches and a round trip of z through memory, at the cost of more complex grid dispatch and extra register pressure. A launch counter is also added to the launch macro.

```diff
diff --git a/coskad_amd/csrc/api.hip b/coskad_amd/csrc/api.hip
--- a/coskad_amd/csrc/api.hip
+++ b/coskad_amd/csrc/api.hip
@@ -16,6 +16,8 @@
   va_end(ap);
   return code;
 }
+
+unsigned long long g_launch_count = 0;
 
 int check_launch(const char* what) {
   hipError_t e = hipGetLastError();
@@ -87,5 +89,6 @@
 }
 
 int coskad_abi_version(void) { return COSKAD_ABI_VERSION; }
+unsigned long long coskad_launch_count(void) { return coskad::g_launch_count; }
 const char* coskad_last_error(void) { return coskad::err_buf(); }
 }
diff --git a/coskad_amd/csrc/bottleneck.hip b/coskad_amd/csrc/bottleneck.hip
--- a/coskad_amd/csrc/bottleneck.hip
+++ b/coskad_amd/csrc/bottleneck.hip
@@ -1,5 +1,6 @@
 #include "tile_ops.h"
 #include "layer_launch.h"
+#include "heads_common.h"
 
 namespace coskad {
 
@@ -230,9 +231,13 @@
                                                        const float* __restrict__ dap, int nda,
                                                        float* __restrict__ dslope, int accumulate,
                                                        const float* __restrict__ rows, int RP, int RE,
-                                                       double* __restrict__ rsum) {
+                                                       double* __restrict__ rsum, HeadPending head) {
   __shared__ double sh[256];
   const unsigned nE = (unsigned)((E + 255) / 256);
+  if (head.partials && blockIdx.x == gridDim.x - 1) {
+    head_finalize_columns(head.partials, head.P, head.scale0, head.stats, head.acc);
+    return;
+  }
   if (blockIdx.x > nE + L) {
     const int col = threadIdx.x & 15, slice = threadIdx.x >> 4;
     const int e = (int)(blockIdx.x - (nE + L + 1)) * 16 + col;
@@ -307,10 +312,10 @@
 
 int launch_btlnk_reduce(const float* partials, int P, size_t E, float* out, const float* dz, int B, int L, float* db,
                         const float* dap, int nda, float* dslope, int accumulate, hipStream_t stream, const float* rows,
-                        int RP, int RE, double* rsum) {
-  const unsigned extra = rows ? (unsigned)ceil_div(RE, 16) : 0u;
+                        int RP, int RE, double* rsum, const HeadPending& head) {
+  const unsigned extra = (rows ? (unsigned)ceil_div(RE, 16) : 0u) + (head.partials ? 1u : 0u);
   hipLaunchKernelGGL(k_btlnk_reduce, dim3((unsigned)((E + 255) / 256) + L + 1 + extra), dim3(256), 0, stream, partials, P, E, out, dz,
-                     B, L, db, dap, nda, dslope, accumulate, rows, RP, RE, rsum);
+                     B, L, db, dap, nda, dslope, accumulate, rows, RP, RE, rsum, head);
   return check_launch("btlnk_bwd_reduce");
 }
 
@@ -356,6 +361,19 @@
   if ((rc = check_launch("btlnk_fwd_t"))) return rc;
   hipLaunchKernelGGL(k_btlnk_fwd_sum, dim3(ceil_div(B * 16, 256)), dim3(256), 0, stream, part, bias, z, B, L, kBtlKS);
   return check_launch("btlnk_fwd_sum");
+}
+
+int coskad_btlnk_fwd_slabs_ks(void) { return kBtlKS; }
+int coskad_btlnk_fwd_slabs_f32(const float* U, const float* W, const float* slope, void* ws, size_t ws_bytes, int B, int K, int L,
+                               hipStream_t stream) {
+  if (!U || !W || !ws) return fail(COSKAD_ERR_ARG, "btlnk_fwd_slabs: null pointer");
+  if (B <= 0 || K <= 0 || L <= 0) return fail(COSKAD_ERR_ARG, "btlnk_fwd_slabs: B=%d K=%d L=%d", B, K, L);
+  if (L > 16) return fail(COSKAD_ERR_SHAPE, "btlnk_fwd_slabs: latent_dim=%d > 16 not supported", L);
+  if (K % 16) return fail(COSKAD_ERR_SHAPE, "btlnk_fwd_slabs: K=%d must be a multiple of 16", K);
+  if ((size_t)ws & 15) return fail(COSKAD_ERR_ARG, "btlnk_fwd_slabs: ws must be 16-byte aligned");
+  if (ws_bytes < coskad_btlnk_fwd_ws_bytes(B)) return fail(COSKAD_ERR_WORKSPACE, "btlnk_fwd_slabs: workspace too small");
+  hipLaunchKernelGGL(k_btlnk_fwd_t, dim3(ceil_div(B, 64), kBtlKS), dim3(256), 0, stream, U, W, slope, reinterpret_cast<float*>(ws), B, K, L);
+  return check_launch("btlnk_fwd_t");
 }
 
 size_t coskad_btlnk_bwd_ws_bytes(int B, int K, int L) {
diff --git a/coskad_amd/csrc/btlnk_chain.hip b/coskad_amd/csrc/btlnk_chain.hip
--- a/coskad_amd/csrc/btlnk_chain.hip
+++ b/coskad_amd/csrc/btlnk_chain.hip
@@ -250,6 +250,8 @@
 
 using namespace coskad;
 
+extern "C" int coskad_head_finalize_pending(int B);
+
 extern "C" {
 
 int coskad_btlnk_bwd_chain_ok(int K, int TV, int below_Ci) {
@@ -273,10 +275,10 @@
   return ((size_t)p.S * L * K + (size_t)p.S * p.npt + 64) * sizeof(float);
 }
 
-int coskad_btlnk_bwd_chain_f32(const float* U, const float* W, const float* dz, const float* slope, float* dU, float* dW,
-                               float* db, float* dslope, void* ws, size_t ws_bytes, int accumulate, int B, int K, int L,
-                               const float* below_in, const float* below_Z, const float* below_in_slope, int below_Ci, int TV,
-                               float* stats_out, size_t stats_out_bytes, int* stats_rows, hipStream_t stream) {
+static int btlnk_bwd_chain(const float* U, const float* W, const float* dz, const float* slope, float* dU, float* dW,
+                          float* db, float* dslope, void* ws, size_t ws_bytes, int accumulate, int B, int K, int L,
+                          const float* below_in, const float* below_Z, const float* below_in_slope, int below_Ci, int TV,
+                          float* stats_out, size_t stats_out_bytes, int* stats_rows, hipStream_t stream, const HeadPending& head) {
   if (!U || !W || !dz || !dU || !dW || !ws || !below_in || !below_Z || !stats_out || !stats_rows)
     return fail(COSKAD_ERR_ARG, "btlnk_bwd_chain: null pointer");
   if (B <= 0 || K <= 0 || L <= 0) return fail(COSKAD_ERR_ARG, "btlnk_bwd_chain: B=%d K=%d L=%d", B, K, L);
@@ -311,7 +313,27 @@
   if ((rc = check_launch("btlnk_bwd_stats"))) return rc;
   *stats_rows = rows;
   return launch_btlnk_reduce(dWp, p.S, (size_t)L * K, dW, dz, B, L, db, dap, rows, (dslope && slope) ? dslope : nullptr, accumulate, stream,
-                             stats_out, rows, E, reinterpret_cast<double*>(stats_out + bc::sums_offset(rows, E)));
-}
-
-}
+                             stats_out, rows, E, reinterpret_cast<double*>(stats_out + bc::sums_offset(rows, E)), head);
+}
+
+int coskad_btlnk_bwd_chain_f32(const float* U, const float* W, const float* dz, const float* slope, float* dU, float* dW,
+                               float* db, float* dslope, void* ws, size_t ws_bytes, int accumulate, int B, int K, int L,
+                               const float* below_in, const float* below_Z, const float* below_in_slope, int below_Ci, int TV,
+                               float* stats_out, size_t stats_out_bytes, int* stats_rows, hipStream_t stream) {
+  return btlnk_bwd_chain(U, W, dz, slope, dU, dW, db, dslope, ws, ws_bytes, accumulate, B, K, L, below_in, below_Z, below_in_slope,
+                         below_Ci, TV, stats_out, stats_out_bytes, stats_rows, stream, HeadPending{});
+}
+
+int coskad_btlnk_bwd_chain_head_f32(const float* U, const float* W, const float* dz, const float* slope, float* dU, float* dW,
+                                    float* db, float* dslope, void* ws, size_t ws_bytes, int accumulate, int B, int K, int L,
+                                    const float* below_in, const float* below_Z, const float* below_in_slope, int below_Ci, int TV,
+                                    float* stats_out, size_t stats_out_bytes, int* stats_rows, const float* head_ws,
+                                    float head_scale0, float* head_stats, float* head_acc, hipStream_t stream) {
+  HeadPending head;
+  const int P = coskad_head_finalize_pending(B);
+  if (head_ws && P > 0 && (head_stats || head_acc)) head = HeadPending{head_ws, P, head_scale0, head_stats, head_acc};
+  return btlnk_bwd_chain(U, W, dz, slope, dU, dW, db, dslope, ws, ws_bytes, accumulate, B, K, L, below_in, below_Z, below_in_slope,
+                         below_Ci, TV, stats_out, stats_out_bytes, stats_rows, stream, head);
+}
+
+}
diff --git a/coskad_amd/csrc/common.h b/coskad_amd/csrc/common.h
--- a/coskad_amd/csrc/common.h
+++ b/coskad_amd/csrc/common.h
@@ -5,6 +5,16 @@
 #include <cstring>
 
 #define COSKAD_ABI_VERSION 1
+
+namespace coskad {
+extern unsigned long long g_launch_count;
+}
+#undef hipLaunchKernelGGL
+#define hipLaunchKernelGGL(kernelName, ...)                       \
+  do {                                                            \
+    ++coskad::g_launch_count;                                     \
+    hipLaunchKernelGGLInternal((kernelName), __VA_ARGS__);        \
+  } while (0)
 
 #define COSKAD_OK 0
 #define COSKAD_ERR_ARG (-1)
diff --git a/coskad_amd/csrc/first_layer.hip b/coskad_amd/csrc/first_layer.hip
--- a/coskad_amd/csrc/first_layer.hip
+++ b/coskad_amd/csrc/first_layer.hip
@@ -1,4 +1,5 @@
 #include "mfma_ops.h"
+#include "fused_ops.h"
 #include "layer_launch.h"
 
 namespace coskad {
@@ -196,20 +197,43 @@
 
 
 constexpr int NWM = 8;
+constexpr int kFtabBlocks = (ff::LAYER_F4 * 4 + 64 * NWM - 1) / (64 * NWM);
 template <int T, int V, int CI>
 __global__ __launch_bounds__(64 * NWM, 4) void k_first_moments(const float* __restrict__ in, const float* __restrict__ Aw,
                                                           const float* __restrict__ Tw, const float* __restrict__ in_slope,
-                                                          float* __restrict__ partials, int B, float* __restrict__ Zout) {
+                                                          float* __restrict__ partials, int B, float* __restrict__ Zout, int nmom,
+                                                          FtabArgs ftab) {
   constexpr int TV = T * V, NA = T * V * V, NT = V * T * T, KP = (TV + 63) / 64;
+  const int tid = threadIdx.x, lane = tid & 63;
+  if constexpr (T == ff::T && V == ff::V) {
+    if ((int)blockIdx.x >= nmom) {
+      const int b = uniform((int)blockIdx.x - nmom), layer = b / kFtabBlocks;
+      const int e = (b - layer * kFtabBlocks) * (64 * NWM) + tid;
+      if (e < ff::LAYER_F4 * 4) ftab.tab[layer][e] = ff::ftab_value(ftab.A[layer], ftab.Tm[layer], e);
+      return;
+    }
+  }
   extern __shared__ __attribute__((aligned(16))) float lds[];
   float* AwL = lds;
   float* TwL = AwL + NA;
-  const int tid = threadIdx.x, lane = tid & 63;
   const int wave = uniform(tid >> 6);
   float* Xl = TwL + NT + wave * 2 * CI * TV;
   float* Yl = Xl + CI * TV;
   const bool pre = in_slope != nullptr;
   const float a_in = pre ? in_slope[0] : 0.f;
+  float xr[KP][CI];
+  auto load_clip = [&](int r) {
+    const int clip = (r * nmom + blockIdx.x) * NWM + wave;
+    const bool live = clip < B;
+    const float* gx = in + (size_t)(live ? clip : 0) * CI * TV;
+#pragma unroll
+    for (int k = 0; k < KP; ++k) {
+      const int p = lane + 64 * k;
+#pragma unroll
+      for (int c = 0; c < CI; ++c) xr[k][c] = (live && p < TV) ? gx[c * TV + p] : 0.f;
+    }
+  };
+  load_clip(0);
   for (int e = tid; e < NA; e += 64 * NWM) AwL[e] = Aw[e];
   for (int e = tid; e < NT; e += 64 * NWM) {
     const int v = e / (T * T), tq = e - v * T * T;
@@ -223,11 +247,11 @@
     for (int b = 0; b < CI; ++b) { mx[a][b] = 0.f; mz[a][b] = 0.f; }
   }
   __syncthreads();
-  const int rounds = (B + gridDim.x * NWM - 1) / (gridDim.x * NWM);
+  const int rounds = (B + nmom * NWM - 1) / (nmom * NWM);
   for (int r = 0; r < rounds; ++r) {
-    const int clip = (r * gridDim.x + blockIdx.x) * NWM + wave;
+    const int clip = (r * nmom + blockIdx.x) * NWM + wave;
     const bool live = clip < B;
-    const float* gx = in + (size_t)(live ? clip : 0) * CI * TV;
+    if (r > 0) load_clip(r);
 #pragma unroll
     for (int k = 0; k < KP; ++k) {
       const int p = lane + 64 * k;
@@ -235,7 +259,7 @@
         float x[CI];
 #pragma unroll
         for (int c = 0; c < CI; ++c) {
-          x[c] = live ? act(gx[c * TV + p], pre, a_in) : 0.f;
+          x[c] = act(xr[k][c], pre, a_in);
           Xl[c * TV + p] = x[c];
           sx[c] += x[c];
         }
@@ -413,17 +437,24 @@
 
 template <int T, int V>
 static int launch_first_moments_tv(const float* in, const float* Aw, const float* Tw, const float* in_slope, float* partials, int B,
-                                   int Ci, float* Zout, int max_rows, hipStream_t st, int* rows_out) {
+                                   int Ci, float* Zout, int max_rows, hipStream_t st, int* rows_out, const FtabArgs* ftab) {
   int grid = (B + fl::NWM - 1) / fl::NWM;
   if (grid > 512) grid = 512;
   if (grid > max_rows) grid = max_rows;
   *rows_out = grid;
+  FtabArgs fa{};
+  int riders = 0;
+  if (ftab && ftab->n > 0) {
+    if (T != ff::T || V != ff::V || ftab->n > 4) return fail(COSKAD_ERR_SHAPE, "first_moments: operand tables ride at T=12, V=17, 1..4 layers");
+    fa = *ftab;
+    riders = fa.n * fl::kFtabBlocks;
+  }
   const size_t lds = ((size_t)T * V * V + (size_t)V * T * T + 2 * fl::NWM * (size_t)Ci * T * V) * sizeof(float);
 #define LAUNCH_FM(CI)                                                                                                   \
   do {                                                                                                                  \
     auto k = fl::k_first_moments<T, V, CI>;                                                                             \
     if (lds > 64 * 1024) (void)hipFuncSetAttribute((const void*)k, hipFuncAttributeMaxDynamicSharedMemorySize, (int)lds); \
-    hipLaunchKernelGGL(k, dim3(grid), dim3(64 * fl::NWM), lds, st, in, Aw, Tw, in_slope, partials, B, Zout);                    \
+    hipLaunchKernelGGL(k, dim3(grid + riders), dim3(64 * fl::NWM), lds, st, in, Aw, Tw, in_slope, partials, B, Zout, grid, fa);   \
   } while (0)
   {
     ProbeScope probe(KID_FWD_MOMENTS, Ci, 0, st);
@@ -437,8 +468,8 @@
 }
 
 int launch_first_moments(const float* in, const float* Aw, const float* Tw, const float* in_slope, float* partials, int B, int Ci,
-                         int T, int V, float* Zout, int max_rows, hipStream_t st, int* rows_out) {
-#define CALL(T_, V_) return launch_first_moments_tv<T_, V_>(in, Aw, Tw, in_slope, partials, B, Ci, Zout, max_rows, st, rows_out)
+                         int T, int V, float* Zout, int max_rows, hipStream_t st, int* rows_out, const FtabArgs* ftab) {
+#define CALL(T_, V_) return launch_first_moments_tv<T_, V_>(in, Aw, Tw, in_slope, partials, B, Ci, Zout, max_rows, st, rows_out, ftab)
   COSKAD_DISPATCH_TV(T, V, CALL);
 #undef CALL
 }
diff --git a/coskad_amd/csrc/fused_apply_next.hip b/coskad_amd/csrc/fused_apply_next.hip
--- a/coskad_amd/csrc/fused_apply_next.hip
+++ b/coskad_amd/csrc/fused_apply_next.hip
@@ -10,30 +10,11 @@
 
 using namespace ff;
 
-struct FtabArgs {
-  const float* A[4];
-  const float* Tm[4];
-  float* tab[4];
-};
 __global__ void k_build_ftab(FtabArgs args) {
   const int layer = blockIdx.y;
-  const float* __restrict__ Aw = args.A[layer];
-  const float* __restrict__ Tw = args.Tm[layer];
   const int e = blockIdx.x * blockDim.x + threadIdx.x;
   if (e >= LAYER_F4 * 4) return;
-  float val = 0.f;
-  if (e < TEMP_F4 * 4) {
-    const int v = e / 256, l = (e >> 2) & 63, s = e & 3, j = l & 15, q = l >> 4;
-    if (s < 3 && j < T) val = Tw[v * T * T + (4 * s + q) * T + j];
-  } else {
-    const int r = e - TEMP_F4 * 4;
-    const int t = r / (3 * 256), c = (r / 256) % 3, l = (r >> 2) & 63, k = 4 * c + (r & 3), j = l & 15, q = l >> 4;
-    if (k < 10) {
-      const int s = k < 5 ? k : k - 5, w = 4 * s + q;
-      if (w < V) val = Aw[t * V * V + w * V + (k < 5 ? j : 16)];
-    }
-  }
-  args.tab[layer][e] = val;
+  args.tab[layer][e] = ftab_value(args.A[layer], args.Tm[layer], e);
 }
 
 template <int CT, int OTP>
@@ -342,7 +323,8 @@
 
 int launch_build_ftab(const float* const* A, const float* const* Tm, float* const* tab, int n, hipStream_t st) {
   if (n < 1 || n > 4) return fail(COSKAD_ERR_ARG, "build_ftab: 1..4 layers per launch, got %d", n);
-  fn::FtabArgs args{};
+  FtabArgs args{};
+  args.n = n;
   for (int i = 0; i < n; ++i) {
     if (!A[i] || !Tm[i] || !tab[i]) return fail(COSKAD_ERR_ARG, "build_ftab: null pointer (layer %d)", i);
     args.A[i] = A[i]; args.Tm[i] = Tm[i]; args.tab[i] = tab[i];
diff --git a/coskad_amd/csrc/fused_ops.h b/coskad_amd/csrc/fused_ops.h
--- a/coskad_amd/csrc/fused_ops.h
+++ b/coskad_amd/csrc/fused_ops.h
@@ -32,6 +32,22 @@
 constexpr int KP = NTILE * 4 * 64 * 4;
 constexpr int TEMP_F4 = V * 64;
 constexpr int LAYER_F4 = TEMP_F4 + T * 3 * 64;
+__device__ __forceinline__ float ftab_value(const float* __restrict__ Aw, const float* __restrict__ Tw, int e) {
+  float val = 0.f;
+  if (e < TEMP_F4 * 4) {
+    const int v = e / 256, l = (e >> 2) & 63, s = e & 3, j = l & 15, q = l >> 4;
+    if (s < 3 && j < T) val = Tw[v * T * T + (4 * s + q) * T + j];
+  } else {
+    const int r = e - TEMP_F4 * 4;
+    const int t = r / (3 * 256), c = (r / 256) % 3, l = (r >> 2) & 63, k = 4 * c + (r & 3), j = l & 15, q = l >> 4;
+    if (k < 10) {
+      const int s = k < 5 ? k : k - 5, w = 4 * s + q;
+      if (w < V) val = Aw[t * V * V + w * V + (k < 5 ? j : 16)];
+    }
+  }
+  return val;
+}
+
 enum { W1A = 0, W1B = 2, WP = 4, WR = 12, WX3 = 20, WZ3 = 28, WZ4 = 36, WX4 = 68, B1 = 100, B2 = 108, B3 = 112, B4 = 120, NWREG = 136 };
 
 __device__ __forceinline__ f32x4 mfma(float a, float b, f32x4 c) {
diff --git a/coskad_amd/csrc/heads.hip b/coskad_amd/csrc/heads.hip
--- a/coskad_amd/csrc/heads.hip
+++ b/coskad_amd/csrc/heads.hip
@@ -17,6 +17,11 @@
 #pragma unroll
   for (int j = 0; j < LMAX; ++j)
     if (j < L) p[j] = a.v[j];
+}
+__device__ __forceinline__ void store_vec4(float* p, const Vec& a, int L) {
+#pragma unroll
+  for (int q = 0; q < LMAX / 4; ++q)
+    if (4 * q < L) reinterpret_cast<float4*>(p)[q] = float4{a.v[4 * q], a.v[4 * q + 1], a.v[4 * q + 2], a.v[4 * q + 3]};
 }
 __device__ __forceinline__ float dot(const Vec& a, const Vec& b) {
   float s = 0.f;
@@ -139,14 +144,23 @@
                                                     float* __restrict__ dz, float* __restrict__ score,
                                                     float* __restrict__ partials, int B, int L,
                                                     float gscale, float scale0, float* __restrict__ stats,
-                                                    float* __restrict__ acc) {
+                                                    float* __restrict__ acc, const float* __restrict__ part,
+                                                    const float* __restrict__ zbias, int KS, float* __restrict__ zout) {
   float vals[kHeadSlots];
 #pragma unroll
   for (int k = 0; k < kHeadSlots; ++k) vals[k] = 0.f;
   const Vec c = load_vec(cvec, L);
+  const bool v4 = (L & 3) == 0 && (((size_t)dz | (size_t)zout) & 15) == 0;
 #pragma unroll 4
   for (int n = blockIdx.x * kFlatBlock + threadIdx.x; n < B; n += gridDim.x * kFlatBlock) {
-    const Vec u = load_vec(z + (size_t)n * L, L);
+    Vec u;
+    if (part) {
+      load_z_row_from_slabs(part, zbias, KS, B, n, L, u.v);
+      if (v4) store_vec4(zout + (size_t)n * L, u, L);
+      else store_vec(zout + (size_t)n * L, u, L);
+    } else {
+      u = load_vec(z + (size_t)n * L, L);
+    }
     Vec g;
     float sq = 0.f;
 #pragma unroll
@@ -159,7 +173,10 @@
     vals[0] += sq;
     vals[LMAX + 1] += 1.f;
     vals[LMAX + 2] += sqrtf(dot(u, u));
-    if (dz) store_vec(dz + (size_t)n * L, g, L);
+    if (dz) {
+      if (v4) store_vec4(dz + (size_t)n * L, g, L);
+      else store_vec(dz + (size_t)n * L, g, L);
+    }
     if (score) score[n] = sq / (float)L;
   }
   block_partials(vals, partials, scale0, stats, acc);
@@ -272,12 +289,8 @@
 __global__ __launch_bounds__(64) void k_head_finalize(const float* __restrict__ partials, int P,
                                                        float scale0, float* __restrict__ stats,
                                                        float* __restrict__ acc) {
-  const int k = threadIdx.x;
-  if (k >= kHeadSlots) return;
-  double s = 0.0;
-  for (int p = 0; p < P; ++p) s += (double)partials[p * kHeadSlots + k];
-  if (stats) stats[k] = (float)(k == 0 ? s * (double)scale0 : s);
-  if (acc) acc[k] += (float)s;
+  static_assert(kHeadSlots == LMAX + 3, "head_finalize_columns' row length");
+  head_finalize_columns(partials, P, scale0, stats, acc);
 }
 
 __global__ __launch_bounds__(kFlatBlock) void k_poincare_dist(const float* __restrict__ zh,
@@ -417,11 +430,28 @@
   if (L > LMAX) return wide_mse_head(z, c, dz, score, stats, acc, upstream, ws, B, L, stream);
   const int P = head_blocks(B);
   hipLaunchKernelGGL(k_mse_head, dim3(P), dim3(kFlatBlock), 0, stream, z, c, dz, score, ws, B, L,
-                     upstream / ((float)B * (float)L), 1.f / ((float)B * (float)L), stats, acc);
+                     upstream / ((float)B * (float)L), 1.f / ((float)B * (float)L), stats, acc, (const float*)nullptr,
+                     (const float*)nullptr, 0, (float*)nullptr);
   if ((stats || acc) && P > 1)
     hipLaunchKernelGGL(k_head_finalize, dim3(1), dim3(64), 0, stream, ws, P, 1.f / ((float)B * (float)L), stats, acc);
   return check_launch("mse_head");
 }
+
+int coskad_btlnk_sum_mse_head_f32(const float* part, const float* bias, int KS, const float* c, float* z, float* dz, float* score,
+                                  float* stats, float* acc, float upstream, float* ws, int B, int L, int defer_finalize,
+                                  hipStream_t stream) {
+  if (!part || !c || !z || !ws) return fail(COSKAD_ERR_ARG, "btlnk_sum_mse_head: null pointer");
+  if (B <= 0 || L <= 0 || L > LMAX || KS <= 0) return fail(COSKAD_ERR_SHAPE, "btlnk_sum_mse_head: B=%d latent=%d (max %d) KS=%d", B, L, LMAX, KS);
+  if ((size_t)part & 15) return fail(COSKAD_ERR_ARG, "btlnk_sum_mse_head: part must be 16-byte aligned");
+  const int P = head_blocks(B);
+  hipLaunchKernelGGL(k_mse_head, dim3(P), dim3(kFlatBlock), 0, stream, (const float*)nullptr, c, dz, score, ws, B, L,
+                     upstream / ((float)B * (float)L), 1.f / ((float)B * (float)L), stats, acc, part, bias, KS, z);
+  if ((stats || acc) && P > 1 && !defer_finalize)
+    hipLaunchKernelGGL(k_head_finalize, dim3(1), dim3(64), 0, stream, ws, P, 1.f / ((float)B * (float)L), stats, acc);
+  return check_launch("btlnk_sum_mse_head");
+}
+
+int coskad_head_finalize_pending(int B) { return B > 0 && head_blocks(B) > 1 ? head_blocks(B) : 0; }
 
 int coskad_mahalanobis_head_f32(const float* z, const float* c, const float* VI, float* dz, float* score,
                                 float* stats, float* acc, float* gram, int gram_accumulate, float upstream,
diff --git a/coskad_amd/csrc/heads_common.h b/coskad_amd/csrc/heads_common.h
--- a/coskad_amd/csrc/heads_common.h
+++ b/coskad_amd/csrc/heads_common.h
@@ -14,6 +14,49 @@
 __host__ __device__ inline int head_lp(int L) { return L > LMAX ? L : LMAX; }
 __host__ __device__ inline int head_slots_for(int L) { return head_lp(L) + 3; }
 
+#ifdef __HIPCC__
+__device__ __forceinline__ void load_z_row_from_slabs(const float* __restrict__ part, const float* __restrict__ bias, int KS, int B,
+                                                      int n, int L, float (&zr)[LMAX]) {
+  static_assert(LMAX == 16, "slab rows are 16 floats");
+  float s[LMAX];
+#pragma unroll
+  for (int j = 0; j < LMAX; ++j) s[j] = 0.f;
+  auto add = [&](const float4 (&v)[4]) {
+#pragma unroll
+    for (int q = 0; q < 4; ++q) { s[4 * q] += v[q].x; s[4 * q + 1] += v[q].y; s[4 * q + 2] += v[q].z; s[4 * q + 3] += v[q].w; }
+  };
+  int k = 0;
+  for (; k + 4 <= KS; k += 4) {
+    float4 v[4][4];
+#pragma unroll
+    for (int u = 0; u < 4; ++u)
+#pragma unroll
+      for (int q = 0; q < 4; ++q) v[u][q] = reinterpret_cast<const float4*>(part + ((size_t)(k + u) * B + n) * 16)[q];
+#pragma unroll
+    for (int u = 0; u < 4; ++u) add(v[u]);
+  }
+  for (; k < KS; ++k) {
+    float4 v[4];
+#pragma unroll
+    for (int q = 0; q < 4; ++q) v[q] = reinterpret_cast<const float4*>(part + ((size_t)k * B + n) * 16)[q];
+    add(v);
+  }
+#pragma unroll
+  for (int j = 0; j < LMAX; ++j) zr[j] = j < L ? s[j] + (bias ? bias[j] : 0.f) : 0.f;
+}
+
+__device__ __forceinline__ void head_finalize_columns(const float* __restrict__ partials, int P, float scale0,
+                                                      float* __restrict__ stats, float* __restrict__ acc) {
+  constexpr int S = LMAX + 3;
+  const int k = threadIdx.x;
+  if (k >= S) return;
+  double s = 0.0;
+  for (int p = 0; p < P; ++p) s += (double)partials[p * S + k];
+  if (stats) stats[k] = (float)(k == 0 ? s * (double)scale0 : s);
+  if (acc) acc[k] += (float)s;
+}
+#endif
+
 size_t wide_head_ws_floats(int B, int L);
 int wide_mse_head(const float* z, const float* c, float* dz, float* score, float* stats, float* acc, float upstream, float* ws,
                   int B, int L, hipStream_t stream);
diff --git a/coskad_amd/csrc/layer_launch.h b/coskad_amd/csrc/layer_launch.h
--- a/coskad_amd/csrc/layer_launch.h
+++ b/coskad_amd/csrc/layer_launch.h
@@ -102,6 +102,13 @@
   float* bias = nullptr;
   float* stat = nullptr;
 };
+struct FtabArgs {
+  const float* A[4];
+  const float* Tm[4];
+  float* tab[4];
+  int n;
+};
+
 struct LayerStatsArgs {
   const float* in = nullptr;
   const float* A = nullptr;
@@ -117,6 +124,7 @@
   size_t ws_bytes = 0;
   int B = 0, Ci = 0, Co = 0;
   hipStream_t stream = nullptr;
+  const FtabArgs* ftab = nullptr;
 };
 
 void launch_reduce_partials(const float* partials, int rows, int E, double* out, hipStream_t st);
@@ -169,7 +177,7 @@
                      const float* in_slope, float* partials, int B, int Ci, int Co, int T, int V, int max_rows, hipStream_t st,
                      int* rows_out);
 int launch_first_moments(const float* in, const float* Aw, const float* Tw, const float* in_slope, float* partials, int B, int Ci,
-                         int T, int V, float* Zout, int max_rows, hipStream_t st, int* rows_out);
+                         int T, int V, float* Zout, int max_rows, hipStream_t st, int* rows_out, const FtabArgs* ftab = nullptr);
 int launch_first_apply(const float* Z, const float* in, float* out, const float* wfold, const float* bias, const float* in_slope,
                        int B, int Ci, int Co, int TVr, hipStream_t st);
 bool fwd_moments_bpc_ok(int T_, int V_, int Ci);
@@ -205,9 +213,16 @@
 int launch_layer_apply_next_bpc(const float* Z, const float* in, float* out, const float* wfold, const float* bias,
                                 const float* in_slope, const float* out_slope, const float* ftab, float* Znext, float* partials,
                                 int B, int Ci, int Co, hipStream_t st);
+struct HeadPending {
+  const float* partials = nullptr;
+  int P = 0;
+  float scale0 = 0.f;
+  float* stats = nullptr;
+  float* acc = nullptr;
+};
 int launch_btlnk_reduce(const float* partials, int P, size_t E, float* out, const float* dz, int B, int L, float* db,
                         const float* dap, int nda, float* dslope, int accumulate, hipStream_t stream, const float* rows,
-                        int RP, int RE, double* rsum);
+                        int RP, int RE, double* rsum, const HeadPending& head = HeadPending{});
 size_t wide_btlnk_fwd_ws_bytes(int B, int K, int L);
 size_t wide_btlnk_bwd_ws_bytes(int B, int K, int L);
 int wide_btlnk_fwd(const float* U, const float* W, const float* bias, const float* slope, float* z, void* ws, int B, int K, int L,
diff --git a/coskad_amd/csrc/stsgcn_train.hip b/coskad_amd/csrc/stsgcn_train.hip
--- a/coskad_amd/csrc/stsgcn_train.hip
+++ b/coskad_amd/csrc/stsgcn_train.hip
@@ -295,7 +295,7 @@
   const int need_x = a.sums ? 1 : (a.p.Wr != nullptr);
   int rows = grid;
   if (a.Zout && Ci <= 4 && TV % 4 == 0) {
-    int rc1 = launch_first_moments(a.in, a.A, a.Tm, a.in_slope, partials, B, Ci, T, V, a.Zout, kMaxGrid, st, &rows);
+    int rc1 = launch_first_moments(a.in, a.A, a.Tm, a.in_slope, partials, B, Ci, T, V, a.Zout, kMaxGrid, st, &rows, a.ftab);
     if (rc1) return rc1;
   } else if (a.Zout && fwd_moments_bpc_ok(T, V, Ci)) {
     ProbeScope probe(KID_FWD_MOMENTS, Ci, Co, st);
@@ -371,6 +371,7 @@
 extern "C" {
 
 size_t coskad_train_stats_ws_bytes(int Ci) { return train_stats_ws_bytes(Ci); }
+int coskad_layer_train_stats_ftab_ok(int Ci, int T, int V) { return Ci > 0 && Ci <= 4 && T == 12 && V == 17; }
 int coskad_stat_floats(int Ci, int Co) { return stat_floats(Ci, Co); }
 
 int coskad_layer_train_stats_z_f32(const float* in, const float* A, const float* Tm, const float* in_slope,
@@ -392,6 +393,35 @@
   return dispatch_train_stats("layer_train_stats", a, T, V, true);
 }
 
+int coskad_layer_train_stats_z_ftab_f32(const float* in, const float* A, const float* Tm, const float* in_slope,
+                                        const float* Wt, const float* bt, const float* gamma_t,
+                                        const float* beta_t, float* rmean_t, float* rvar_t, long long* nbt_t,
+                                        const float* Wr, const float* br, const float* gamma_r,
+                                        const float* beta_r, float* rmean_r, float* rvar_r, long long* nbt_r,
+                                        float momentum, float* wfold, float* bias, float* stat, void* ws,
+                                        size_t ws_bytes, int B, int Ci, int Co, int T, int V,
+                                        hipStream_t stream, float* Z, const float* const* tab_A, const float* const* tab_T,
+                                        float* const* tab, int n_tab) {
+  if (!tab_A || !tab_T || !tab || n_tab < 1 || n_tab > 4) return fail(COSKAD_ERR_ARG, "layer_train_stats_ftab: 1..4 tables, got %d", n_tab);
+  if (!coskad_layer_train_stats_ftab_ok(Ci, T, V) || !Z)
+    return fail(COSKAD_ERR_SHAPE, "layer_train_stats_ftab: C_in=%d T=%d V=%d (needs C_in <= 4, T = 12, V = 17, Z stored)", Ci, T, V);
+  FtabArgs fa{};
+  fa.n = n_tab;
+  for (int i = 0; i < n_tab; ++i) {
+    if (!tab_A[i] || !tab_T[i] || !tab[i]) return fail(COSKAD_ERR_ARG, "layer_train_stats_ftab: null pointer (table %d)", i);
+    fa.A[i] = tab_A[i]; fa.Tm[i] = tab_T[i]; fa.tab[i] = tab[i];
+  }
+  const LayerStatsArgs a{
+      .in = in, .A = A, .Tm = Tm, .in_slope = in_slope,
+      .p = {.Wt = Wt, .bt = bt, .gt = gamma_t, .bet = beta_t, .rm_t = rmean_t, .rv_t = rvar_t, .nbt_t = nbt_t, .Wr = Wr, .br = br,
+            .gr = gamma_r, .ber = beta_r, .rm_r = rmean_r, .rv_r = rvar_r, .nbt_r = nbt_r, .momentum = momentum},
+      .out = {.wfold = wfold, .bias = bias, .stat = stat},
+      .Zout = Z, .ws = ws, .ws_bytes = ws_bytes, .B = B, .Ci = Ci, .Co = Co, .stream = stream, .ftab = &fa};
+  if (int rc = check_layer_stats("layer_train_stats_ftab", a, kNeedInput | kNeedFold | kNeedWs)) return rc;
+  if (B <= 0 || Ci <= 0 || Co <= 0) return fail(COSKAD_ERR_ARG, "layer_train_stats_ftab: B=%d Ci=%d Co=%d", B, Ci, Co);
+  return dispatch_train_stats("layer_train_stats_ftab", a, T, V, true);
+}
+
 int coskad_layer_train_stats_f32(const float* in, const float* A, const float* Tm, const float* in_slope,
                                  const float* Wt, const float* bt, const float* gamma_t,
                                  const float* beta_t, float* rmean_t, float* rvar_t, long long* nbt_t,
diff --git a/coskad_amd/engine.py b/coskad_amd/engine.py
--- a/coskad_amd/engine.py
+++ b/coskad_amd/engine.py
@@ -133,16 +133,21 @@
     h, slope = x, in_slope
     n = len(layers)
     fuse = [False] * n
-    ftab = None
+    ftab = ftab_ride = None
     if all(batch_stats) and STORE_Z and FUSE_NEXT:
         for i in range(n - 1):
             fuse[i] = layers[i + 1].Ci == layers[i].Co and ops.layer_apply_next_ok(layers[i].Ci, layers[i].Co, T, V)
         nxt = [i + 1 for i in range(n - 1) if fuse[i]]
         if nxt:
             ftab = torch.empty(n, ops.ftab_floats(), device=x.device, dtype=torch.float32)
+            ride = (pending0 is None and sync is None and len(nxt) >= 1 and ops.layer_train_stats_ftab_ok(layers[0].Ci, T, V))
             for k in range(0, len(nxt), 4):
                 grp = nxt[k:k + 4]
-                ops.build_ftabs([layers[i].A for i in grp], [layers[i].T for i in grp], [ftab[i] for i in grp])
+                tabs = ([layers[i].A for i in grp], [layers[i].T for i in grp], [ftab[i] for i in grp])
+                if ride and k == 0:
+                    ftab_ride = tabs
+                else:
+                    ops.build_ftabs(*tabs)
     fuse_flat = [False] * n
     if all(batch_stats) and STORE_Z and FUSE_NEXT and sync is None:
         for i in range(n - 1):
@@ -183,7 +188,8 @@
                     Z = torch.empty_like(h)
                 wfold, bias, stat = ops.layer_train_stats(
                     h, L.A, L.T, slope, L.w2(L.Wt), L.bt, L.gt, L.bet, L.rm_t, L.rv_t, L.nbt_t,
-                    L.w2(L.Wr), L.br, L.gr, L.ber, L.rm_r, L.rv_r, L.nbt_r, buf, momentum=L.step_momentum(), Z=Z)
+                    L.w2(L.Wr), L.br, L.gr, L.ber, L.rm_r, L.rv_r, L.nbt_r, buf, momentum=L.step_momentum(), Z=Z,
+                    ftabs=ftab_ride if i == 0 else None)
         else:
             wfold, bias = eval_fold(L)
             stat = None
@@ -242,16 +248,23 @@
             self.ws = torch.empty(ws_bytes, device=device, dtype=torch.uint8)
 
 
+def btlnk_chain_ok(ctx: Optional[ChainCtx], layers: List[LayerTensors], U: Tensor, W: Tensor) -> bool:
+    i = len(layers) - 1 if layers else -1
+    Z = ctx.zs[i] if (ctx is not None and ctx.zs and i >= 0) else None
+    return bool(FUSE_TOP and Z is not None and U.dim() == 4 and layers[i].Wr is not None and W.shape[0] <= 16
+                and ops.btlnk_bwd_chain_ok(U.numel() // U.shape[0], U.shape[2] * U.shape[3], layers[i].Ci))
+
+
 def btlnk_backward(ctx: Optional[ChainCtx], layers: List[LayerTensors], U: Tensor, W: Tensor, dz: Tensor, slope: Optional[Tensor],
-                   dW: Tensor, db: Optional[Tensor], dslope: Optional[Tensor], ws: Workspace):
+                   dW: Tensor, db: Optional[Tensor], dslope: Optional[Tensor], ws: Workspace, head=None):
     B = U.shape[0]
     K, L = U.numel() // B, W.shape[0]
     i = len(layers) - 1 if layers else -1
-    Z = ctx.zs[i] if (ctx is not None and ctx.zs and i >= 0) else None
-    if (FUSE_TOP and Z is not None and U.dim() == 4 and layers[i].Wr is not None and L <= 16
-            and ops.btlnk_bwd_chain_ok(K, U.shape[2] * U.shape[3], layers[i].Ci)):
+    if btlnk_chain_ok(ctx, layers, U, W):
         in_slope = layers[i - 1].slope if i > 0 else ctx.in_slope
-        return ops.btlnk_bwd_chain(U, W, dz, slope, dW, db, dslope, ws, ctx.inputs[i], Z, in_slope)
+        return ops.btlnk_bwd_chain(U, W, dz, slope, dW, db, dslope, ws, ctx.inputs[i], ctx.zs[i], in_slope, head=head)
+    if head is not None:
+        raise ValueError("btlnk_backward: a deferred head finish rides in the chain form only (btlnk_chain_ok)")
     buf = ws.get(ops.btlnk_bwd_ws_bytes(B, K, L), U.device)
     return ops.btlnk_bwd(U, W, dz, slope, dW, db, dslope, buf), None
 
diff --git a/coskad_amd/ops.py b/coskad_amd/ops.py
--- a/coskad_amd/ops.py
+++ b/coskad_amd/ops.py
@@ -168,7 +168,7 @@
 
 
 def layer_train_stats(x, A, Tm, in_slope, Wt, bt, gt, bet, rm_t, rv_t, nbt_t,
-                      Wr, br, gr, ber, rm_r, rv_r, nbt_r, ws, momentum: float = 0.1, Z: Optional[Tensor] = None):
+                      Wr, br, gr, ber, rm_r, rv_r, nbt_r, ws, momentum: float = 0.1, Z: Optional[Tensor] = None, ftabs=None):
     B, Ci, T, V = x.shape
     Co = Wt.shape[0]
     _chk(x, "x"); _chk(A, "A", (T, V, V)); _chk(Tm, "T", (V, T, T))
@@ -189,11 +189,27 @@
     _chk(Z, "Z", tuple(x.shape), optional=True)
     args = (x, A, Tm, in_slope, Wt, bt, gt, bet, rm_t, rv_t, nbt_t, Wr, br, gr, ber, rm_r, rv_r, nbt_r, momentum, wfold, bias, stat, ws,
             ws.numel() * ws.element_size(), B, Ci, Co, T, V, _stream())
-    if Z is None:
+    if ftabs is not None:
+        As, Ts, tabs = ftabs
+        n = len(As)
+        if Z is None or not layer_train_stats_ftab_ok(Ci, T, V) or not (1 <= n <= 4) or len(Ts) != n or len(tabs) != n:
+            raise ValueError("layer_train_stats: ftabs ride with a stored-Z few-channel layer at T=12, V=17, 1..4 tables")
+        nf = ftab_floats()
+        for A2, T2, tab in zip(As, Ts, tabs):
+            _chk(A2, "ftab A", (T, V, V)); _chk(T2, "ftab T", (V, T, T)); _chk(tab, "tab", (nf,))
+        arr = ctypes.c_void_p * n
+        call("coskad_layer_train_stats_z_ftab_f32", x, A, Tm, in_slope, Wt, bt, gt, bet, rm_t, rv_t, nbt_t, Wr, br, gr, ber, rm_r, rv_r, nbt_r,
+             momentum, wfold, bias, stat, ws, ws.numel() * ws.element_size(), B, Ci, Co, T, V, _stream(), Z,
+             arr(*[t.data_ptr() for t in As]), arr(*[t.data_ptr() for t in Ts]), arr(*[t.data_ptr() for t in tabs]), n)
+    elif Z is None:
         call("coskad_layer_train_stats_f32", *args)
     else:
         call("coskad_layer_train_stats_z_f32", *args, Z)
     return wfold, bias, stat
+
+
+def layer_train_stats_ftab_ok(Ci: int, T: int, V: int) -> bool:
+    return bool(_lib.lib().coskad_layer_train_stats_ftab_ok(Ci, T, V))
 
 
 def layer_train_moments(x, A, Tm, in_slope, ws, Z: Optional[Tensor] = None) -> Tensor:
@@ -480,6 +496,24 @@
     return z
 
 
+def btlnk_fwd_slabs_ok(K: int, L: int) -> bool:
+    return L <= 16 and K % 16 == 0 and BTLNK_SPLITK_MIN_B <= 1
+
+
+def btlnk_fwd_slabs(U: Tensor, W: Tensor, slope: Optional[Tensor], ws=None) -> Tensor:
+    B = U.shape[0]
+    K = U.numel() // B
+    L = W.shape[0]
+    _chk(U, "U"); _chk(W, "W", (L, K)); _chk(slope, "slope", (1,), optional=True)
+    if not btlnk_fwd_slabs_ok(K, L):
+        raise ValueError(f"btlnk_fwd_slabs: K={K} L={L} (needs K % 16 == 0, L <= 16)")
+    lib = _lib.lib()
+    nbytes = lib.coskad_btlnk_fwd_ws_bytes(B)
+    buf = ws.get(nbytes, U.device) if ws is not None else torch.empty(nbytes, dtype=torch.uint8, device=U.device)
+    call("coskad_btlnk_fwd_slabs_f32", U, W, slope, buf, nbytes, B, K, L, _stream())
+    return buf[:nbytes].view(torch.float32).view(lib.coskad_btlnk_fwd_slabs_ks(), B, 16)
+
+
 BTLNK_SPLITK_MIN_B = 1
 BTLNK_LMAX = 512
 
@@ -507,7 +541,7 @@
     return bool(_lib.lib().coskad_btlnk_bwd_chain_ok(K, TV, below_Ci))
 
 
-def btlnk_bwd_chain(U, W, dz, slope, dW, db, dslope, ws, below_in, below_Z, below_in_slope, dU=None, accumulate=False):
+def btlnk_bwd_chain(U, W, dz, slope, dW, db, dslope, ws, below_in, below_Z, below_in_slope, dU=None, accumulate=False, head=None):
     B, Ch, T, V = U.shape
     TV = T * V
     K = Ch * TV
@@ -525,6 +559,11 @@
     if dU is None:
         dU = torch.empty_like(U)
     rows = ctypes.c_int(0)
+    if head is not None:
+        hws, hscale0, hstats, hacc = head
+        call("coskad_btlnk_bwd_chain_head_f32", U, W, dz, slope, dU, dW, db, dslope, buf, _bytes(buf), 1 if accumulate else 0, B, K, L,
+             below_in, below_Z, below_in_slope, Ci, TV, stats, _bytes(stats), ctypes.byref(rows), hws, hscale0, hstats, hacc, _stream())
+        return dU, (stats, rows.value)
     call("coskad_btlnk_bwd_chain_f32", U, W, dz, slope, dU, dW, db, dslope, buf, _bytes(buf), 1 if accumulate else 0, B, K, L, below_in,
          below_Z, below_in_slope, Ci, TV, stats, _bytes(stats), ctypes.byref(rows), _stream())
     return dU, (stats, rows.value)
@@ -846,6 +885,27 @@
     stats = torch.empty(S, device=z.device, dtype=torch.float32)
     call("coskad_mse_head_f32", z, c, dz, score, stats, acc, upstream, ws, B, L, _stream())
     return stats, dz, score
+
+
+def head_finalize_pending(B: int) -> int:
+    return _lib.lib().coskad_head_finalize_pending(B)
+
+
+def mse_head_from_slabs(part, bias, c, need_grad=True, need_score=False, acc=None, upstream=1.0, ws=None, defer=False):
+    KS, B, _ = part.shape
+    L = c.shape[0]
+    S = head_slots(L)
+    _chk(part, "part", (KS, B, 16)); _chk(c, "c", (L,)); _chk(bias, "bias", (L,), optional=True); _chk(acc, "acc", (S,), optional=True)
+    if L > 16:
+        raise ValueError("mse_head_from_slabs: latent <= 16")
+    ws = head_ws(B, part.device, L) if ws is None else ws
+    z = torch.empty(B, L, device=part.device, dtype=torch.float32)
+    dz = torch.empty_like(z) if need_grad else None
+    score = torch.empty(B, device=part.device, dtype=torch.float32) if need_score else None
+    stats = torch.empty(S, device=part.device, dtype=torch.float32)
+    call("coskad_btlnk_sum_mse_head_f32", part, bias, KS, c, z, dz, score, stats, acc, upstream, ws, B, L, 1 if defer else 0, _stream())
+    pending = (ws, 1.0 / (float(B) * float(L)), stats, acc) if (defer and head_finalize_pending(B)) else None
+    return z, stats, dz, score, pending
 
 
 def mahalanobis_head(z, c, VI, need_grad=True, need_score=False, acc=None, gram=None, gram_accumulate=True,
diff --git a/coskad_amd/trainer.py b/coskad_amd/trainer.py
--- a/coskad_amd/trainer.py
+++ b/coskad_amd/trainer.py
@@ -548,17 +548,25 @@
         m, gv = self.model, self.fp.gviews
         U, slope, saved_stack = self.stack.forward(x, self.ws)
         ctx, top_layers = self.stack.top(saved_stack)
+        stats = pending = None
         if self.mlp:
             wname, W = "btlnk.net.0.", m.btlnk.net[0].weight
             z, saved = self._mlp_forward(U, slope)
         else:
             wname, W = "btlnk.", m.btlnk.weight
-            z = ops.btlnk_fwd(U, W, m.btlnk.bias, slope, ws=self.ws)
-        stats, dz = self._head(z)
+            if self.head == 'euclidean' and ops.btlnk_fwd_slabs_ok(U.numel() // U.shape[0], W.shape[0]):
+                bctx = ctx if self.side is None else None
+                part = ops.btlnk_fwd_slabs(U, W, slope, ws=self.ws)
+                z, stats, dz, _, pending = ops.mse_head_from_slabs(part, m.btlnk.bias, m.c, acc=self.center_acc,
+                                                                   defer=engine.btlnk_chain_ok(bctx, top_layers or [], U, W))
+            else:
+                z = ops.btlnk_fwd(U, W, m.btlnk.bias, slope, ws=self.ws)
+        if stats is None:
+            stats, dz = self._head(z)
         if self.mlp:
             dz = self._mlp_backward(saved, dz)
         dU, top_stats = engine.btlnk_backward(ctx if self.side is None else None, top_layers or [], U, W, dz, slope, gv[wname + "weight"],
-                                              gv.get(wname + "bias"), self.stack.last_slope_grad, self.ws)
+                                              gv.get(wname + "bias"), self.stack.last_slope_grad, self.ws, head=pending)
         work = None
         if self.world > 1 and self.tail_off is not None:
             work = dist.all_reduce(self.fp.grad[self.tail_off:], group=self.pg, async_op=True)
diff --git a/include/coskad_hip.h b/include/coskad_hip.h
--- a/include/coskad_hip.h
+++ b/include/coskad_hip.h
@@ -7,6 +7,7 @@
 #endif
 
 int coskad_abi_version(void);
+unsigned long long coskad_launch_count(void);
 const char* coskad_last_error(void);
 
 int coskad_probe_begin(int kernel, int Ci, int Co);
@@ -75,6 +76,16 @@
                                    float momentum, float* wfold, float* bias, float* stat, void* ws,
                                    size_t ws_bytes, int B, int Ci, int Co, int T, int V,
                                    hipStream_t stream, float* Z);
+int coskad_layer_train_stats_ftab_ok(int Ci, int T, int V);
+int coskad_layer_train_stats_z_ftab_f32(const float* in, const float* A, const float* Tm, const float* in_slope,
+                                        const float* Wt, const float* bt, const float* gamma_t,
+                                        const float* beta_t, float* rmean_t, float* rvar_t, long long* nbt_t,
+                                        const float* Wr, const float* br, const float* gamma_r,
+                                        const float* beta_r, float* rmean_r, float* rvar_r, long long* nbt_r,
+                                        float momentum, float* wfold, float* bias, float* stat, void* ws,
+                                        size_t ws_bytes, int B, int Ci, int Co, int T, int V,
+                                        hipStream_t stream, float* Z, const float* const* tab_A, const float* const* tab_T,
+                                        float* const* tab, int n_tab);
 int coskad_layer_apply_z_f32(const float* Z, const float* in, float* out, const float* A, const float* Tm,
                              const float* wfold, const float* bias, const float* in_slope, const float* out_slope,
                              int B, int Ci, int Co, int T, int V, hipStream_t stream);
@@ -225,6 +236,9 @@
 size_t coskad_btlnk_fwd_ws_bytes_l(int B, int K, int L);
 int coskad_btlnk_fwd_ws_f32(const float* U, const float* W, const float* bias, const float* slope, float* z, void* ws,
                             size_t ws_bytes, int B, int K, int L, hipStream_t stream);
+int coskad_btlnk_fwd_slabs_ks(void);
+int coskad_btlnk_fwd_slabs_f32(const float* U, const float* W, const float* slope, void* ws, size_t ws_bytes, int B, int K, int L,
+                               hipStream_t stream);
 size_t coskad_btlnk_bwd_ws_bytes(int B, int K, int L);
 int coskad_btlnk_bwd_f32(const float* U, const float* W, const float* dz, const float* slope, float* dU,
                          float* dW, float* db, float* dslope, void* ws, size_t ws_bytes, int accumulate,
@@ -238,6 +252,11 @@
                                float* db, float* dslope, void* ws, size_t ws_bytes, int accumulate, int B, int K, int L,
                                const float* below_in, const float* below_Z, const float* below_in_slope, int below_Ci, int TV,
                                float* stats_out, size_t stats_out_bytes, int* stats_rows, hipStream_t stream);
+int coskad_btlnk_bwd_chain_head_f32(const float* U, const float* W, const float* dz, const float* slope, float* dU, float* dW,
+                                    float* db, float* dslope, void* ws, size_t ws_bytes, int accumulate, int B, int K, int L,
+                                    const float* below_in, const float* below_Z, const float* below_in_slope, int below_Ci, int TV,
+                                    float* stats_out, size_t stats_out_bytes, int* stats_rows, const float* head_ws,
+                                    float head_scale0, float* head_stats, float* head_acc, hipStream_t stream);
 
 
 int coskad_gather_transform_f32(const float* xy, const long long* index, const float* mats, float* out, int B, int N,
@@ -251,6 +270,10 @@
 
 int coskad_mse_head_f32(const float* z, const float* c, float* dz, float* score, float* stats, float* acc,
                         float upstream, float* ws, int B, int L, hipStream_t stream);
+int coskad_btlnk_sum_mse_head_f32(const float* part, const float* bias, int KS, const float* c, float* z, float* dz, float* score,
+                                  float* stats, float* acc, float upstream, float* ws, int B, int L, int defer_finalize,
+                                  hipStream_t stream);
+int coskad_head_finalize_pending(int B);
 
 int coskad_mahalanobis_head_f32(const float* z, const float* c, const float* VI, float* dz, float* score,
                                 float* stats, float* acc, float* gram, int gram_accumulate, float upstream,
```

Measured after the change: 3.008 million clips/s (median of 6 runs). Within noise of the previous version (+0.8%).
